# pghysels/STRUMPACK

Hardware: AMD Instinct MI355X
Metric: hss_compress_ulv_factor_solve_gflops (higher is better)
Workload: dtype f64

## Files before the change

include/hssk.h:

```cpp
#ifndef HSSK_H
#define HSSK_H

#ifdef __cplusplus
extern "C" {
#endif

typedef struct hssk_ctx hssk_ctx;

int hssk_ctx_create(hssk_ctx** ctx, int device);
void hssk_ctx_destroy(hssk_ctx* ctx);
void* hssk_ctx_stream(hssk_ctx* ctx);
int hssk_sync(hssk_ctx* ctx);
const char* hssk_last_error(void);
typedef struct hssk_plan hssk_plan;
int hssk_plan_begin(hssk_ctx* ctx, hssk_plan** plan);
int hssk_plan_end(hssk_ctx* ctx);
int hssk_plan_replay(hssk_ctx* ctx, hssk_plan* plan);
void hssk_plan_destroy(hssk_plan* plan);
int hssk_plan_size(const hssk_plan* plan);

void* hssk_malloc(long long bytes);
void hssk_free(void* dptr);
long long hssk_device_total_bytes(void);
int hssk_memcpy_h2d(hssk_ctx* ctx, void* dst, const void* src, long long bytes);
int hssk_memcpy_d2h(hssk_ctx* ctx, void* dst, const void* src, long long bytes);
int hssk_upload_async(hssk_ctx* ctx, void* dst, const void* src, long long bytes);
int hssk_memcpy_d2d(hssk_ctx* ctx, void* dst, const void* src, long long bytes);
int hssk_memcpy2d_h2d(hssk_ctx* ctx, void* dst, long long dpitch, const void* src, long long spitch,
                      long long width, long long height);
int hssk_memcpy2d_d2h(hssk_ctx* ctx, void* dst, long long dpitch, const void* src, long long spitch,
                      long long width, long long height);
int hssk_memset_zero(hssk_ctx* ctx, void* dst, long long bytes);
int hssk_h2d_block_async(hssk_ctx* ctx, double* dst, long long ldd, const double* src, long long lds, long long rows,
                         long long cols);
int hssk_h2d_bytes_async(hssk_ctx* ctx, void* dst, long long dpitch, const void* src, long long spitch, long long width,
                         long long cols);
int hssk_copy_fence(hssk_ctx* ctx);
int hssk_compute_fence(hssk_ctx* ctx);
int hssk_compute_mark(hssk_ctx* ctx, int slot);
int hssk_copy_wait(hssk_ctx* ctx, int slot);
int hssk_is_device_pointer(const void* ptr);
typedef struct hssk_aca_desc {
  const double* A;
  int lda, m, n;
  double rtol, atol;
  int max_rank, row0;
  double* U;
  int ldu;
  double* V;
  int ldv;
  int* rank;
} hssk_aca_desc;
int hssk_aca_vbatched(hssk_ctx* ctx, const hssk_aca_desc* descs, int count);
int hssk_side_begin(hssk_ctx* ctx);
int hssk_side_end(hssk_ctx* ctx);
int hssk_side_join(hssk_ctx* ctx);
int hssk_stream_wait(hssk_ctx* waiter, hssk_ctx* on);
int hssk_watch_start(hssk_ctx* ctx, int id);
int hssk_watch_stop(hssk_ctx* ctx, int id);
double hssk_watch_read_ms(hssk_ctx* ctx, int id, int* pairs);
float hssk_last_dgemm_ms(hssk_ctx* ctx);
double hssk_last_dgemm_flops(hssk_ctx* ctx);
int hssk_dgemm_timing_defer(hssk_ctx* ctx);
int hssk_dgemm_timing_collect(hssk_ctx* ctx, double* ms, double* flops, int* launches);
long long hssk_last_dgemm_trace(hssk_ctx* ctx, long long* out, long long max_wgs);
double hssk_last_dgemm_clock_ghz(hssk_ctx* ctx);

int hssk_fill_toeplitz(hssk_ctx* ctx, double* A, int n, long long lda, char kind);
int hssk_fill_toeplitz_block(hssk_ctx* ctx, double* A, int rows, int cols, long long lda, int i0, int j0, char kind);
int hssk_randn(hssk_ctx* ctx, double* P, int rows, long long cols, long long ld, int row0,
               long long stride, unsigned long long seed);

int hssk_dgemm(hssk_ctx* ctx, int transB, int m, long long n, long long k, double alpha,
               const double* A, long long lda, const double* B, long long ldb, double beta,
               double* C, long long ldc);

int hssk_sgemm_sketch(hssk_ctx* ctx, int transB, int m, long long n, long long k, double alpha,
                      const double* A, long long lda,
                      const float* B, long long ldb,
                      double beta, double* C, long long ldc);
int hssk_narrow_f32(hssk_ctx* ctx, float* dst, long long ldd, const double* src, long long lds, long long rows, long long cols);

#define HSSK_GEN_TOEPLITZ 1
#define HSSK_GEN_TOEPLITZ_UPPER 2
typedef struct hssk_gen {
  int kind, reserved;
  double p[4];
} hssk_gen;
int hssk_sketch_gen(hssk_ctx* ctx, const hssk_gen* g, int transG, int m, long long n, long long k, long long j0, double alpha,
                    const double* A, long long lda, double beta, double* C, long long ldc);
int hssk_gen_fill(hssk_ctx* ctx, const hssk_gen* g, double* A, long long rows, long long cols, long long lda, long long i0,
                  long long j0, int trans);

typedef struct hssk_gemm_desc {
  const double* A;
  const double* B;
  double* C;
  int m, n, k;
  int lda, ldb, ldc;
  int transA, transB;
  double alpha, beta;
} hssk_gemm_desc;
int hssk_gemm_vbatched(hssk_ctx* ctx, const hssk_gemm_desc* descs, int count);

typedef struct hssk_leaf_update_desc {
  const double* R;
  const double* D;
  double* Sr;
  double* Sc;
  int d, m, ldr, ldd, lds;
} hssk_leaf_update_desc;
int hssk_leaf_update_vbatched(hssk_ctx* ctx, const hssk_leaf_update_desc* descs, int count);

typedef struct hssk_kernel_spec {
  const double* X;
  long long n;
  int d, type, p;
  double h, lambda;
} hssk_kernel_spec;
typedef struct hssk_keval_desc {
  const int* ri;
  const int* ci;
  double* out;
  int nr, nc, ldo, r0, c0;
} hssk_keval_desc;
int hssk_kernel_eval_vbatched(hssk_ctx* ctx, const hssk_kernel_spec* spec, const hssk_keval_desc* descs, int count);
int hssk_knn(hssk_ctx* ctx, const double* X, int d, int n, int k, int q0, int q1, int* out_idx);
typedef struct hssk_colset_desc {
  const int* src0;
  const int* src1;
  int n0, n1, lo, hi;
  int* out;
  int* count;
  const int* n0_dev;
  const int* n1_dev;
} hssk_colset_desc;
int hssk_colsets(hssk_ctx* ctx, const hssk_colset_desc* descs, int count, int universe);
long long hssk_colsets_max_universe(void);
int hssk_cluster_median(hssk_ctx* ctx, double* X, int d, int n, int algo, int cluster_size, int* perm, int* status);
int hssk_kernel_predict(hssk_ctx* ctx, const hssk_kernel_spec* spec, const double* w, const double* T, int m, double* pred);

typedef struct hssk_colgather_desc {
  const double* src;
  double* dst;
  const int* idx;
  int rows, ncols, lds, ldd;
  int scatter;
} hssk_colgather_desc;
int hssk_gather_cols(hssk_ctx* ctx, const hssk_colgather_desc* descs, int count);
enum { HSSK_DT_F64 = 0, HSSK_DT_F32 = 1, HSSK_DT_C32 = 2, HSSK_DT_C64 = 3 };
int hssk_expand_image(hssk_ctx* ctx, double* dst, long long ldd, const void* src, long long lds, long long rows, long long cols,
                      int dtype);
typedef struct hssk_rowgather_desc {
  const double* src;
  double* dst;
  const int* idx;
  int nrows, cols, lds, ldd;
  int scatter, accumulate;
} hssk_rowgather_desc;
int hssk_gather_rows(hssk_ctx* ctx, const hssk_rowgather_desc* descs, int count);
typedef struct hssk_elem_desc {
  const double* A;
  long long lda;
  const int* I;
  const int* J;
  int i0, j0;
  double* B;
  int m, n, ldb, transpose;
  int rlo, rhi, clo, chi;
} hssk_elem_desc;
int hssk_gather_elems(hssk_ctx* ctx, const hssk_elem_desc* descs, int count);
int hssk_gather_elems_f32(hssk_ctx* ctx, const hssk_elem_desc* descs, int count);
int hssk_gen_elems(hssk_ctx* ctx, const hssk_gen* g, const hssk_elem_desc* descs, int count);
int hssk_sum_slabs(hssk_ctx* ctx, const double* slabs, long long count, long long stride, int nslab, double* out);
typedef struct hssk_transpose_desc {
  const double* src;
  double* dst;
  int rows, cols, lds, ldd;
} hssk_transpose_desc;
int hssk_transpose(hssk_ctx* ctx, const hssk_transpose_desc* descs, int count);

typedef struct hssk_triu_desc {
  const double* src;
  double* dst;
  int rows, cols, lds, ldd;
  int dstride;
} hssk_triu_desc;
int hssk_copy_triu(hssk_ctx* ctx, const hssk_triu_desc* descs, int count);

int hssk_sjlt_dense(hssk_ctx* ctx, double* Rt, int dn, long long K, long long ld, const int* pat, int nnz);
int hssk_sjlt_sketch(hssk_ctx* ctx, int transA, long long n_out, long long K, const double* A, long long lda,
                     const int* pat, int nnz, int dn, double* St, long long lds);

typedef struct hssk_combine_desc {
  const double *G0, *G1;
  int ldg, gsplit;
  const int* gidx;
  const double *M0, *M1;
  int ldm, msplit;
  const int* midx;
  const double* C;
  int csj, csk;
  double alpha;
  double* out;
  int ldo, rows, J, K;
} hssk_combine_desc;
int hssk_gather_combine(hssk_ctx* ctx, const hssk_combine_desc* descs, int count);

typedef struct hssk_ulvsplit_desc {
  const double* D;
  int ldd, m, r;
  const int* perm;
  const double* X;
  int ldx;
  double* W1;
  int ldw;
  double* W0t;
  int ldt;
} hssk_ulvsplit_desc;
int hssk_ulv_split(hssk_ctx* ctx, const hssk_ulvsplit_desc* descs, int count);
typedef struct hssk_ulvnode_desc {
  const double *B01, *B10, *Vt1a, *Vt1b, *Vd;
  double *Dh, *Vh;
  int ra, rb, rva, rvb;
  int eliminate;
  const int* perm;
  const double* X;
  double *W1, *Rlq, *Qt, *tau, *Vt0T, *Vt1, *Dt, *WQ;
  int m, r, rv, ldt;
} hssk_ulvnode_desc;
int hssk_ulv_node_vbatched(hssk_ctx* ctx, const hssk_ulvnode_desc* descs, int count);
int hssk_ulv_node_fits(int m, int r, int rv, int ra, int rb, int rva, int rvb);
long long hssk_ulv_node_launches(void);

typedef struct hssk_id_desc {
  double* W;
  int ldw, d, m;
  double rtol, atol;
  int max_rank;
  int* perm;
  int* rank;
  double* work;
  const double* src;
  int lds;
  int defer_x;
} hssk_id_desc;
int hssk_id_vbatched(hssk_ctx* ctx, const hssk_id_desc* descs, int count);
long long hssk_id_group_launches(void);
int hssk_id_solves_inline(int dmax, int mmax);
typedef struct hssk_xsolve_desc {
  const double* W;
  int ldw, rank, m;
  double* X;
  int ldx, solved;
} hssk_xsolve_desc;
int hssk_id_xsolve_vbatched(hssk_ctx* ctx, const hssk_xsolve_desc* descs, int count);
typedef struct hssk_pchol_desc {
  const double* G;
  int ldg, m;
  double rtol, atol;
  int max_rank;
  int* perm;
  int* rank;
  double* R;
  int ldr;
} hssk_pchol_desc;
int hssk_pchol_id_vbatched(hssk_ctx* ctx, const hssk_pchol_desc* descs, int count);
int hssk_pchol_id_max_m(void);
int hssk_pchol_id_rank_cap(int m);
typedef struct hssk_sum_desc {
  const double* P;
  long long stride, n;
  int count;
  double* out;
} hssk_sum_desc;
int hssk_sum_partials(hssk_ctx* ctx, const hssk_sum_desc* descs, int count);
typedef struct hssk_gram_desc {
  const double* W;
  int ldw, rows, m;
  double* G;
  int ldg;
} hssk_gram_desc;
int hssk_gram_vbatched(hssk_ctx* ctx, const hssk_gram_desc* descs, int count);
typedef struct hssk_gramgen_desc {
  const int* ri;
  int r0;
  const int* ci;
  int c0;
  int rows, m;
  double* G;
  int ldg;
} hssk_gramgen_desc;
int hssk_gram_gen_vbatched(hssk_ctx* ctx, const hssk_kernel_spec* spec, const hssk_gramgen_desc* descs, int count);
int hssk_gram_gen_supported(const hssk_kernel_spec* spec, int mmax);

typedef struct hssk_tnode {
  int c0, c1, lvl, reserved;
  double* S[2];
  int* perm[2];
  double* Rred[2];
  int* I[2];
  double* X[2];
  double *B01, *B10;
  double* W[2];
  int r[2], m[2], flag[2];
  int status, pad;
} hssk_tnode;
typedef struct hssk_elem_src {
  const double* A;
  long long lda;
  hssk_gen gen;
  int use_gen;
} hssk_elem_src;
int hssk_tree_inner(hssk_ctx* ctx, hssk_tnode* nodes, const int* order, int count, int d, int lds, int rcap, double rtol,
                    double atol, int max_rank, const hssk_elem_src* src, int* res);
int hssk_tree_rcap_max(void);

typedef struct hssk_qr_desc {
  double* A;
  int lda, rows, cols;
  double* Q;
  int ldq, nq;
  double* rdiag;
  double* work;
  int stair;
  double stop_rel, stop_abs;
  int r_only;
} hssk_qr_desc;
int hssk_qr_vbatched(hssk_ctx* ctx, const hssk_qr_desc* descs, int count);
typedef struct hssk_tpqr_desc {
  double* R1;
  int ld1;
  const double* R2;
  int ld2, m;
} hssk_tpqr_desc;
int hssk_tpqr_vbatched(hssk_ctx* ctx, const hssk_tpqr_desc* descs, int count);
int hssk_formq_vbatched(hssk_ctx* ctx, const hssk_qr_desc* descs, int count);

typedef struct hssk_trsm_desc {
  const double* T;
  double* B;
  int n, nrhs, ldt, ldb;
  int lower, transT, unit;
  const double* Tinv;
} hssk_trsm_desc;
int hssk_trsm_vbatched(hssk_ctx* ctx, const hssk_trsm_desc* descs, int count);
typedef struct hssk_lu_desc {
  double* A;
  int n, lda;
  int* piv;
  int* info;
} hssk_lu_desc;
int hssk_getrf_vbatched(hssk_ctx* ctx, const hssk_lu_desc* descs, int count);
typedef struct hssk_lusolve_desc {
  const double* LU;
  const int* piv;
  double* B;
  int n, nrhs, lda, ldb;
} hssk_lusolve_desc;
int hssk_getrs_vbatched(hssk_ctx* ctx, const hssk_lusolve_desc* descs, int count);
int hssk_laswp_vbatched(hssk_ctx* ctx, const hssk_lusolve_desc* descs, int count);

typedef struct hssk_blr_term {
  const double* U;
  const double* V;
  int r, n, src_off, src_flag;
} hssk_blr_term;
typedef struct hssk_blr_row {
  int first_term, nterms, off, m;
  const double* LU;
  int lda, mode;
  const int* piv;
  const double* Tinv;
} hssk_blr_row;
int hssk_blr_sweep(hssk_ctx* ctx, const hssk_blr_row* rows, int nrows, const hssk_blr_term* terms, int nterms, double* X, int* flags);
int hssk_blr_sweep_check(const hssk_blr_row* rows, int nrows, const hssk_blr_term* terms, int nterms);
int hssk_blr_sweep_resident(hssk_ctx* ctx, const hssk_blr_row* d_rows, int nrows, const hssk_blr_term* d_terms, double* X, int* flags);

int hssk_sweep_arm(hssk_ctx* ctx, double* handoff, long long count);
typedef struct hssk_sweep_fwd_desc {
  const double* fsrc;
  const double *B01, *B10, *zc;
  const int* permU;
  const double* XU;
  const double* Rlq;
  const double* Tinv;
  const double* WQ;
  const double* Vt0T;
  const int* permV;
  const double* XV;
  double *ft1, *y, *z;
  const double *LU, *TinvL, *TinvU;
  const int* piv;
  double* xroot;
  int ldf, rU0, rU1, rV0, rV1, ldz_in, m, r, mv, rv, ldp, ldz, ldxr;
  int wait0, wait1;
  const double* G;
  int ldg;
} hssk_sweep_fwd_desc;
int hssk_sweep_chain_ok(int m, int r, int mv, int rv);
long long hssk_sweep_chain_launches(void);
int hssk_ulv_fwd_sweep(hssk_ctx* ctx, const hssk_sweep_fwd_desc* descs, int count, int nrhs);
typedef struct hssk_sweep_bwd_desc {
  const double *Qt, *y, *xpart;
  double* out;
  int m, r, ldx, ldo;
  int wait0;
} hssk_sweep_bwd_desc;
int hssk_ulv_bwd_sweep(hssk_ctx* ctx, const hssk_sweep_bwd_desc* descs, int count, int nrhs);
typedef struct hssk_apply_up_desc {
  const double* src;
  const int* perm;
  const double* X;
  double* dst;
  int m, r, lds, ldd;
  int inner;
  int wait0, wait1;
} hssk_apply_up_desc;
typedef struct hssk_apply_down_desc {
  const double* tmp2;
  const int* perm;
  const double* X;
  const double *D, *x;
  const double *B01, *B10, *t1;
  double* out;
  double beta;
  int ld2, mo, ro, m, ldx, trans, ri_a, ri_b, ro_a, ro_b, ldt1, ldo;
  int wait0, wait1, wait2;
  int acc;
} hssk_apply_down_desc;
int hssk_apply_sweep(hssk_ctx* ctx, const hssk_apply_up_desc* ups, int nup, const hssk_apply_down_desc* downs, int ndown,
                     int nrhs);
int hssk_sweep_status(hssk_ctx* ctx);
int hssk_sweep_require_mma(hssk_ctx* ctx, int on);
int hssk_sweep_mma_min_nrhs(void);
long long hssk_sweep_mma_launches(void);
long long hssk_sweep_fused_launches(void);
long long hssk_sweep_fallbacks(void);
typedef struct hssk_trtri_desc {
  const double* R;
  double* Tinv;
  int n, ldr;
  int mode;
} hssk_trtri_desc;
int hssk_trtri_diag_vbatched(hssk_ctx* ctx, const hssk_trtri_desc* descs, int count);

typedef struct hssk_tree_node {
  int lo, m, c0, c1;
  int rU, rV, mU, mV;
  const double *XU, *XV;
  const int *ipermU, *ipermV;
  const double *B01, *B10, *D;
} hssk_tree_node;
typedef struct hssk_extract_block {
  int ri0, ni, cj0, nj;
  double* out;
  int ldo;
} hssk_extract_block;
int hssk_hss_extract(hssk_ctx* ctx, const hssk_tree_node* nodes, int root, int rmax, int maxdepth, const int* rows, int nrows,
                     const int* cols, int ncols, const hssk_extract_block* blocks, const long long* pair_off, int nblocks,
                     long long npairs, int accumulate, double* work);

typedef struct hssk_norm_desc {
  const double* P;
  int rows, cols, ld;
  double* out;
} hssk_norm_desc;
int hssk_sumsq_vbatched(hssk_ctx* ctx, const hssk_norm_desc* descs, int count);
typedef struct hssk_basis_desc {
  const double* X;
  const int* perm;
  double* out;
  int m, r, ldx, ldo;
} hssk_basis_desc;
int hssk_basis_dense(hssk_ctx* ctx, const hssk_basis_desc* descs, int count);
typedef struct hssk_shift_desc {
  double* A;
  int n, lda;
} hssk_shift_desc;
int hssk_shift_diag(hssk_ctx* ctx, const hssk_shift_desc* descs, int count, double sigma);
int hssk_shift_diag_cplx(hssk_ctx* ctx, const hssk_shift_desc* descs, int count, double re, double im);
double hssk_mfma_f64_peak_tflops(hssk_ctx* ctx, int iters);
int hssk_mfma_f64_probe(hssk_ctx* ctx, int iters, int waves_per_simd, int zero_data, double* out);

#ifdef __cplusplus
}
#endif
#endif
```

strumpack_amd/csrc/host/hss_compress.cpp:

```cpp
#include "hss_engine_internal.hpp"
#include <cstdio>

namespace strumpack {
namespace HSS {

void DeviceHSS::drop_plans() {
  for (auto& kv : plans_) if (kv.second.plan) hssk_plan_destroy(kv.second.plan);
  plans_.clear();
  if (plan_arena_) plan_arena_->reset();
}
bool DeviceHSS::plans_enabled() const {
  static const bool off = [] { const char* e = std::getenv("STRUMPACK_AMD_NO_PLANS"); return e && e[0] == '1'; }();
  return !off;
}

void DeviceHSS::reset_compression() {
  book_ = PendingBook();
  defer_book_ = false;
  drop_plans();
  for (auto& nd : nodes_) {
    int lo = nd.lo, m = nd.m, lvl = nd.lvl, h = nd.height, c0 = nd.c0, c1 = nd.c1, p = nd.parent;
    nd = Node();
    nd.lo = lo; nd.m = m; nd.lvl = lvl; nd.height = h; nd.c0 = c0; nd.c1 = c1; nd.parent = p;
  }
  factor_cancel();
  persist_->reset();
  dev_tree_ = nullptr;
  work_->reset();
  fact_->reset();
  invalidate_factors();
  d_ranks_ = persist_->ints(2 * nodes_.size() + 2);
}

void DeviceHSS::restart_nodes(int d_have) {
  ck(hssk_sync(ctx_));
  factor_cancel();
  for (auto& nd : nodes_) {
    int lo = nd.lo, m = nd.m, lvl = nd.lvl, h = nd.height, c0 = nd.c0, c1 = nd.c1, p = nd.parent;
    nd = Node();
    nd.lo = lo; nd.m = m; nd.lvl = lvl; nd.height = h; nd.c0 = c0; nd.c1 = c1; nd.parent = p;
  }
  persist_->reset();
  dev_tree_ = nullptr;
  invalidate_factors();
  d_ranks_ = persist_->ints(2 * nodes_.size() + 2);
  if (d_have > 0) {
    std::vector<hssk_colgather_desc> cp;
    const int ncols = (int)std::min<long long>(n_, 0x7fffffff);
    cp.push_back(hssk_colgather_desc{Srt0_, Srt_, nullptr, d_have, ncols, dcap_, dcap_, 0});
    cp.push_back(hssk_colgather_desc{Sct0_, Sct_, nullptr, d_have, ncols, dcap_, dcap_, 0});
    ck(hssk_gather_cols(ctx_, cp.data(), 2));
  }
}

void DeviceHSS::free_compress_workspace() {
  ck(hssk_sync(ctx_));
  work_->reset();
  Rt_ = Srt_ = Sct_ = Srt0_ = Sct0_ = nullptr;
  sj_pat_ = nullptr;
  for (auto& nd : nodes_) { nd.Srt = nd.Sct = nd.Rrt = nd.Rct = nd.RrtRed = nd.RctRed = nd.Qr = nd.Qc = nullptr; nd.panels = false; }
}

void DeviceHSS::compress(Source& src) {
  OpGuard op_guard(op_mu_);
  double t0 = now();
  stats_ = PhaseStats();
  int dcap = o_.algorithm != 1 ? o_.d0 + o_.p : o_.d0 + o_.dd;
  dcap = std::max(16, (dcap + 15) / 16 * 16);
  for (;;) {
    if (compress_attempt(src, dcap)) break;
    dcap *= 2;
    if (o_.verbose) std::cout << "# HSS compression: growing the sample capacity to " << dcap << std::endl;
  }
  static const bool trace_host = [] { const char* e = std::getenv("STRUMPACK_AMD_TRACE_HOST"); return e && e[0] == '1'; }();
  const double th0 = now();
  if (dist_subtree_) exchange_node_table();
  free_compress_workspace();
  comm_arena_->reset();
  const double th1 = now();
  {
    const double ms = hssk_watch_read_ms(ctx_, 5, nullptr);
    if (ms > 0.) stats_.t_sketch = ms * 1e-3;
    double kms = 0., kfl = 0.;
    int kn = 0;
    ck(hssk_dgemm_timing_collect(ctx_, &kms, &kfl, &kn));
    stats_.sketch_kernel_ms += kms; stats_.sketch_kernel_flops += kfl; stats_.sketch_launches += kn;
  }
  stats_.t_compress = now() - t0;
  stats_.t_tree = stats_.t_compress - stats_.t_sketch - stats_.t_random;
  stats_.t_mark = now();
  if (trace_host) std::fprintf(stderr, "# host: compress end: free workspace %.1f us, timers %.1f us\n", (th1 - th0) * 1e6, (now() - th1) * 1e6);
}

void DeviceHSS::fill_random(int r0, int dn) {
  if (o_.user_random) { sj_pat_ = nullptr; return; }
  double t0 = now();
  const long long N = n_;
  sj_pat_ = nullptr;
  if (o_.sketch == 1) {
    if (r0 == 0 || !rng_) rng_.reset(new HostRng());
    auto& e = rng_->sj;
    const int nnz = std::max(1, std::min(r0 == 0 ? o_.nnz0 : o_.nnz, dn));
    const bool dense_pat = nnz > 8;
    const int nq = dense_pat ? nnz : (nnz <= 4 ? 4 : 8);
    std::vector<int> pat((size_t)nq * N, dn);
    std::uniform_int_distribution<int> sign(0, 1);
    if (o_.sjlt_algo == 0) {
      const int chunk = dn / nnz;
      std::uniform_int_distribution<int> shift(0, chunk - 1);
      for (long long k = 0; k < N; k++)
        for (int q = 0; q < nnz; q++) {
          const int c = shift(e) + chunk * q;
          pat[(size_t)k * nq + q] = sign(e) == 0 ? c : (c | (int)0x80000000);
        }
    } else {
      std::vector<int> cols(dn);
      for (int j = 0; j < dn; j++) cols[j] = j;
      for (long long k = 0; k < N; k++)
        for (int q = 0; q < nnz; q++) {
          std::uniform_int_distribution<int> pick(q, dn - 1);
          std::swap(cols[q], cols[pick(e)]);
          pat[(size_t)k * nq + q] = sign(e) == 0 ? cols[q] : (cols[q] | (int)0x80000000);
        }
    }
    if (dense_pat) {
      std::vector<double> buf((size_t)dn * N, 0.);
      host_parallel_for((size_t)N, [&](size_t k) {
        for (int q = 0; q < nnz; q++) {
          const int p = pat[k * nq + q];
          buf[(size_t)(p & 0x7fffffff) + k * dn] = p < 0 ? -1. : 1.;
        }
      });
      ck(hssk_memcpy2d_h2d(ctx_, Rt_ + r0, sizeof(double) * dcap_, buf.data(), sizeof(double) * dn, sizeof(double) * dn, N));
      ck(hssk_sync(ctx_));
      stats_.t_random += now() - t0;
      return;
    }
    int* dp = work_->ints((size_t)nq * N);
    ck(hssk_memcpy_h2d(ctx_, dp, pat.data(), (long long)sizeof(int) * nq * N));
    ck(hssk_sjlt_dense(ctx_, Rt_ + r0, dn, N, dcap_, dp, nnz));
    sj_pat_ = dp;
    sj_nnz_ = nnz;
  } else if (o_.random_engine == 2) {
    if (o_.random_dist != 0) throw std::invalid_argument("philox engine implements the normal distribution only");
    ck(hssk_randn(ctx_, Rt_ + r0, dn, N, dcap_, r0, N, 0x5354524dull));
  } else {
    if (r0 == 0 || !rng_) rng_.reset(new HostRng());
    if (o_.random_engine == 0 && o_.random_dist == 0 && N > 0 && dn > 0) {
      std::vector<double> blk((size_t)dn * N);
      rng_->linnorm.fill(blk.data(), blk.size(), [](std::size_t n, const std::function<void(std::size_t)>& fn) { host_parallel_for(n, fn); });
      double* dT = tmp_->dbl((size_t)dn * N);
      ck(hssk_memcpy_h2d(ctx_, dT, blk.data(), (long long)(sizeof(double) * blk.size())));
      hssk_transpose_desc t{dT, Rt_ + r0, (int)N, dn, (int)N, dcap_};
      ck(hssk_transpose(ctx_, &t, 1));
    } else {
      std::minstd_rand* lin = &rng_->lin;
      std::mt19937* mer = &rng_->mer;
      auto& nd = rng_->nd;
      auto& ud = rng_->ud;
      std::vector<double> buf((size_t)dn * N);
      for (int s = 0; s < dn; s++)
        for (long long c = 0; c < N; c++) {
          double v;
          if (o_.random_engine == 0) v = o_.random_dist == 0 ? nd(*lin) : ud(*lin);
          else v = o_.random_dist == 0 ? nd(*mer) : ud(*mer);
          buf[s + (size_t)c * dn] = v;
        }
      ck(hssk_memcpy2d_h2d(ctx_, Rt_ + r0, sizeof(double) * dcap_, buf.data(), sizeof(double) * dn, sizeof(double) * dn, N));
    }
  }
  ck(hssk_sync(ctx_));
  stats_.t_random += now() - t0;
}

bool DeviceHSS::compress_attempt(Source& src, int dcap) {
  reset_compression();
  attempt_++;
  dcap_ = dcap;
  const size_t N = n_;
  cols_per_rank_ = o_.world > 1 ? ((long long)N + o_.world - 1) / o_.world : (long long)N;
  const size_t Npad = o_.world > 1 ? (size_t)cols_per_rank_ * o_.world : N;
  Rt_ = work_->dbl((size_t)dcap * N);
  Srt_ = work_->dbl((size_t)dcap * Npad);
  Sct_ = work_->dbl((size_t)dcap * Npad);
  if (o_.algorithm == 2) { Srt0_ = work_->dbl((size_t)dcap * Npad); Sct0_ = work_->dbl((size_t)dcap * Npad); }
  stats_.rounds = 0;
  stats_.f_sketch = stats_.f_local = stats_.f_reduce = stats_.f_id = stats_.f_ortho = 0;
  const bool original = (o_.algorithm != 1);
  if (!original) {
    int d = o_.d0, dd = o_.dd;
    while (!is_compressed()) {
      int c = (d == o_.d0) ? 0 : d;
      int dnew = (d == o_.d0) ? d + dd : dd;
      if (c + dnew > dcap) return false;
      fill_random(c, dnew);
      if (stats_.rounds == 0 && src.extract_before_sample()) {
        std::vector<int> leaves;
        for (auto& ids : own_by_height_) for (int id : ids) if (nodes_[id].leaf() && nodes_[id].lvl != 0) leaves.push_back(id);
        extract_blocks(src, leaves);
      }
      ck(hssk_watch_start(ctx_, 5));
      src.sample(*this, c, dnew);
      ck(hssk_watch_stop(ctx_, 5));
      stats_.f_sketch += src.sketch_flops(*this, dnew);
      if (o_.verbose) std::cout << "# compressing with d+dd = " << d << "+" << dd << " (stable)" << std::endl;
      stats_.rounds++;
      for (size_t h = 0; h < own_by_height_.size(); h++) {
        if (h == 1 && tree_pass(src, d, dd)) {
          for (size_t hh = 1; hh < own_by_height_.size(); hh++) factor_ahead_level(hh);
          break;
        }
        process_level(src, own_by_height_[h], d, dd, false);
        factor_ahead_level(h);
      }
      if (dist_subtree_) {
        exchange_cut_compress(d + dd);
        for (auto& ids : top_by_height_) process_level(src, ids, d, dd, false);
      }
      stats_.d_final = d + dd;
      if (!is_compressed()) {
        d += dd;
        dd = std::min(dd, o_.max_rank - d);
        if (dd <= 0) break;
      }
    }
  } else {
    int d_old = 0, d = o_.d0 + o_.p;
    while (!is_compressed()) {
      if (d > dcap) return false;
      fill_random(d_old, d - d_old);
      ck(hssk_watch_start(ctx_, 5));
      src.sample(*this, d_old, d - d_old);
      ck(hssk_watch_stop(ctx_, 5));
      stats_.f_sketch += src.sketch_flops(*this, d - d_old);
      if (o_.verbose) std::cout << "# compressing with d = " << d - o_.p << " + " << o_.p << (o_.algorithm == 2 ? " (original, hard restart)" : " (original)") << std::endl;
      if (o_.algorithm == 2) {
        if (dist_subtree_ || o_.world > 1) throw std::invalid_argument("hard restart is a single-GPU option");
        std::vector<hssk_colgather_desc> cp;
        cp.push_back(hssk_colgather_desc{Srt_ + d_old, Srt0_ + d_old, nullptr, d - d_old, (int)N, dcap_, dcap_, 0});
        cp.push_back(hssk_colgather_desc{Sct_ + d_old, Sct0_ + d_old, nullptr, d - d_old, (int)N, dcap_, dcap_, 0});
        ck(hssk_gather_cols(ctx_, cp.data(), 2));
      }
      stats_.rounds++;
      for (auto& ids : own_by_height_) process_level(src, ids, d, d - d_old, true);
      if (dist_subtree_) {
        exchange_cut_compress(d);
        for (auto& ids : top_by_height_) process_level(src, ids, d, d - d_old, true);
      }
      stats_.d_final = d;
      if (!is_compressed()) {
        d_old = d;
        d = 2 * (d_old - o_.p) + o_.p;
        if (d_old >= 4 * n_ + o_.p + 64) break;
        if (o_.algorithm == 2 && d <= dcap) restart_nodes(d_old);
      }
    }
  }
  return true;
}

void DeviceHSS::process_level(Source& src, const std::vector<int>& ids_all, int d, int dd, bool original) {
  const int dtot = original ? d : d + dd;
  const int dnew0 = original ? d - dd : d;
  std::vector<int> ids;
  for (int id : ids_all) {
    Node& nd = nodes_[id];
    if (!nd.leaf() && !(nodes_[nd.c0].compressed() && nodes_[nd.c1].compressed())) continue;
    if (nd.lvl == 0 && nd.compressed()) continue;
    ids.push_back(id);
  }
  if (ids.empty()) return;
  std::vector<int> fresh;
  std::vector<char> was_untouched(nodes_.size(), 0), was_compressed(nodes_.size(), 0);
  for (int id : ids) {
    Node& nd = nodes_[id];
    was_untouched[id] = nd.untouched();
    was_compressed[id] = nd.compressed();
    if (nd.untouched()) fresh.push_back(id);
  }
  extract_blocks(src, fresh);
  std::vector<int> work_ids, r0s, dns;
  for (int id : ids) {
    Node& nd = nodes_[id];
    if (nd.lvl == 0) { nd.Ustate = nd.Vstate = 2; continue; }
    if (!nd.panels) {
      if (nd.leaf()) {
        nd.mU = nd.mV = nd.m;
        nd.Srt = Srt_ + (size_t)nd.lo * dcap_;
        nd.Sct = Sct_ + (size_t)nd.lo * dcap_;
        nd.Rrt = nd.Rct = Rt_ + (size_t)nd.lo * dcap_;
      } else {
        nd.mU = nodes_[nd.c0].rU + nodes_[nd.c1].rU;
        nd.mV = nodes_[nd.c0].rV + nodes_[nd.c1].rV;
        nd.Srt = work_->dbl((size_t)dcap_ * std::max(nd.mU, 1));
        nd.Sct = work_->dbl((size_t)dcap_ * std::max(nd.mV, 1));
        nd.Rrt = work_->dbl((size_t)dcap_ * std::max(nd.mV, 1));
        nd.Rct = work_->dbl((size_t)dcap_ * std::max(nd.mU, 1));
      }
      nd.panels = true;
    }
    work_ids.push_back(id);
    r0s.push_back(was_untouched[id] ? 0 : dnew0);
    dns.push_back(was_untouched[id] ? dtot : dtot - dnew0);
  }
  if (work_ids.empty()) return;
  local_samples(work_ids, r0s, dns);

  std::vector<int> id_nodes, id_which, ot_nodes, ot_which;
  for (int id : work_ids) {
    Node& nd = nodes_[id];
    if (was_compressed[id]) continue;
    for (int w = 0; w < 2; w++) {
      int st = w == 0 ? nd.Ustate : nd.Vstate;
      if (st == 2) continue;
      int rows = w == 0 ? nd.mU : nd.mV;
      if (original || dtot >= o_.max_rank || dtot >= rows) { id_nodes.push_back(id); id_which.push_back(w); }
      else { ot_nodes.push_back(id); ot_which.push_back(w); }
    }
  }
  if (!ot_nodes.empty()) {
    std::vector<char> resolved;
    ortho_test(ot_nodes, ot_which, d, dd, resolved);
    for (size_t i = 0; i < ot_nodes.size(); i++) {
      if (resolved[i]) { id_nodes.push_back(ot_nodes[i]); id_which.push_back(ot_which[i]); }
      else {
        Node& nd = nodes_[ot_nodes[i]];
        (ot_which[i] == 0 ? nd.Ustate : nd.Vstate) = 1;
      }
    }
  }
  defer_book_ = !original;
  run_id(id_nodes, id_which, dtot);
  defer_book_ = false;
  if (original) {
    for (int id : work_ids) {
      Node& nd = nodes_[id];
      if (was_compressed[id]) continue;
      bool ok = (dtot - o_.p >= o_.max_rank) || (nd.rU < dtot - o_.p && nd.rV < dtot - o_.p);
      if (!ok) { nd.Ustate = nd.Vstate = 1; nd.rU = nd.rV = 0; nd.Ir.clear(); nd.Ic.clear(); }
    }
  }
  std::vector<int> rd_ids, rd_r0, rd_dn;
  for (int id : work_ids) {
    Node& nd = nodes_[id];
    if (!nd.compressed()) continue;
    if (!was_compressed[id]) {
      nd.RrtRed = work_->dbl((size_t)dcap_ * std::max(nd.rV, 1));
      nd.RctRed = work_->dbl((size_t)dcap_ * std::max(nd.rU, 1));
      rd_ids.push_back(id); rd_r0.push_back(0); rd_dn.push_back(dtot);
    } else {
      rd_ids.push_back(id); rd_r0.push_back(dnew0); rd_dn.push_back(dtot - dnew0);
    }
  }
  reduce_samples(rd_ids, rd_r0, rd_dn);
  finish_id_bookkeeping();
}

void DeviceHSS::extract_blocks(Source& src, const std::vector<int>& ids) {
  std::vector<ElemReq> reqs;
  for (int id : ids) {
    Node& nd = nodes_[id];
    if (nd.leaf()) {
      if (nd.D) continue;
      nd.D = persist_->dbl((size_t)nd.m * nd.m);
      reqs.push_back(ElemReq{nullptr, nullptr, nullptr, nullptr, nd.lo, nd.lo, nd.m, nd.m, nd.D, nd.m});
    } else {
      Node &a = nodes_[nd.c0], &b = nodes_[nd.c1];
      nd.B01 = persist_->dbl((size_t)std::max(a.rU, 1) * std::max(b.rV, 1));
      nd.B10 = persist_->dbl((size_t)std::max(b.rU, 1) * std::max(a.rV, 1));
      reqs.push_back(ElemReq{a.dIr, b.dIc, &a.Ir, &b.Ic, 0, 0, a.rU, b.rV, nd.B01, std::max(a.rU, 1)});
      reqs.push_back(ElemReq{b.dIr, a.dIc, &b.Ir, &a.Ic, 0, 0, b.rU, a.rV, nd.B10, std::max(b.rU, 1)});
    }
  }
  if (!reqs.empty()) src.extract(*this, reqs);
}

void DeviceHSS::local_samples(const std::vector<int>& ids, const std::vector<int>& r0s, const std::vector<int>& dns) {
  std::vector<hssk_combine_desc> cb;
  std::vector<hssk_gemm_desc> mm;
  std::vector<hssk_leaf_update_desc> lu;
  for (size_t k = 0; k < ids.size(); k++) {
    Node& nd = nodes_[ids[k]];
    const int r0 = r0s[k], dn = dns[k];
    if (dn <= 0) continue;
    if (nd.leaf()) {
      const int m = nd.m;
      if (dn <= 192 && dn % 2 == 0 && r0 % 2 == 0 && nd.Rrt == nd.Rct)
        lu.push_back(hssk_leaf_update_desc{nd.Rrt + r0, nd.D, nd.Srt + r0, nd.Sct + r0, dn, m, dcap_, m, dcap_});
      else {
        mm.push_back(hssk_gemm_desc{nd.Rrt + r0, nd.D, nd.Srt + r0, dn, m, m, dcap_, m, dcap_, 0, 1, -1.0, 1.0});
        mm.push_back(hssk_gemm_desc{nd.Rct + r0, nd.D, nd.Sct + r0, dn, m, m, dcap_, m, dcap_, 0, 0, -1.0, 1.0});
      }
      stats_.f_local += 4.0 * m * (double)m * dn;
    } else {
      Node &a = nodes_[nd.c0], &b = nodes_[nd.c1];
      const int none = 0x7fffffff;
      const int l01 = std::max(a.rU, 1), l10 = std::max(b.rU, 1);
      cb.push_back(hssk_combine_desc{a.Srt + r0, nullptr, dcap_, none, a.permU, b.RrtRed + r0, nullptr, dcap_, none, nullptr,
                                     nd.B01, 1, l01, -1.0, nd.Srt + r0, dcap_, dn, a.rU, b.rV});
      cb.push_back(hssk_combine_desc{b.Srt + r0, nullptr, dcap_, none, b.permU, a.RrtRed + r0, nullptr, dcap_, none, nullptr,
                                     nd.B10, 1, l10, -1.0, nd.Srt + r0 + (size_t)a.rU * dcap_, dcap_, dn, b.rU, a.rV});
      cb.push_back(hssk_combine_desc{a.Sct + r0, nullptr, dcap_, none, a.permV, b.RctRed + r0, nullptr, dcap_, none, nullptr,
                                     nd.B10, l10, 1, -1.0, nd.Sct + r0, dcap_, dn, a.rV, b.rU});
      cb.push_back(hssk_combine_desc{b.Sct + r0, nullptr, dcap_, none, b.permV, a.RctRed + r0, nullptr, dcap_, none, nullptr,
                                     nd.B01, l01, 1, -1.0, nd.Sct + r0 + (size_t)a.rV * dcap_, dcap_, dn, b.rV, a.rU});
      stats_.f_local += 4.0 * ((double)a.rU * b.rV + (double)b.rU * a.rV) * dn;
    }
  }
  if (!cb.empty()) ck(hssk_gather_combine(ctx_, cb.data(), (int)cb.size()));
  if (!lu.empty()) {
    int rc = hssk_leaf_update_vbatched(ctx_, lu.data(), (int)lu.size());
    if (rc == 2) {
      for (auto& u : lu) {
        mm.push_back(hssk_gemm_desc{u.R, u.D, u.Sr, u.d, u.m, u.m, u.ldr, u.ldd, u.lds, 0, 1, -1.0, 1.0});
        mm.push_back(hssk_gemm_desc{u.R, u.D, u.Sc, u.d, u.m, u.m, u.ldr, u.ldd, u.lds, 0, 0, -1.0, 1.0});
      }
    } else ck(rc);
  }
  if (!mm.empty()) ck(hssk_gemm_vbatched(ctx_, mm.data(), (int)mm.size()));
}

void DeviceHSS::reduce_samples(const std::vector<int>& ids, const std::vector<int>& r0s, const std::vector<int>& dns) {
  if (ids.empty()) return;
  std::vector<hssk_combine_desc> cb;
  const int none = 0x7fffffff;
  for (size_t k = 0; k < ids.size(); k++) {
    Node& nd = nodes_[ids[k]];
    const int r0 = r0s[k], dn = dns[k];
    if (dn <= 0) continue;
    const double *rr0, *rr1 = nullptr, *rc0, *rc1 = nullptr;
    int sr = none, sc = none;
    if (nd.leaf()) { rr0 = nd.Rrt + r0; rc0 = nd.Rct + r0; }
    else {
      Node &a = nodes_[nd.c0], &b = nodes_[nd.c1];
      rr0 = a.RrtRed + r0; rr1 = b.RrtRed + r0; sr = a.rV;
      rc0 = a.RctRed + r0; rc1 = b.RctRed + r0; sc = a.rU;
    }
    {
      const int m = nd.mV, r = nd.rV, K = (m > r && r > 0) ? m - r : 0;
      if (r > 0)
        cb.push_back(hssk_combine_desc{rr0, rr1, dcap_, sr, nd.permV, rr0, rr1, dcap_, sr, nd.permV + r, nd.XV, 1, r, 1.0,
                                       nd.RrtRed + r0, dcap_, dn, r, K});
      stats_.f_reduce += 2.0 * r * (double)K * dn;
    }
    {
      const int m = nd.mU, r = nd.rU, K = (m > r && r > 0) ? m - r : 0;
      if (r > 0)
        cb.push_back(hssk_combine_desc{rc0, rc1, dcap_, sc, nd.permU, rc0, rc1, dcap_, sc, nd.permU + r, nd.XU, 1, r, 1.0,
                                       nd.RctRed + r0, dcap_, dn, r, K});
      stats_.f_reduce += 2.0 * r * (double)K * dn;
    }
  }
  if (!cb.empty()) ck(hssk_gather_combine(ctx_, cb.data(), (int)cb.size()));
}

void DeviceHSS::run_id(const std::vector<int>& ids, const std::vector<int>& which, int dtot) {
  if (ids.empty()) return;
  Arena& tmp = *tmp_;
  tmp.rewind();
  const size_t cnt = ids.size();
  std::vector<double*> Ws(cnt, nullptr);
  std::vector<const double*> srcs(cnt, nullptr);
  std::vector<int> ds(cnt, dtot);
  for (size_t k = 0; k < cnt; k++) {
    Node& nd = nodes_[ids[k]];
    const int m = which[k] == 0 ? nd.mU : nd.mV;
    const double* S = which[k] == 0 ? nd.Srt : nd.Sct;
    if (m == 0) continue;
    Ws[k] = tmp.dbl((size_t)dtot * m);
    srcs[k] = S;
  }
  id_panels(ids, which, Ws, ds, &srcs, dcap_);
}

static bool tsqr_staircase() {
  const char* e = std::getenv("STRUMPACK_AMD_TSQR_DENSE");
  return !(e && std::atoi(e));
}

void DeviceHSS::tsqr_reduce(const std::vector<int>& ids, const std::vector<int>& which, std::vector<double*>& Ws,
                            std::vector<int>& ds) {
  Arena& tmp = *tmp_;
  const size_t cnt = ids.size();
  struct Piece { double* p; int ld, rows; };
  std::vector<std::vector<Piece>> pieces(cnt);
  std::vector<int> ms(cnt, 0);
  bool any = false;
  std::vector<hssk_qr_desc> qr;
  for (size_t k = 0; k < cnt; k++) {
    const Node& nd = nodes_[ids[k]];
    const int m = which[k] == 0 ? nd.mU : nd.mV, d = ds[k];
    ms[k] = m;
    if (m <= 0 || !Ws[k] || d <= std::max(256, 2 * m)) continue;
    const int chunk = m <= 192 ? 256 : (m <= 208 ? 208 : (m <= 256 ? 512 : 2 * m));
    for (int r0 = 0; r0 < d; r0 += chunk) {
      const int cr = std::min(chunk, d - r0);
      double* wk = tmp.dbl((size_t)cr + m);
      qr.push_back(hssk_qr_desc{Ws[k] + r0, d, cr, m, nullptr, 0, 0, nullptr, wk, 0, 0., 0., 1});
      pieces[k].push_back(Piece{Ws[k] + r0, d, std::min(cr, m)});
      {
        const double a_ = std::max(cr, m), b_ = std::min(cr, m);
        stats_.f_ortho += 2.0 * a_ * b_ * b_ - 2.0 / 3.0 * b_ * b_ * b_;
      }
    }
    any = true;
  }
  if (!any) return;
  ck(hssk_qr_vbatched(ctx_, qr.data(), (int)qr.size()));
  static const bool pairs_off = [] { const char* e = std::getenv("STRUMPACK_AMD_TSQR_PAIRS"); return e && e[0] == '0'; }();
  for (;;) {
    std::vector<hssk_triu_desc> cp;
    std::vector<hssk_tpqr_desc> tp;
    qr.clear();
    bool more = false;
    for (size_t k = 0; k < cnt; k++) {
      std::vector<Piece>& pc = pieces[k];
      if (pc.size() <= 1) continue;
      const int m = ms[k];
      static const int fan_env = std::getenv("STRUMPACK_AMD_TSQR_FANIN") ? std::atoi(std::getenv("STRUMPACK_AMD_TSQR_FANIN")) : 0;
      const size_t fan_wide = fan_env >= 2 ? (size_t)fan_env : 2;
      const size_t fan = m <= 128 ? std::max<size_t>(2, 256 / std::max(m, 1)) : fan_wide;
      std::vector<Piece> next;
      for (size_t i = 0; i < pc.size(); i += fan) {
        const size_t cntp = std::min(fan, pc.size() - i);
        if (cntp == 1) { next.push_back(pc[i]); continue; }
        int rows = 0;
        bool full = true;
        for (size_t t = 0; t < cntp; t++) { rows += pc[i + t].rows; full = full && pc[i + t].rows == m; }
        if (cntp == 2 && full && m <= 224 && !pairs_off && tsqr_staircase()) {
          tp.push_back(hssk_tpqr_desc{pc[i].p, pc[i].ld, pc[i + 1].p, pc[i + 1].ld, m});
          next.push_back(pc[i]);
          stats_.f_ortho += 2.0 / 3.0 * (double)m * m * m;
          continue;
        }
        double* dst = tmp.dbl((size_t)rows * m);
        const bool stair = full && rows > 256 && tsqr_staircase();
        int r0 = 0;
        for (size_t t = 0; t < cntp; t++) {
          if (stair) cp.push_back(hssk_triu_desc{pc[i + t].p, dst + t, pc[i + t].rows, m, pc[i + t].ld, rows, (int)cntp});
          else cp.push_back(hssk_triu_desc{pc[i + t].p, dst + r0, pc[i + t].rows, m, pc[i + t].ld, rows, 1});
          r0 += pc[i + t].rows;
        }
        double* wk = tmp.dbl((size_t)rows + m);
        qr.push_back(hssk_qr_desc{dst, rows, rows, m, nullptr, 0, 0, nullptr, wk, stair ? (int)cntp : 0, 0., 0., 1});
        next.push_back(Piece{dst, rows, std::min(rows, m)});
        {
          const double a_ = std::max(rows, m), b_ = std::min(rows, m);
          stats_.f_ortho += (2.0 * a_ * b_ * b_ - 2.0 / 3.0 * b_ * b_ * b_) * (stair ? 1.0 / 3.0 : 1.0);
        }
      }
      pc.swap(next);
      more = more || pc.size() > 1;
    }
    if (cp.empty() && tp.empty()) break;
    if (!tp.empty()) ck(hssk_tpqr_vbatched(ctx_, tp.data(), (int)tp.size()));
    if (!cp.empty()) {
      ck(hssk_copy_triu(ctx_, cp.data(), (int)cp.size()));
      ck(hssk_qr_vbatched(ctx_, qr.data(), (int)qr.size()));
    }
    if (!more) break;
  }
  std::vector<hssk_triu_desc> fin;
  for (size_t k = 0; k < cnt; k++) {
    if (pieces[k].empty()) continue;
    const Piece& pc = pieces[k][0];
    double* R = tmp.dbl((size_t)pc.rows * ms[k]);
    fin.push_back(hssk_triu_desc{pc.p, R, pc.rows, ms[k], pc.ld, pc.rows});
    Ws[k] = R;
    ds[k] = pc.rows;
  }
  if (!fin.empty()) ck(hssk_copy_triu(ctx_, fin.data(), (int)fin.size()));
}

void DeviceHSS::id_panels(const std::vector<int>& ids, const std::vector<int>& which, const std::vector<double*>& Ws_in,
                          const std::vector<int>& ds_in, const std::vector<const double*>* srcs, int ldsrc) {
  Arena& tmp = *tmp_;
  const size_t cnt = ids.size();
  std::vector<double*> Ws(Ws_in);
  std::vector<int> ds(ds_in);
  if (srcs) {
    std::vector<hssk_colgather_desc> cp;
    bool tall = false;
    for (size_t k = 0; k < cnt; k++) tall = tall || ds[k] > 256;
    if (tall) {
      for (size_t k = 0; k < cnt; k++) {
        const int m = which[k] == 0 ? nodes_[ids[k]].mU : nodes_[ids[k]].mV;
        if (Ws[k] && m) cp.push_back(hssk_colgather_desc{(*srcs)[k], Ws[k], nullptr, ds[k], m, ldsrc, ds[k], 0});
      }
      if (!cp.empty()) ck(hssk_gather_cols(ctx_, cp.data(), (int)cp.size()));
      srcs = nullptr;
    }
  }
  static const bool gram_on = [] { const char* e = std::getenv("STRUMPACK_AMD_ID_GRAM"); return !(e && e[0] == '0'); }();
  std::vector<char> gram(cnt, 0);
  std::vector<double*> gramR(cnt, nullptr);
  std::vector<int> gramLd(cnt, 0);
  std::vector<hssk_pchol_desc> pcd;
  std::vector<size_t> pck;
  const std::vector<hssk_keval_desc>* gen = id_gen_;
  std::vector<char> evaluated(cnt, gen ? 0 : 1);
  auto evaluate = [&](const std::vector<size_t>& ks_) {
    std::vector<hssk_keval_desc> ev;
    for (size_t k : ks_)
      if (!evaluated[k] && (*gen)[k].out) { ev.push_back((*gen)[k]); evaluated[k] = 1; }
    if (!ev.empty()) ck(hssk_kernel_eval_vbatched(ctx_, &id_gen_spec_, ev.data(), (int)ev.size()));
  };
  if (gram_on && id_gram_ && !srcs) {
    std::vector<hssk_gram_desc> gd;
    std::vector<hssk_gramgen_desc> gg;
    std::vector<hssk_sum_desc> sd;
    size_t tiles_total = 0;
    for (size_t k = 0; k < cnt; k++) {
      const Node& nd = nodes_[ids[k]];
      const int m = which[k] == 0 ? nd.mU : nd.mV, d = ds[k];
      if (m <= 0 || m > hssk_pchol_id_max_m() || !Ws[k] || d <= std::max(256, 2 * m) || o_.rel_tol / nd.lvl < 1e-6) continue;
      gram[k] = 1;
      tiles_total++;
    }
    for (size_t k = 0; k < cnt; k++) {
      if (!gram[k]) continue;
      const Node& nd = nodes_[ids[k]];
      const int m = which[k] == 0 ? nd.mU : nd.mV, d = ds[k];
      static const int wgs = [] { const char* e = std::getenv("STRUMPACK_AMD_GRAM_WGS"); return e ? std::max(1, std::atoi(e)) : 768; }();
      const int want = (int)std::max<size_t>(1, ((size_t)wgs + tiles_total - 1) / tiles_total);
      const int chunks = std::max(1, std::min(want, (d + 255) / 256)), rows = ((d + chunks - 1) / chunks + 15) & ~15;
      int nch = (d + rows - 1) / rows;
      if (nch > 1 && d - (nch - 1) * rows < 16) nch--;
      double* G = tmp.dbl((size_t)m * m);
      double* P = nch > 1 ? tmp.dbl((size_t)nch * m * m) : G;
      const bool fused = gen && (*gen)[k].out == Ws[k] && hssk_gram_gen_supported(&id_gen_spec_, m);
      for (int c = 0; c < nch; c++) {
        const int r0 = c * rows, kr = c == nch - 1 ? d - r0 : rows;
        if (fused) {
          const hssk_keval_desc& kd = (*gen)[k];
          gg.push_back(hssk_gramgen_desc{kd.ri ? kd.ri + r0 : nullptr, kd.r0 + r0, kd.ci, kd.c0, kr, m, P + (size_t)c * m * m, m});
        } else gd.push_back(hssk_gram_desc{Ws[k] + r0, d, kr, m, P + (size_t)c * m * m, m});
      }
      if (!fused && gen) evaluate({k});
      if (nch > 1) sd.push_back(hssk_sum_desc{P, (long long)m * m, (long long)m * m, nch, G});
      const int cap = std::max(1, std::min(m, hssk_pchol_id_rank_cap(m)));
      gramR[k] = tmp.dbl((size_t)cap * m);
      gramLd[k] = cap;
      pcd.push_back(hssk_pchol_desc{G, m, m, o_.rel_tol / nd.lvl, o_.abs_tol / nd.lvl, o_.max_rank, nullptr, nullptr, gramR[k], cap});
      pck.push_back(k);
      stats_.f_ortho += (double)d * m * (m + 1.0);
    }
    if (!gd.empty()) ck(hssk_gram_vbatched(ctx_, gd.data(), (int)gd.size()));
    if (!gg.empty()) ck(hssk_gram_gen_vbatched(ctx_, &id_gen_spec_, gg.data(), (int)gg.size()));
    if (!sd.empty()) ck(hssk_sum_partials(ctx_, sd.data(), (int)sd.size()));
  }
  {
    std::vector<double*> Wt(Ws);
    for (size_t k = 0; k < cnt; k++) if (gram[k]) Wt[k] = nullptr;
    if (gen) {
      std::vector<size_t> rest;
      for (size_t k = 0; k < cnt; k++) if (!gram[k]) rest.push_back(k);
      evaluate(rest);
    }
    tsqr_reduce(ids, which, Wt, ds);
    for (size_t k = 0; k < cnt; k++) if (!gram[k]) Ws[k] = Wt[k];
  }
  std::vector<hssk_id_desc> idd;
  int id_dmax = 0, id_mmax = 0;
  std::vector<int*> perms(cnt, nullptr);
  size_t perm_total = 0;
  for (size_t k = 0; k < cnt; k++) perm_total += (which[k] == 0 ? nodes_[ids[k]].mU : nodes_[ids[k]].mV);
  int* rank_block = persist_->ints(cnt + std::max<size_t>(perm_total, 1));
  int* perm_block = rank_block + cnt;
  size_t poff = 0;
  for (size_t k = 0; k < cnt; k++) {
    Node& nd = nodes_[ids[k]];
    const int m = which[k] == 0 ? nd.mU : nd.mV;
    perms[k] = perm_block + poff;
    poff += m;
    if (m == 0) continue;
    if (gram[k]) continue;
    double* wk = tmp.dbl(3 * (size_t)m);
    idd.push_back(hssk_id_desc{Ws[k], ds[k], ds[k], m, o_.rel_tol / nd.lvl, o_.abs_tol / nd.lvl, o_.max_rank, perms[k], rank_block + k, wk,
                               srcs ? (*srcs)[k] : nullptr, ldsrc, 1});
    id_dmax = std::max(id_dmax, ds[k]);
    id_mmax = std::max(id_mmax, m);
  }
  if (!idd.empty()) ck(hssk_id_vbatched(ctx_, idd.data(), (int)idd.size()));
  for (size_t q = 0; q < pcd.size(); q++) { pcd[q].perm = perms[pck[q]]; pcd[q].rank = rank_block + pck[q]; }
  if (!pcd.empty()) ck(hssk_pchol_id_vbatched(ctx_, pcd.data(), (int)pcd.size()));
  const int x_solved = hssk_id_solves_inline(id_dmax, id_mmax);
  std::vector<int> hall(cnt + std::max<size_t>(perm_total, 1));
  ck(hssk_memcpy_d2h(ctx_, hall.data(), rank_block, (long long)sizeof(int) * (cnt + perm_total)));
  {
    std::vector<int> rid, rwh, rds;
    std::vector<double*> rW;
    std::vector<size_t> rk_;
    for (size_t k = 0; k < cnt; k++)
      if (gram[k] && hall[k] < 0) { rid.push_back(ids[k]); rwh.push_back(which[k]); rW.push_back(Ws[k]); rds.push_back(ds[k]); rk_.push_back(k); }
    if (!rid.empty()) {
      if (gen) evaluate(rk_);
      tsqr_reduce(rid, rwh, rW, rds);
      std::vector<hssk_id_desc> rdd;
      int dmx = 0, mmx = 0;
      for (size_t q = 0; q < rid.size(); q++) {
        const size_t k = rk_[q];
        const Node& nd = nodes_[ids[k]];
        const int m = which[k] == 0 ? nd.mU : nd.mV;
        double* wk = tmp.dbl(3 * (size_t)m);
        rdd.push_back(hssk_id_desc{rW[q], rds[q], rds[q], m, o_.rel_tol / nd.lvl, o_.abs_tol / nd.lvl, o_.max_rank, perms[k], rank_block + k, wk, nullptr, 0, 0});
        dmx = std::max(dmx, rds[q]); mmx = std::max(mmx, m);
        gram[k] = 2;
        Ws[k] = rW[q]; ds[k] = rds[q];
      }
      ck(hssk_id_vbatched(ctx_, rdd.data(), (int)rdd.size()));
      ck(hssk_memcpy_d2h(ctx_, hall.data(), rank_block, (long long)sizeof(int) * (cnt + perm_total)));
    }
  }
  if (hssk_sweep_status(ctx_)) throw std::runtime_error(std::string("compress: interpolative decomposition: ") + hssk_last_error());
  const int* hranks = hall.data();
  const int* hperm = hall.data() + cnt;
  std::vector<hssk_xsolve_desc> xc;
  std::vector<size_t> idx_off(cnt), perm_off(cnt);
  size_t idx_total = 0;
  poff = 0;
  for (size_t k = 0; k < cnt; k++) {
    Node& nd = nodes_[ids[k]];
    const int w = which[k];
    const int m = w == 0 ? nd.mU : nd.mV;
    const int dtot = gram[k] == 1 ? gramLd[k] : ds[k];
    const int r = m ? hranks[k] : 0;
    perm_off[k] = poff;
    poff += m;
    idx_off[k] = idx_total;
    idx_total += r;
    double* X = persist_->dbl((size_t)std::max(r, 1) * std::max(m - r, 1));
    if (r > 0 && m > r) xc.push_back(hssk_xsolve_desc{gram[k] == 1 ? gramR[k] : Ws[k], dtot, r, m, X, r, gram[k] == 1 ? 0 : (gram[k] == 2 ? 1 : x_solved)});
    if (w == 0) { nd.rU = r; nd.XU = X; nd.permU = perms[k]; nd.Ustate = 2; }
    else { nd.rV = r; nd.XV = X; nd.permV = perms[k]; nd.Vstate = 2; }
    stats_.f_id += 2.0 * (4.0 * m * (double)dtot * r - 2.0 * (m + dtot) * (double)r * r + 4.0 * r * (double)r * r / 3.0 + (double)r * r * (m - r));
  }
  if (!xc.empty()) ck(hssk_id_xsolve_vbatched(ctx_, xc.data(), (int)xc.size()));
  book_.ids = ids; book_.which = which; book_.hall = std::move(hall);
  book_.idx_off = std::move(idx_off); book_.perm_off = std::move(perm_off);
  book_.cnt = cnt; book_.idx_total = idx_total; book_.active = true;
  if (!defer_book_) finish_id_bookkeeping();
}

void DeviceHSS::finish_id_bookkeeping() {
  if (!book_.active) return;
  book_.active = false;
  const std::vector<int>&ids = book_.ids, &which = book_.which;
  const size_t cnt = book_.cnt, idx_total = book_.idx_total;
  const int* hperm = book_.hall.data() + cnt;
  std::vector<int> idx_host(std::max<size_t>(idx_total, 1));
  for (size_t k = 0; k < cnt; k++) {
    Node& nd = nodes_[ids[k]];
    const int w = which[k];
    const int m = w == 0 ? nd.mU : nd.mV;
    const int r = w == 0 ? nd.rU : nd.rV;
    std::vector<int> perm(hperm + book_.perm_off[k], hperm + book_.perm_off[k] + m);
    std::vector<int> I(r);
    if (nd.leaf()) for (int i = 0; i < r; i++) I[i] = nd.lo + perm[i];
    else {
      const std::vector<int>& ia = w == 0 ? nodes_[nd.c0].Ir : nodes_[nd.c0].Ic;
      const std::vector<int>& ib = w == 0 ? nodes_[nd.c1].Ir : nodes_[nd.c1].Ic;
      const int r0 = (int)ia.size();
      for (int i = 0; i < r; i++) I[i] = perm[i] < r0 ? ia[perm[i]] : ib[perm[i] - r0];
    }
    std::copy(I.begin(), I.end(), idx_host.begin() + book_.idx_off[k]);
    if (w == 0) { nd.hpermU = std::move(perm); nd.Ir = std::move(I); }
    else { nd.hpermV = std::move(perm); nd.Ic = std::move(I); }
  }
  int* idx_dev = persist_->ints(std::max<size_t>(idx_total, 1));
  if (idx_total) ck(hssk_upload_async(ctx_, idx_dev, idx_host.data(), (long long)sizeof(int) * idx_total));
  for (size_t k = 0; k < cnt; k++) {
    Node& nd = nodes_[ids[k]];
    (which[k] == 0 ? nd.dIr : nd.dIc) = idx_dev + book_.idx_off[k];
  }
}

void DeviceHSS::ortho_test(const std::vector<int>& ids, const std::vector<int>& which, int d, int dd,
                           std::vector<char>& resolved) {
  const size_t cnt = ids.size();
  resolved.assign(cnt, 0);
  Arena& tmp = *tmp_;
  tmp.rewind();
  std::vector<hssk_transpose_desc> tr;
  std::vector<hssk_colgather_desc> cp;
  std::vector<hssk_qr_desc> qr;
  double* rdiag = tmp.dbl(2 * cnt);
  std::vector<char> untouched(cnt);
  for (size_t k = 0; k < cnt; k++) {
    Node& nd = nodes_[ids[k]];
    const int w = which[k];
    const int m = w == 0 ? nd.mU : nd.mV;
    const double* S = w == 0 ? nd.Srt : nd.Sct;
    double* Q = w == 0 ? nd.Qr : nd.Qc;
    untouched[k] = (w == 0 ? nd.Ustate : nd.Vstate) == 0;
    int c2, n2;
    if (untouched[k]) { c2 = 0; n2 = std::min(d, m); }
    else { c2 = d - dd; n2 = std::min(dd, m - (d - dd)); }
    double* T = tmp.dbl((size_t)m * std::max(n2, 1));
    if (untouched[k]) tr.push_back(hssk_transpose_desc{S, T, n2, m, dcap_, m});
    else cp.push_back(hssk_colgather_desc{Q + (size_t)c2 * m, T, nullptr, m, n2, m, m, 0});
    double* wk = tmp.dbl((size_t)m + n2);
    {
      const double atol = o_.abs_tol / nd.lvl, rtol = o_.rel_tol / nd.lvl;
      const double r0 = w == 0 ? nd.Ur_max : nd.Vr_max;
      hssk_qr_desc q{T, m, m, n2, nullptr, m, 0, rdiag + 2 * k, wk, 0, 0., 0.};
      if (untouched[k]) { q.stop_rel = rtol * (1. - 1e-12); q.stop_abs = atol; }
      else q.stop_abs = std::max(atol, rtol * std::abs(r0) * (1. - 1e-12));
      qr.push_back(q);
    }
    stats_.f_ortho += 4.0 * m * (double)n2 * n2;
  }
  if (!cp.empty()) ck(hssk_gather_cols(ctx_, cp.data(), (int)cp.size()));
  if (!tr.empty()) ck(hssk_transpose(ctx_, tr.data(), (int)tr.size()));
  ck(hssk_qr_vbatched(ctx_, qr.data(), (int)qr.size()));
  std::vector<double> hr(2 * cnt);
  ck(hssk_memcpy_d2h(ctx_, hr.data(), rdiag, (long long)sizeof(double) * 2 * cnt));
  std::vector<size_t> pend;
  for (size_t k = 0; k < cnt; k++) {
    Node& nd = nodes_[ids[k]];
    const int w = which[k];
    double r_max = hr[2 * k], r_min = hr[2 * k + 1];
    double& r_max_0 = w == 0 ? nd.Ur_max : nd.Vr_max;
    if (untouched[k]) r_max_0 = r_max;
    const double atol = o_.abs_tol / nd.lvl, rtol = o_.rel_tol / nd.lvl;
    if (std::abs(r_min) < atol || std::abs(r_min / r_max_0) < rtol) resolved[k] = 1;
    else pend.push_back(k);
  }
  if (pend.empty()) return;
  {
    std::vector<hssk_qr_desc> fq;
    tr.clear();
    for (size_t k : pend) {
      Node& nd = nodes_[ids[k]];
      const int w = which[k];
      const int m = w == 0 ? nd.mU : nd.mV;
      const double* S = w == 0 ? nd.Srt : nd.Sct;
      double*& Q = w == 0 ? nd.Qr : nd.Qc;
      if (!Q) Q = work_->dbl((size_t)m * dcap_);
      const int c2 = untouched[k] ? 0 : d - dd;
      hssk_qr_desc q = qr[k];
      q.Q = Q + (size_t)c2 * m; q.ldq = m; q.nq = q.cols; q.rdiag = nullptr;
      fq.push_back(q);
      tr.push_back(hssk_transpose_desc{S + d, Q + (size_t)d * m, dd, m, dcap_, m});
    }
    ck(hssk_formq_vbatched(ctx_, fq.data(), (int)fq.size()));
    ck(hssk_transpose(ctx_, tr.data(), (int)tr.size()));
  }
  const int pc = std::min(dd, o_.p);
  double* nrm = tmp.dbl(2 * pend.size());
  std::vector<hssk_norm_desc> n0, n1;
  std::vector<hssk_gemm_desc> g1, g2;
  for (size_t i = 0; i < pend.size(); i++) {
    size_t k = pend[i];
    Node& nd = nodes_[ids[k]];
    const int w = which[k];
    const int m = w == 0 ? nd.mU : nd.mV;
    double* Q = w == 0 ? nd.Qr : nd.Qc;
    const int q12 = std::min(d, m);
    double* Q3 = Q + (size_t)d * m;
    double* P = tmp.dbl((size_t)q12 * dd);
    n0.push_back(hssk_norm_desc{Q3, m, pc, m, nrm + 2 * i});
    g1.push_back(hssk_gemm_desc{Q, Q3, P, q12, dd, m, m, m, q12, 1, 0, 1.0, 0.0});
    g2.push_back(hssk_gemm_desc{Q, P, Q3, m, dd, q12, m, q12, m, 0, 0, -1.0, 1.0});
    n1.push_back(hssk_norm_desc{Q3, m, pc, m, nrm + 2 * i + 1});
    stats_.f_ortho += 8.0 * m * (double)q12 * dd;
  }
  ck(hssk_sumsq_vbatched(ctx_, n0.data(), (int)n0.size()));
  for (int it = 0; it < 2; it++) {
    ck(hssk_gemm_vbatched(ctx_, g1.data(), (int)g1.size()));
    ck(hssk_gemm_vbatched(ctx_, g2.data(), (int)g2.size()));
  }
  ck(hssk_sumsq_vbatched(ctx_, n1.data(), (int)n1.size()));
  std::vector<double> hn(2 * pend.size());
  ck(hssk_memcpy_d2h(ctx_, hn.data(), nrm, (long long)sizeof(double) * hn.size()));
  for (size_t i = 0; i < pend.size(); i++) {
    size_t k = pend[i];
    Node& nd = nodes_[ids[k]];
    const double atol = o_.abs_tol / nd.lvl, rtol = o_.rel_tol / nd.lvl;
    double S3 = std::sqrt(hn[2 * i]), Q3 = std::sqrt(hn[2 * i + 1]);
    if (Q3 / std::sqrt(double(dd)) < atol || Q3 / S3 < rtol) resolved[k] = 1;
  }
}

}
}
```

strumpack_amd/csrc/host/hss_sources.cpp:

```cpp
#include "hss_engine_internal.hpp"

namespace strumpack {
namespace HSS {

double DeviceHSS::Source::sketch_flops(const DeviceHSS& H, int dn) const {
  return 2.0 * products(H) * (double)H.n_ * (double)H.n_ * (H.sj_pat_ ? H.sj_nnz_ : dn);
}

struct DeviceHSS::DenseDeviceSource : DeviceHSS::Source {
  const double* dA;
  long long lda;
  DenseDeviceSource(const double* a, long long l) : dA(a), lda(l) {}
  bool extract_before_sample() const override { return true; }
  bool device_elems(const DeviceHSS&, hssk_elem_src* e) const override { e->A = dA; e->lda = lda; e->use_gen = 0; return true; }
  int done_products_ = 2;
  bool done_sparse_ = false;
  int products(const DeviceHSS&) const override { return done_products_; }
  double sketch_flops(const DeviceHSS& H, int dn) const override {
    return 2.0 * done_products_ * (double)H.n_ * (double)H.n_ * (done_sparse_ ? H.sj_nnz_ : dn);
  }
  void sample(DeviceHSS& H, int r0, int dn) override {
    const long long N = H.n_;
    long long j0 = 0, j1 = N;
    if (H.dist_subtree_) {
      const Node& c = H.nodes_[H.cut_nodes_[H.o_.rank]];
      j0 = c.lo; j1 = c.lo + c.m;
    } else if (H.o_.world > 1) {
      j0 = std::min(N, H.cols_per_rank_ * H.o_.rank); j1 = std::min(N, j0 + H.cols_per_rank_);
    }
    const long long nloc = j1 - j0;
    static const bool sj_dense = std::getenv("STRUMPACK_AMD_SJLT_DENSE") && std::atoi(std::getenv("STRUMPACK_AMD_SJLT_DENSE"));
    done_sparse_ = H.sj_pat_ && dn <= 1024 && !sj_dense;
    done_products_ = (!done_sparse_ && H.o_.symmetric) ? 1 : 2;
    if (nloc > 0 && done_sparse_) {
      for (int t = 0; t < 2; t++) {
        const double* Aop = t == 0 ? dA + j0 : dA + j0 * lda;
        double* St = (t == 0 ? H.Srt_ : H.Sct_) + r0 + j0 * H.dcap_;
        ck(hssk_sjlt_sketch(H.ctx_, t, nloc, N, Aop, lda, H.sj_pat_, H.sj_nnz_, dn, St, H.dcap_));
        ck(hssk_sync(H.ctx_));
        float ms = hssk_last_dgemm_ms(H.ctx_);
        if (ms > 0) {
          H.stats_.sketch_kernel_ms += ms; H.stats_.sketch_launches++;
          H.stats_.sketch_kernel_flops += hssk_last_dgemm_flops(H.ctx_);
          H.stats_.sketch_kernel_bytes += 8.0 * (double)nloc * (double)N;
        }
      }
    } else if (nloc > 0) {
      ck(hssk_dgemm(H.ctx_, 1, dn, nloc, N, 1.0, H.Rt_ + r0, H.dcap_, dA + j0, lda, 0.0, H.Srt_ + r0 + j0 * H.dcap_, H.dcap_));
      ck(hssk_dgemm_timing_defer(H.ctx_));
      if (H.o_.symmetric) {
        hssk_colgather_desc cp{H.Srt_ + r0 + j0 * H.dcap_, H.Sct_ + r0 + j0 * H.dcap_, nullptr, dn, (int)nloc, H.dcap_, H.dcap_, 0};
        ck(hssk_gather_cols(H.ctx_, &cp, 1));
      } else {
        ck(hssk_dgemm(H.ctx_, 0, dn, nloc, N, 1.0, H.Rt_ + r0, H.dcap_, dA + j0 * lda, lda, 0.0, H.Sct_ + r0 + j0 * H.dcap_, H.dcap_));
        ck(hssk_dgemm_timing_defer(H.ctx_));
      }
    }
    if (H.o_.world > 1 && !H.dist_subtree_) {
      const long long bytes = (long long)sizeof(double) * H.dcap_ * H.cols_per_rank_;
      H.comm(H.Srt_, bytes);
      H.comm(H.Sct_, bytes);
    }
  }
  void extract(DeviceHSS& H, const std::vector<ElemReq>& reqs) override {
    std::vector<hssk_elem_desc> d;
    d.reserve(reqs.size());
    for (auto& r : reqs)
      if (r.m > 0 && r.n > 0) d.push_back(hssk_elem_desc{dA, lda, r.dI, r.dJ, r.i0, r.j0, r.dB, r.m, r.n, r.ldb, 0});
    if (!d.empty()) ck(hssk_gather_elems(H.ctx_, d.data(), (int)d.size()));
  }
};

struct DeviceHSS::DenseDeviceSourceF32 : DeviceHSS::Source {
  const float* dA;
  long long lda;
  int route;
  double* dBuf = nullptr;
  long long nb = 0;
  int gen = -1;
  int done_products_ = 2;
  DenseDeviceSourceF32(const float* a, long long l, int r) : dA(a), lda(l), route(r) {}
  bool extract_before_sample() const override { return true; }
  bool device_elems(const DeviceHSS&, hssk_elem_src* e) const override {
    e->A = reinterpret_cast<const double*>(dA); e->lda = lda; e->use_gen = 2;
    return true;
  }
  int products(const DeviceHSS&) const override { return done_products_; }
  double sketch_flops(const DeviceHSS& H, int dn) const override { return 2.0 * done_products_ * (double)H.n_ * (double)H.n_ * dn; }
  void sample(DeviceHSS& H, int r0, int dn) override {
    if (H.o_.world > 1) throw std::invalid_argument("single-precision device operand: single-GPU only (multi-GPU float operands are not supported)");
    if (H.sj_pat_) throw std::invalid_argument("single-precision device operand: the SJLT sketch is not supported; use the Gaussian sketch");
    const long long N = H.n_;
    if (N <= 0 || dn <= 0) return;
    auto timed = [&](double bytes) {
      ck(hssk_dgemm_timing_defer(H.ctx_));
      H.stats_.sketch_kernel_bytes += bytes;
    };
    if (route == 1) {
      done_products_ = H.o_.symmetric ? 1 : 2;
      ck(hssk_sgemm_sketch(H.ctx_, 1, dn, N, N, 1.0, H.Rt_ + r0, H.dcap_, dA, lda, 0.0, H.Srt_ + r0, H.dcap_));
      timed(4.0 * (double)N * (double)N);
      if (H.o_.symmetric) {
        hssk_colgather_desc cp{H.Srt_ + r0, H.Sct_ + r0, nullptr, dn, (int)N, H.dcap_, H.dcap_, 0};
        ck(hssk_gather_cols(H.ctx_, &cp, 1));
      } else {
        ck(hssk_sgemm_sketch(H.ctx_, 0, dn, N, N, 1.0, H.Rt_ + r0, H.dcap_, dA, lda, 0.0, H.Sct_ + r0, H.dcap_));
        timed(4.0 * (double)N * (double)N);
      }
      return;
    }
    done_products_ = 2;
    if (gen != H.attempt_) {
      gen = H.attempt_;
      nb = std::max<long long>(64, (1LL << 30) / (8 * N) / 64 * 64);
      nb = std::min(nb, (N + 63) / 64 * 64);
      dBuf = H.work_->dbl((size_t)N * nb);
    }
    for (long long c0 = 0, b = 0; c0 < N; c0 += nb, b++) {
      const long long c1 = std::min(N, c0 + nb);
      ck(hssk_expand_image(H.ctx_, dBuf, N, dA + c0 * lda, lda, N, c1 - c0, HSSK_DT_F32));
      ck(hssk_dgemm(H.ctx_, 0, dn, c1 - c0, N, 1.0, H.Rt_ + r0, H.dcap_, dBuf, N, 0.0, H.Sct_ + r0 + c0 * H.dcap_, H.dcap_));
      timed(0.);
      ck(hssk_dgemm(H.ctx_, 1, dn, N, c1 - c0, 1.0, H.Rt_ + r0 + c0 * H.dcap_, H.dcap_, dBuf, N, b ? 1.0 : 0.0, H.Srt_ + r0, H.dcap_));
      timed(0.);
    }
  }
  void extract(DeviceHSS& H, const std::vector<ElemReq>& reqs) override {
    std::vector<hssk_elem_desc> d;
    d.reserve(reqs.size());
    for (auto& r : reqs)
      if (r.m > 0 && r.n > 0) d.push_back(hssk_elem_desc{reinterpret_cast<const double*>(dA), lda, r.dI, r.dJ, r.i0, r.j0, r.dB, r.m, r.n, r.ldb, 0});
    if (!d.empty()) ck(hssk_gather_elems_f32(H.ctx_, d.data(), (int)d.size()));
  }
};

struct DeviceHSS::ShardedDenseSource : DeviceHSS::Source {
  const double* dRows;
  long long ldr;
  const double* dCols;
  long long ldc;
  ShardedDenseSource(const double* r, long long lr, const double* c, long long lc) : dRows(r), ldr(lr), dCols(c), ldc(lc) {}
  bool device_elems(const DeviceHSS& H, hssk_elem_src* e) const override {
    const Node& c = H.nodes_[H.o_.world == 1 ? 0 : H.cut_nodes_[H.o_.rank]];
    e->A = dCols - (long long)c.lo * ldc; e->lda = ldc; e->use_gen = 0;
    return true;
  }
  void sample(DeviceHSS& H, int r0, int dn) override {
    const bool single = H.o_.world == 1;
    if (!single && !H.dist_subtree_) throw std::invalid_argument("sharded operand: the tree cannot be cut into one subtree per rank (world must be a power of two and the tree complete down to that depth)");
    if (H.sj_pat_) throw std::invalid_argument("sharded operand: the SJLT sketch needs the replicated-operand interface");
    const long long N = H.n_;
    const Node& c = H.nodes_[single ? 0 : H.cut_nodes_[H.o_.rank]];
    const long long j0 = c.lo, nloc = c.m;
    auto timed = [&] { ck(hssk_dgemm_timing_defer(H.ctx_)); };
    ck(hssk_dgemm(H.ctx_, 0, dn, nloc, N, 1.0, H.Rt_ + r0, H.dcap_, dCols, ldc, 0.0, H.Sct_ + r0 + j0 * H.dcap_, H.dcap_));
    timed();
    if (dRows) {
      ck(hssk_dgemm(H.ctx_, 1, dn, nloc, N, 1.0, H.Rt_ + r0, H.dcap_, dRows, ldr, 0.0, H.Srt_ + r0 + j0 * H.dcap_, H.dcap_));
      timed();
    } else {
      H.tmp_->rewind();
      double* P = H.tmp_->dbl((size_t)dn * N);
      double* mineP = H.tmp_->dbl((size_t)dn * nloc);
      ck(hssk_dgemm(H.ctx_, 1, dn, N, nloc, 1.0, H.Rt_ + r0 + j0 * H.dcap_, H.dcap_, dCols, ldc, 0.0, P, dn));
      timed();
      const double tc = now();
      std::vector<long long> offs(H.o_.world), counts(H.o_.world);
      for (int g = 0; g < H.o_.world; g++) {
        const Node& cg = H.nodes_[single ? 0 : H.cut_nodes_[g]];
        offs[g] = (long long)cg.lo * dn; counts[g] = (long long)cg.m * dn;
      }
      H.reduce_scatter_sum(P, offs, counts, mineP);
      hssk_colgather_desc cp{mineP, H.Srt_ + r0 + j0 * H.dcap_, nullptr, dn, (int)nloc, dn, H.dcap_, 0};
      ck(hssk_gather_cols(H.ctx_, &cp, 1));
      ck(hssk_sync(H.ctx_));
      H.stats_.t_comm += now() - tc;
    }
  }
  void extract(DeviceHSS& H, const std::vector<ElemReq>& reqs) override {
    const Node& c = H.nodes_[H.o_.world == 1 ? 0 : H.cut_nodes_[H.o_.rank]];
    const int j0 = c.lo, j1 = c.lo + c.m;
    auto inside = [&](const std::vector<int>* h, int i0, int cnt) {
      if (!h) return i0 >= j0 && i0 + cnt <= j1;
      for (int i = 0; i < cnt; i++) if ((*h)[i] < j0 || (*h)[i] >= j1) return false;
      return true;
    };
    std::vector<hssk_elem_desc> own, part, back;
    size_t tot = 0;
    for (auto& r : reqs) if (r.m > 0 && r.n > 0 && !(inside(r.hI, r.i0, r.m) && inside(r.hJ, r.j0, r.n))) tot += (size_t)r.m * r.n;
    double* stage = tot ? H.comm_arena_->dbl(tot) : nullptr;
    size_t off = 0;
    for (auto& r : reqs) {
      if (r.m <= 0 || r.n <= 0) continue;
      if (inside(r.hI, r.i0, r.m) && inside(r.hJ, r.j0, r.n)) {
        own.push_back(hssk_elem_desc{dCols - (long long)j0 * ldc, ldc, r.dI, r.dJ, r.i0, r.j0, r.dB, r.m, r.n, r.ldb, 0, 0, 0, 0, 0});
      } else {
        double* T = stage + off;
        off += (size_t)r.m * r.n;
        if (dRows) part.push_back(hssk_elem_desc{dRows - j0, ldr, r.dI, r.dJ, r.i0, r.j0, T, r.m, r.n, r.m, 0, j0, j1, 0, 0});
        else part.push_back(hssk_elem_desc{dCols - (long long)j0 * ldc, ldc, r.dI, r.dJ, r.i0, r.j0, T, r.m, r.n, r.m, 0, 0, 0, j0, j1});
        back.push_back(hssk_elem_desc{T, r.m, nullptr, nullptr, 0, 0, r.dB, r.m, r.n, r.ldb, 0, 0, 0, 0, 0});
      }
    }
    if (!own.empty()) ck(hssk_gather_elems(H.ctx_, own.data(), (int)own.size()));
    if (!part.empty()) {
      const double tc = now();
      ck(hssk_gather_elems(H.ctx_, part.data(), (int)part.size()));
      H.allreduce_sum(stage, (long long)tot);
      ck(hssk_gather_elems(H.ctx_, back.data(), (int)back.size()));
      H.stats_.t_comm += now() - tc;
    }
  }
};

struct DeviceHSS::HostBlockSource : DeviceHSS::Source {
  const void* hA;
  long long lda;
  int dtype = HSSK_DT_F64;
  const host_fill_t* fill;
  const host_elem_t* elem;
  double* dBuf[2] = {nullptr, nullptr};
  double* dNat[2] = {nullptr, nullptr};
  long long nb = 0;
  int gen = -1;
  std::vector<double*> dcache;
  HostBlockSource(const void* a, long long l, const host_fill_t* f, const host_elem_t* e, int dt = HSSK_DT_F64)
      : hA(a), lda(l), dtype(dt), fill(f), elem(e) {}
  long long reals() const { return dtype == HSSK_DT_C32 || dtype == HSSK_DT_C64 ? 2 : 1; }
  size_t esize() const { return dtype == HSSK_DT_F32 ? 4 : dtype == HSSK_DT_C64 ? 16 : 8; }
  double image_at(size_t I, size_t J) const {
    switch (dtype) {
      case HSSK_DT_F32: return (double)((const float*)hA)[I + J * (size_t)lda];
      case HSSK_DT_C32: {
        const float* z = (const float*)hA + 2 * (I / 2 + (J / 2) * (size_t)lda);
        return (I & 1) == (J & 1) ? (double)z[0] : ((I & 1) ? (double)z[1] : -(double)z[1]);
      }
      case HSSK_DT_C64: {
        const double* z = (const double*)hA + 2 * (I / 2 + (J / 2) * (size_t)lda);
        return (I & 1) == (J & 1) ? z[0] : ((I & 1) ? z[1] : -z[1]);
      }
      default: return ((const double*)hA)[I + J * (size_t)lda];
    }
  }
  void sample(DeviceHSS& H, int r0, int dn) override {
    if (H.o_.world > 1) throw std::invalid_argument("host-resident operands are single-GPU (use the device / sharded interfaces)");
    const long long N = H.n_;
    const bool typed = hA && dtype != HSSK_DT_F64;
    const long long W = typed ? reals() : 1, ns = N / W;
    if (typed && N % W) throw std::logic_error("image dimension of a complex operand must be even");
    const bool first = gen != H.attempt_;
    if (first) {
      gen = H.attempt_;
      long long bytes = 1536LL << 20;
      if (const char* e = std::getenv("STRUMPACK_AMD_HOST_BLOCK_MB")) bytes = std::max(1LL, std::atoll(e)) << 20;
      if (const char* e = std::getenv("STRUMPACK_AMD_HOST_BLOCK_KB")) bytes = std::max(1LL, std::atoll(e)) << 10;
      nb = std::max<long long>(64, bytes / (8 * std::max<long long>(N, 1)) / 64 * 64);
      nb = std::min(nb, (N + 63) / 64 * 64);
      dBuf[0] = H.work_->dbl((size_t)N * nb);
      if (!typed) dBuf[1] = H.work_->dbl((size_t)N * nb);
      else for (int k = 0; k < 2; k++) dNat[k] = H.work_->dbl(((size_t)ns * (size_t)(nb / W) * esize() + 7) / 8);
    }
    const long long nblk = (N + nb - 1) / nb;
    const bool capture = first;
    if (capture) {
      dcache.assign(H.nodes_.size(), nullptr);
      for (size_t id = 0; id < H.nodes_.size(); id++)
        if (H.nodes_[id].leaf() && H.nodes_[id].m > 0) dcache[id] = H.work_->dbl((size_t)H.nodes_[id].m * H.nodes_[id].m);
    }
    std::vector<double> tmp;
    auto upload = [&](long long b) {
      const long long c0 = b * nb, c1 = std::min(N, c0 + nb);
      if (typed)
        ck(hssk_h2d_bytes_async(H.ctx_, dNat[b & 1], (long long)(ns * esize()), (const char*)hA + (size_t)(c0 / W) * lda * esize(),
                                (long long)(lda * esize()), (long long)(ns * esize()), (c1 - c0) / W));
      else if (hA) ck(hssk_h2d_block_async(H.ctx_, dBuf[b & 1], N, (const double*)hA + (size_t)c0 * lda, lda, N, c1 - c0));
      else {
        tmp.resize((size_t)N * (c1 - c0));
        (*fill)(c0, c1, tmp.data());
        ck(hssk_h2d_block_async(H.ctx_, dBuf[b & 1], N, tmp.data(), N, N, c1 - c0));
      }
    };
    upload(0);
    for (long long b = 0; b < nblk; b++) {
      const long long c0 = b * nb, c1 = std::min(N, c0 + nb);
      ck(hssk_copy_fence(H.ctx_));
      const double* Ab = typed ? dBuf[0] : dBuf[b & 1];
      if (typed) {
        ck(hssk_expand_image(H.ctx_, dBuf[0], N, dNat[b & 1], ns, ns, (c1 - c0) / W, dtype));
        ck(hssk_compute_mark(H.ctx_, (int)(b & 1)));
      }
      ck(hssk_dgemm(H.ctx_, 0, dn, c1 - c0, N, 1.0, H.Rt_ + r0, H.dcap_, Ab, N, 0.0, H.Sct_ + r0 + c0 * H.dcap_, H.dcap_));
      ck(hssk_dgemm(H.ctx_, 1, dn, N, c1 - c0, 1.0, H.Rt_ + r0 + c0 * H.dcap_, H.dcap_, Ab, N, b ? 1.0 : 0.0, H.Srt_ + r0, H.dcap_));
      if (capture) {
        std::vector<hssk_colgather_desc> dg;
        for (size_t id = 0; id < H.nodes_.size(); id++) {
          const Node& nd = H.nodes_[id];
          if (!dcache[id]) continue;
          const long long a = std::max<long long>(nd.lo, c0), e = std::min<long long>(nd.lo + nd.m, c1);
          if (a >= e) continue;
          dg.push_back(hssk_colgather_desc{Ab + nd.lo + (size_t)(a - c0) * N, dcache[id] + (size_t)(a - nd.lo) * nd.m, nullptr, nd.m, (int)(e - a),
                                           (int)N, nd.m, 0});
        }
        if (!dg.empty()) ck(hssk_gather_cols(H.ctx_, dg.data(), (int)dg.size()));
      }
      if (!typed) ck(hssk_compute_mark(H.ctx_, (int)(b & 1)));
      if (b + 1 < nblk) {
        ck(hssk_copy_wait(H.ctx_, (int)((b + 1) & 1)));
        upload(b + 1);
      }
    }
    ck(hssk_sync(H.ctx_));
  }
  void extract(DeviceHSS& H, const std::vector<ElemReq>& reqs) override {
    std::vector<size_t> off(reqs.size() + 1, 0);
    for (size_t k = 0; k < reqs.size(); k++) off[k + 1] = off[k] + (size_t)std::max(reqs[k].m, 0) * std::max(reqs[k].n, 0);
    std::vector<const double*> hit(reqs.size(), nullptr);
    if (!dcache.empty()) {
      std::vector<std::pair<int, size_t>> by_lo;
      for (size_t id = 0; id < H.nodes_.size(); id++) if (dcache[id]) by_lo.push_back({H.nodes_[id].lo, id});
      std::sort(by_lo.begin(), by_lo.end());
      std::vector<hssk_colgather_desc> cp;
      for (size_t k = 0; k < reqs.size(); k++) {
        const ElemReq& r = reqs[k];
        if (r.hI || r.hJ || r.i0 != r.j0 || r.m != r.n || r.m <= 0 || gen != H.attempt_) continue;
        auto it = std::lower_bound(by_lo.begin(), by_lo.end(), std::make_pair(r.i0, size_t(0)));
        if (it == by_lo.end() || it->first != r.i0 || H.nodes_[it->second].m != r.m) continue;
        hit[k] = dcache[it->second];
        cp.push_back(hssk_colgather_desc{hit[k], r.dB, nullptr, r.m, r.n, r.m, r.ldb, 0});
      }
      if (!cp.empty()) ck(hssk_gather_cols(H.ctx_, cp.data(), (int)cp.size()));
    }
    for (size_t k = 0; k < reqs.size(); k++)
      if (hit[k]) off[k + 1] = off[k];
      else off[k + 1] = off[k] + (size_t)std::max(reqs[k].m, 0) * std::max(reqs[k].n, 0);
    std::unique_ptr<double[]> img_store(new double[std::max<size_t>(off.back(), 1)]);
    struct { double* p; double* data() { return p; } } img{img_store.get()};
    host_parallel_for(reqs.size(), [&](size_t k) {
      const ElemReq& r = reqs[k];
      if (r.m <= 0 || r.n <= 0 || hit[k]) return;
      double* B = img.data() + off[k];
      if (hA && dtype != HSSK_DT_F64) {
        for (int j = 0; j < r.n; j++) {
          const size_t J = (size_t)(r.hJ ? (*r.hJ)[j] : r.j0 + j);
          for (int i = 0; i < r.m; i++) B[i + (size_t)j * r.m] = image_at((size_t)(r.hI ? (*r.hI)[i] : r.i0 + i), J);
        }
      } else if (hA) {
        for (int j = 0; j < r.n; j++) {
          const double* col = (const double*)hA + (size_t)(r.hJ ? (*r.hJ)[j] : r.j0 + j) * lda;
          if (r.hI) for (int i = 0; i < r.m; i++) B[i + (size_t)j * r.m] = col[(*r.hI)[i]];
          else std::memcpy(B + (size_t)j * r.m, col + r.i0, sizeof(double) * r.m);
        }
      } else {
        std::vector<int> I(r.m), J(r.n);
        for (int i = 0; i < r.m; i++) I[i] = r.hI ? (*r.hI)[i] : r.i0 + i;
        for (int j = 0; j < r.n; j++) J[j] = r.hJ ? (*r.hJ)[j] : r.j0 + j;
        (*elem)(r.m, I.data(), r.n, J.data(), B, r.m);
      }
    });
    for (size_t k = 0; k < reqs.size(); k++) {
      const ElemReq& r = reqs[k];
      if (r.m <= 0 || r.n <= 0 || hit[k]) continue;
      if (r.ldb == r.m) ck(hssk_upload_async(H.ctx_, r.dB, img.data() + off[k], (long long)(sizeof(double) * (off[k + 1] - off[k]))));
      else ck(hssk_memcpy2d_h2d(H.ctx_, r.dB, sizeof(double) * r.ldb, img.data() + off[k], sizeof(double) * r.m, sizeof(double) * r.m, r.n));
    }
  }
};

struct DeviceHSS::CallbackSource : DeviceHSS::Source {
  const host_mult_t* mult;
  const host_sample_t* usample = nullptr;
  const host_elem_t& elem;
  CallbackSource(const host_mult_t& m, const host_elem_t& e) : mult(&m), elem(e) {}
  CallbackSource(const host_sample_t& s, const host_elem_t& e) : mult(nullptr), usample(&s), elem(e) {}
  void sample(DeviceHSS& H, int r0, int dn) override {
    if (H.o_.world > 1) throw std::invalid_argument("the host-callback interface is single-GPU");
    if (usample) {
      const int N = H.n_;
      if (N == 0 || dn == 0) return;
      std::vector<double> R((size_t)N * dn), Sr((size_t)N * dn), Sc((size_t)N * dn);
      (*usample)(N, dn, R.data(), Sr.data(), Sc.data());
      double* dT = H.tmp_->dbl((size_t)N * dn);
      const double* src[3] = {R.data(), Sr.data(), Sc.data()};
      double* dst[3] = {H.Rt_ + r0, H.Srt_ + r0, H.Sct_ + r0};
      for (int q = 0; q < 3; q++) {
        ck(hssk_memcpy_h2d(H.ctx_, dT, src[q], (long long)(sizeof(double) * (size_t)N * dn)));
        hssk_transpose_desc b{dT, dst[q], N, dn, N, H.dcap_};
        ck(hssk_transpose(H.ctx_, &b, 1));
        ck(hssk_sync(H.ctx_));
      }
      return;
    }
    const int N = H.n_;
    if (N == 0 || dn == 0) return;
    double* dT = H.tmp_->dbl((size_t)N * dn);
    std::vector<double> R((size_t)N * dn), S((size_t)N * dn);
    hssk_transpose_desc t{H.Rt_ + r0, dT, dn, N, H.dcap_, N};
    ck(hssk_transpose(H.ctx_, &t, 1));
    ck(hssk_memcpy_d2h(H.ctx_, R.data(), dT, (long long)(sizeof(double) * R.size())));
    for (int pass = 0; pass < 2; pass++) {
      (*mult)(pass == 0 ? 'N' : 'C', N, dn, R.data(), N, S.data(), N);
      ck(hssk_memcpy_h2d(H.ctx_, dT, S.data(), (long long)(sizeof(double) * S.size())));
      hssk_transpose_desc b{dT, (pass == 0 ? H.Srt_ : H.Sct_) + r0, N, dn, N, H.dcap_};
      ck(hssk_transpose(H.ctx_, &b, 1));
      ck(hssk_sync(H.ctx_));
    }
  }
  void extract(DeviceHSS& H, const std::vector<ElemReq>& reqs) override {
    for (auto& r : reqs) {
      if (r.m <= 0 || r.n <= 0) continue;
      std::vector<int> I(r.m), J(r.n);
      for (int i = 0; i < r.m; i++) I[i] = r.hI ? (*r.hI)[i] : r.i0 + i;
      for (int j = 0; j < r.n; j++) J[j] = r.hJ ? (*r.hJ)[j] : r.j0 + j;
      std::vector<double> B((size_t)r.m * r.n);
      elem(r.m, I.data(), r.n, J.data(), B.data(), r.m);
      ck(hssk_memcpy2d_h2d(H.ctx_, r.dB, sizeof(double) * r.ldb, B.data(), sizeof(double) * r.m, sizeof(double) * r.m, r.n));
    }
  }
};

struct DeviceHSS::GeneratorSource : DeviceHSS::Source {
  hssk_gen g;
  explicit GeneratorSource(const hssk_gen& g_) : g(g_) {}
  bool extract_before_sample() const override { return true; }
  bool device_elems(const DeviceHSS&, hssk_elem_src* e) const override { e->A = nullptr; e->lda = 0; e->gen = g; e->use_gen = 1; return true; }
  int products(const DeviceHSS& H) const override { return H.o_.symmetric ? 1 : 2; }
  void sample(DeviceHSS& H, int r0, int dn) override {
    if (H.sj_pat_) throw std::invalid_argument("generated operand: the SJLT sketch streams a stored matrix; use the Gaussian sketch");
    const long long N = H.n_;
    long long j0 = 0, j1 = N;
    if (H.dist_subtree_) {
      const Node& c = H.nodes_[H.cut_nodes_[H.o_.rank]];
      j0 = c.lo; j1 = c.lo + c.m;
    } else if (H.o_.world > 1) {
      j0 = std::min(N, H.cols_per_rank_ * H.o_.rank); j1 = std::min(N, j0 + H.cols_per_rank_);
    }
    const long long nloc = j1 - j0;
    auto timed = [&] { ck(hssk_dgemm_timing_defer(H.ctx_)); };
    if (nloc > 0) {
      ck(hssk_sketch_gen(H.ctx_, &g, 1, dn, nloc, N, j0, 1.0, H.Rt_ + r0, H.dcap_, 0.0, H.Srt_ + r0 + j0 * H.dcap_, H.dcap_));
      timed();
      if (H.o_.symmetric) {
        hssk_colgather_desc cp{H.Srt_ + r0 + j0 * H.dcap_, H.Sct_ + r0 + j0 * H.dcap_, nullptr, dn, (int)nloc, H.dcap_, H.dcap_, 0};
        ck(hssk_gather_cols(H.ctx_, &cp, 1));
      } else {
        ck(hssk_sketch_gen(H.ctx_, &g, 0, dn, nloc, N, j0, 1.0, H.Rt_ + r0, H.dcap_, 0.0, H.Sct_ + r0 + j0 * H.dcap_, H.dcap_));
        timed();
      }
    }
    if (H.o_.world > 1 && !H.dist_subtree_) {
      const long long bytes = (long long)sizeof(double) * H.dcap_ * H.cols_per_rank_;
      H.comm(H.Srt_, bytes);
      H.comm(H.Sct_, bytes);
    }
  }
  void extract(DeviceHSS& H, const std::vector<ElemReq>& reqs) override {
    std::vector<hssk_elem_desc> d;
    d.reserve(reqs.size());
    for (auto& r : reqs)
      if (r.m > 0 && r.n > 0) d.push_back(hssk_elem_desc{nullptr, 0, r.dI, r.dJ, r.i0, r.j0, r.dB, r.m, r.n, r.ldb, 0});
    if (!d.empty()) ck(hssk_gen_elems(H.ctx_, &g, d.data(), (int)d.size()));
  }
};

void DeviceHSS::compress_generator(const hssk_gen& g) {
  GeneratorSource s(g);
  check_symmetry(s);
  compress(s);
}
void DeviceHSS::check_symmetry(Source& src) {
  if (o_.symmetric != 2 || n_ < 2) return;
  const int q = std::min(512, n_);
  std::vector<int> I(q), J(q);
  std::minstd_rand g(12345);
  for (int i = 0; i < q; i++) { I[i] = (int)(g() % (unsigned)n_); J[i] = (int)(g() % (unsigned)n_); }
  tmp_->rewind();
  int* dI = tmp_->ints(q);
  int* dJ = tmp_->ints(q);
  double* B1 = tmp_->dbl((size_t)q * q);
  double* B2 = tmp_->dbl((size_t)q * q);
  ck(hssk_memcpy_h2d(ctx_, dI, I.data(), (long long)sizeof(int) * q));
  ck(hssk_memcpy_h2d(ctx_, dJ, J.data(), (long long)sizeof(int) * q));
  std::vector<ElemReq> rq{ElemReq{dI, dJ, &I, &J, 0, 0, q, q, B1, q}, ElemReq{dJ, dI, &J, &I, 0, 0, q, q, B2, q}};
  src.extract(*this, rq);
  std::vector<double> h1((size_t)q * q), h2((size_t)q * q);
  ck(hssk_memcpy_d2h(ctx_, h1.data(), B1, (long long)sizeof(double) * q * q));
  ck(hssk_memcpy_d2h(ctx_, h2.data(), B2, (long long)sizeof(double) * q * q));
  double dmax = 0, amax = 0;
  for (int j = 0; j < q; j++)
    for (int i = 0; i < q; i++) {
      dmax = std::max(dmax, std::abs(h1[i + (size_t)j * q] - h2[j + (size_t)i * q]));
      amax = std::max(amax, std::abs(h1[i + (size_t)j * q]));
    }
  if (dmax > 1e-14 * std::max(amax, 1e-300)) throw std::invalid_argument("compress: the operand was declared symmetric and is not (sampled entries differ from their mirror images)");
}

void DeviceHSS::compress_dense_device(const double* dA, long long lda) {
  DenseDeviceSource s(dA, lda);
  check_symmetry(s);
  compress(s);
}
void DeviceHSS::compress_dense_device_f32(const float* dA, long long lda, int precision) {
  if (precision < 0 || precision > 2) throw std::invalid_argument("compress_dense_device_f32: sketch precision must be 0 (auto), 1 (FP32 matrix cores) or 2 (exact)");
  if (o_.world > 1) throw std::invalid_argument("compress_dense_device_f32: single-GPU only (multi-GPU float operands are not supported)");
  if (o_.sketch == 1) throw std::invalid_argument("compress_dense_device_f32: the SJLT sketch is not supported on a float operand; use the Gaussian sketch");
  if (!dA || lda < n_) throw std::invalid_argument("compress_dense_device_f32: bad operand");
  const int route = precision ? precision : (o_.rel_tol >= ((double)n_ + 4.) * std::ldexp(1., -24) ? 1 : 2);
  f32_route_ = route;
  DenseDeviceSourceF32 s(dA, lda, route);
  check_symmetry(s);
  compress(s);
}
void DeviceHSS::compress_dense_host(const double* A, long long lda) {
  HostBlockSource s(A, lda, nullptr, nullptr);
  compress(s);
}
void DeviceHSS::compress_dense_host_typed(const void* A, long long lda, int dtype) {
  if (dtype != HSSK_DT_F32 && dtype != HSSK_DT_C32 && dtype != HSSK_DT_C64) throw std::invalid_argument("compress_dense_host_typed: unknown scalar type");
  HostBlockSource s(A, lda, nullptr, nullptr, dtype);
  compress(s);
}
void DeviceHSS::compress_host_blocks(const host_fill_t& fill, const host_elem_t& elem) {
  HostBlockSource s(nullptr, 0, &fill, &elem);
  compress(s);
}
void DeviceHSS::compress_dense_device_sharded(const double* dRows, long long ldr, const double* dCols, long long ldc) {
  if (!dCols) throw std::invalid_argument("sharded operand: the column block is required");
  ShardedDenseSource s(dRows, ldr, dCols, ldc);
  compress(s);
}
bool DeviceHSS::shard_range(int rank, int& lo, int& hi) const {
  if (o_.world == 1) { lo = 0; hi = n_; return true; }
  if (!dist_subtree_ || rank < 0 || rank >= (int)cut_nodes_.size()) return false;
  lo = nodes_[cut_nodes_[rank]].lo;
  hi = lo + nodes_[cut_nodes_[rank]].m;
  return true;
}
void DeviceHSS::compress_callbacks_user_random(const host_sample_t& sample, const host_elem_t& elem) {
  if (!o_.user_random) throw std::logic_error("compress_callbacks_user_random: the engine was not built with user_random");
  CallbackSource s(sample, elem);
  compress(s);
}
void DeviceHSS::compress_callbacks(const host_mult_t& mult, const host_elem_t& elem) {
  CallbackSource s(mult, elem);
  compress(s);
}

}
}
```

strumpack_amd/csrc/kernels/hssk_dgemm.hip:

```cpp
#include "hssk_device.h"
#include "hssk_internal.h"
#include "hssk_gen.h"

#include <algorithm>
#include <cstdlib>
#include <type_traits>

namespace {

constexpr int BN = 64, BK = 16;

template <int BM, bool TRANSB, bool FULL, int TAG = 0>
__global__ __launch_bounds__(256, 2) void dgemm_kernel(int m, long long n, long long k, const double* __restrict__ A,
                                                       long long lda, const double* __restrict__ B, long long ldb,
                                                       double* __restrict__ P, long long ldp, long long pstride,
                                                       long long kchunk, int jtile0, long long* __restrict__ clk) {
  const long long t0_ = clk ? hssk_clock() : 0, w0_ = clk ? hssk_wallclock() : 0;
  constexpr int LDA_S = BM + 16, LDB_S = BN + 16;
  constexpr int WM = BM / 2;
  constexpr int MT = WM / 16;
  constexpr int NT = 2;
  constexpr int A_PER_THREAD = BM * BK / 256;
  constexpr int B_PER_THREAD = BN * BK / 256;
  constexpr int A2 = A_PER_THREAD / 2, B2 = B_PER_THREAD / 2;
  HSSK_SHARED double As[2 * BK * LDA_S];
  HSSK_SHARED double Bs[2 * BK * LDB_S];

  const int tid = threadIdx.x, lane = tid & 63, wave = tid >> 6;
  const int l15 = lane & 15, l4 = lane >> 4;
  int bx = blockIdx.x;
  {
    const int nx = gridDim.x, x = bx & 7, q = nx >> 3, r = nx & 7;
    bx = x * q + (x < r ? x : r) + (bx >> 3);
  }
  const long long j0 = (long long)(bx + jtile0) * BN;
  const int i0 = blockIdx.y * BM;
  const long long kbeg = (long long)blockIdx.z * kchunk;
  const long long kend = kbeg + kchunk < k ? kbeg + kchunk : k;
  const int wm = (wave & 1) * WM, wn = (wave >> 1) * 32;

  hssk_d4 acc[MT][NT];
#pragma unroll
  for (int a = 0; a < MT; a++)
#pragma unroll
    for (int b = 0; b < NT; b++) acc[a][b] = hssk_d4{0., 0., 0., 0.};

  const double* Ak = A + i0 + kbeg * lda;
  const double* Bk = TRANSB ? B + j0 + kbeg * ldb : B + j0 * ldb + kbeg;
  const long long stepA = (long long)BK * lda, stepB = TRANSB ? (long long)BK * ldb : (long long)BK;
  const long long nst = (kend - kbeg + BK - 1) / BK;

  auto compute = [&](int buf) {
    const double* as = As + buf * BK * LDA_S + wm + l15;
    const double* bs = Bs + buf * BK * LDB_S + wn + l15;
    double af[2][MT], bf[2][NT];
#pragma unroll
    for (int a = 0; a < MT; a++) af[0][a] = as[l4 * LDA_S + a * 16];
#pragma unroll
    for (int b = 0; b < NT; b++) bf[0][b] = bs[l4 * LDB_S + b * 16];
#pragma unroll
    for (int ks = 0; ks < BK; ks += 4) {
      const int cur = (ks >> 2) & 1, nxt = cur ^ 1;
      if (ks + 4 < BK) {
#pragma unroll
        for (int a = 0; a < MT; a++) af[nxt][a] = as[(ks + 4 + l4) * LDA_S + a * 16];
#pragma unroll
        for (int b = 0; b < NT; b++) bf[nxt][b] = bs[(ks + 4 + l4) * LDB_S + b * 16];
      }
#pragma unroll
      for (int a = 0; a < MT; a++)
#pragma unroll
        for (int b = 0; b < NT; b++)
          acc[a][b] = hssk_mfma_f64_16x16x4(bf[cur][b], af[cur][a], acc[a][b]);
    }
  };

  if (FULL) {
    int offA[A2], ldsA[A2], offB[B2], ldsB[B2];
#pragma unroll
    for (int r = 0; r < A2; r++) {
      int e = tid + 256 * r;
      int i = 2 * (e % (BM / 2)), kk = e / (BM / 2);
      offA[r] = i + kk * (int)lda;
      ldsA[r] = kk * LDA_S + i;
    }
#pragma unroll
    for (int r = 0; r < B2; r++) {
      int e = tid + 256 * r;
      if (TRANSB) {
        int j = 2 * (e % (BN / 2)), kk = e / (BN / 2);
        offB[r] = j + kk * (int)ldb;
        ldsB[r] = kk * LDB_S + j;
      } else {
        int kk = 2 * (e % (BK / 2)), j = e / (BK / 2);
        offB[r] = kk + j * (int)ldb;
        ldsB[r] = kk * LDB_S + j;
      }
    }
    hssk_d2 ra0[A2], rb0[B2], ra1[A2], rb1[B2];
    auto load = [&](hssk_d2 (&ra)[A2], hssk_d2 (&rb)[B2]) {
#pragma unroll
      for (int r = 0; r < A2; r++) ra[r] = *reinterpret_cast<const hssk_d2*>(Ak + offA[r]);
#pragma unroll
      for (int r = 0; r < B2; r++) rb[r] = *reinterpret_cast<const hssk_d2*>(Bk + offB[r]);
      Ak += stepA; Bk += stepB;
    };
    auto store = [&](int buf, const hssk_d2 (&ra)[A2], const hssk_d2 (&rb)[B2]) {
      double* as = As + buf * BK * LDA_S;
      double* bs = Bs + buf * BK * LDB_S;
#pragma unroll
      for (int r = 0; r < A2; r++) *reinterpret_cast<hssk_d2*>(as + ldsA[r]) = ra[r];
#pragma unroll
      for (int r = 0; r < B2; r++) {
        if (TRANSB) *reinterpret_cast<hssk_d2*>(bs + ldsB[r]) = rb[r];
        else { bs[ldsB[r]] = rb[r][0]; bs[ldsB[r] + LDB_S] = rb[r][1]; }
      }
    };
    load(ra0, rb0);
    store(0, ra0, rb0);
    if (nst > 1) load(ra1, rb1);
    __syncthreads();
    long long st = 0;
    for (; st + 2 < nst; st += 2) {
      load(ra0, rb0);
      compute(0);
      store(1, ra1, rb1);
      __syncthreads();
      if (st + 3 < nst) load(ra1, rb1);
      compute(1);
      store(0, ra0, rb0);
      __syncthreads();
    }
    compute(0);
    if (st + 1 < nst) {
      store(1, ra1, rb1);
      __syncthreads();
      compute(1);
    }
  } else {
    double ra[A_PER_THREAD], rb[B_PER_THREAD];
    auto load = [&](long long k0) {
#pragma unroll
      for (int r = 0; r < A_PER_THREAD; r++) {
        int e = tid + 256 * r;
        int i = e % BM, kk = e / BM;
        ra[r] = (i0 + i < m && k0 + kk < kend) ? A[i0 + i + (k0 + kk) * lda] : 0.;
      }
#pragma unroll
      for (int r = 0; r < B_PER_THREAD; r++) {
        int e = tid + 256 * r;
        if (TRANSB) {
          int j = e % BN, kk = e / BN;
          rb[r] = (j0 + j < n && k0 + kk < kend) ? B[j0 + j + (k0 + kk) * ldb] : 0.;
        } else {
          int kk = e % BK, j = e / BK;
          rb[r] = (j0 + j < n && k0 + kk < kend) ? B[k0 + kk + (j0 + j) * ldb] : 0.;
        }
      }
    };
    auto store = [&](int buf) {
      double* as = As + buf * BK * LDA_S;
      double* bs = Bs + buf * BK * LDB_S;
#pragma unroll
      for (int r = 0; r < A_PER_THREAD; r++) {
        int e = tid + 256 * r;
        as[(e / BM) * LDA_S + (e % BM)] = ra[r];
      }
#pragma unroll
      for (int r = 0; r < B_PER_THREAD; r++) {
        int e = tid + 256 * r;
        if (TRANSB) bs[(e / BN) * LDB_S + (e % BN)] = rb[r];
        else bs[(e % BK) * LDB_S + (e / BK)] = rb[r];
      }
    };
    if (nst > 0) { load(kbeg); store(0); }
    __syncthreads();
    int buf = 0;
    long long k0 = kbeg;
    for (long long st = 0; st + 1 < nst; st++) {
      k0 += BK;
      load(k0);
      compute(buf);
      store(buf ^ 1);
      __syncthreads();
      buf ^= 1;
    }
    if (nst > 0) compute(buf);
  }
  double* Pz = P + (long long)blockIdx.z * pstride;
#pragma unroll
  for (int a = 0; a < MT; a++)
#pragma unroll
    for (int b = 0; b < NT; b++)
#pragma unroll
      for (int r = 0; r < 4; r++) {
        int gi = i0 + wm + a * 16 + l15;
        long long gj = j0 + wn + b * 16 + l4 + 4 * r;
        if (gi < m && gj < n) Pz[gi + gj * ldp] = acc[a][b][r];
      }
  if (clk && threadIdx.x == 0) {
    const long long w1 = hssk_wallclock();
    if (blockIdx.x == 0 && blockIdx.y == 0 && blockIdx.z == 0) {
      clk[0] = hssk_clock() - t0_;
      clk[1] = w1 - w0_;
    }
    const long long fid = blockIdx.x + (long long)gridDim.x * (blockIdx.y + (long long)gridDim.y * blockIdx.z);
    long long* rec = clk + 4 + 4 * fid;
    rec[0] = w0_; rec[1] = w1; rec[2] = hssk_hwid(); rec[3] = bx;
  }
}

template <int MBLK, bool TRANSB, int TAG = 0, bool GEN = false>
__global__ __launch_bounds__(512, 2) void sketch_kernel(long long n, long long k, const double* __restrict__ A, long long lda,
                                                        const double* __restrict__ B, long long ldb,
                                                        double* __restrict__ P, long long ldp, long long pstride,
                                                        long long kchunk, int jtile0, long long* __restrict__ clk,
                                                        hssk_gen gen, long long jg0) {
  const long long t0_ = clk ? hssk_clock() : 0, w0_ = clk ? hssk_wallclock() : 0;
  constexpr int BM = 64 * MBLK, BN2 = 128;
  constexpr int WM = BM / 2, MT = WM / 16, NT = 2;
  constexpr int A_DBL = BM * BK, B_DBL = BN2 * BK, SLOT = A_DBL + B_DBL;
  constexpr int NCH = GEN ? MBLK : MBLK + 2;
  constexpr bool KJ_IMAGE = TRANSB && !GEN;
  HSSK_DYN_SHARED(double, lds);

  const int tid = threadIdx.x, lane = tid & 63, wave = hssk_uniform(tid >> 6);
  const int l15 = lane & 15, l4 = lane >> 4;
  int bx = blockIdx.x;
  {
    const int nx = gridDim.x, x = bx & 7, q = nx >> 3, r = nx & 7;
    bx = x * q + (x < r ? x : r) + (bx >> 3);
  }
  const long long j0 = (long long)(bx + jtile0) * BN2;
  const int i0 = blockIdx.y * BM;
  const long long kbeg = (long long)blockIdx.z * kchunk;
  const long long kend = kbeg + kchunk < k ? kbeg + kchunk : k;
  const int nst = (int)((kend - kbeg) / BK);
  const int wm = (wave & 1) * WM, wn = (wave >> 1) * 32;

  const int kk = lane >> 5, pos = 2 * (lane & 31);
  const double* srcA = A + i0 + (pos ^ (16 * kk)) + (kbeg + 2 * wave + kk) * lda;
  const long long stepA = (long long)BK * lda;
  const double* srcB[2] = {nullptr, nullptr};
  long long stepB = 0;
  if (GEN) {
  } else if (TRANSB) {
    const long long jp = j0 + (pos ^ (16 * kk));
    srcB[0] = B + (jp < n - 2 ? jp : n - 2) + (kbeg + 2 * wave + kk) * ldb;
    srcB[1] = B + (jp + 64 < n - 2 ? jp + 64 : n - 2) + (kbeg + 2 * wave + kk) * ldb;
    stepB = (long long)BK * ldb;
  } else {
#pragma unroll
    for (int r = 0; r < 2; r++) {
      const int j = 8 * (wave + 8 * r) + (lane >> 3), q = lane & 7;
      const long long jc = j0 + j < n - 1 ? j0 + j : n - 1;
      srcB[r] = B + jc * ldb + kbeg + 2 * (q ^ ((j >> 1) & 7));
    }
    stepB = BK;
  }
  auto copy_one = [&](int stage, int slot, int c) {
    const int sc = stage < nst ? stage : nst - 1;
    double* base = lds + slot * SLOT;
    if (c < MBLK) hssk_glds16(srcA + sc * stepA + 64 * c, base + c * 1024 + wave * 128);
    else if (GEN) {}
    else if (TRANSB) hssk_glds16(srcB[c - MBLK] + sc * stepB, base + A_DBL + (c - MBLK) * 1024 + wave * 128);
    else hssk_glds16(srcB[c - MBLK] + sc * stepB, base + A_DBL + (wave + 8 * (c - MBLK)) * 128);
  };
  const int gen_dfirst = (int)kbeg - ((int)(jg0 + j0) + 127);
  auto gen_tau = [&](int i) {
    const int d = gen_dfirst + i;
    return TRANSB ? hssk_gen_eval(gen, 0, d) : hssk_gen_eval(gen, d, 0);
  };
  auto copy_stage = [&](int stage, int slot) {
#pragma unroll
    for (int c = 0; c < NCH; c++) copy_one(stage, slot, c);
  };

  int offA[MT], offB[NT][4];
#pragma unroll
  for (int a = 0; a < MT; a++) {
    const int il = wm + a * 16 + l15;
    offA[a] = hssk_opaque((il >> 6) * 1024 + ((l4 & 1) + 8 * (l4 >> 1)) * 64 + ((il & 63) ^ (16 * (l4 & 1))));
  }
#pragma unroll
  for (int b = 0; b < NT; b++) {
    const int jl = wn + b * 16 + l15;
    if (GEN) {
      const int o = hssk_opaque(A_DBL + (l4 & 1) + 8 * (l4 >> 1) + 127 - jl);
#pragma unroll
      for (int s = 0; s < 4; s++) offB[b][s] = o + 2 * s;
    } else if (KJ_IMAGE) {
      const int o = hssk_opaque(A_DBL + (jl >> 6) * 1024 + ((l4 & 1) + 8 * (l4 >> 1)) * 64 + ((jl & 63) ^ (16 * (l4 & 1))));
#pragma unroll
      for (int s = 0; s < 4; s++) offB[b][s] = o + s * 128;
    } else {
      const int h = (jl >> 1) & 7;
#pragma unroll
      for (int s = 0; s < 4; s++) offB[b][s] = hssk_opaque(A_DBL + jl * 16 + 2 * ((s + 4 * (l4 >> 1)) ^ h) + (l4 & 1));
    }
  }

  hssk_d4 acc[MT][NT];
#pragma unroll
  for (int a = 0; a < MT; a++)
#pragma unroll
    for (int b = 0; b < NT; b++) acc[a][b] = hssk_d4{0., 0., 0., 0.};
  double af[2][MT], bf[2][NT];
  auto frags = [&](int slot, int s, int set) {
    const double* base = lds + slot * SLOT;
#pragma unroll
    for (int a = 0; a < MT; a++) af[set][a] = base[offA[a] + s * 128];
#pragma unroll
    for (int b = 0; b < NT; b++) bf[set][b] = base[offB[b][s]];
  };
  auto mfmas = [&](int set) {
#pragma unroll
    for (int a = 0; a < MT; a++)
#pragma unroll
      for (int b = 0; b < NT; b++)
        acc[a][b] = hssk_mfma_f64_16x16x4(bf[set][b], af[set][a], acc[a][b]);
  };
  auto stage = [&](int st, auto slot_tag) {
    constexpr int S = decltype(slot_tag)::value;
    double gen_moved = 0.;
    if (GEN && wave < 2 && tid < 127) gen_moved = lds[((S + 1) % 3) * SLOT + A_DBL + tid + 16];
    frags(S, 1, 1);
    hssk_sched_barrier();
    mfmas(0);
    hssk_sched_barrier();
    if (GEN && wave < 2 && tid < 127) lds[((S + 2) % 3) * SLOT + A_DBL + tid] = gen_moved;
    if (GEN && wave == 2 + (st & 1)) lds[((S + 2) % 3) * SLOT + A_DBL + 127 + l15] = gen_tau(16 * (st + 2) + 127 + l15);
    hssk_sched_barrier();
    frags(S, 2, 0);
    hssk_sched_barrier();
    mfmas(1);
    hssk_sched_barrier();
    frags(S, 3, 1);
    hssk_sched_barrier();
    mfmas(0);
    hssk_sched_barrier();
    hssk_wait_glds<NCH>();
    hssk_wg_barrier();
    hssk_sched_barrier();
#pragma unroll
    for (int a = 0; a < MT; a++) {
#pragma unroll
      for (int b = 0; b < NT; b++) acc[a][b] = hssk_mfma_f64_16x16x4(bf[1][b], af[1][a], acc[a][b]);
      hssk_sched_barrier();
      if (a == 0) frags((S + 1) % 3, 0, 0);
      else if (a - 1 < NCH) copy_one(st + 3, S, a - 1);
      hssk_sched_barrier();
    }
#pragma unroll
    for (int c = MT - 1; c < NCH; c++) copy_one(st + 3, S, c);
    hssk_sched_barrier();
  };

  if (nst > 0) {
    copy_stage(0, 0);
    copy_stage(1, 1);
    copy_stage(2, 2);
    if (GEN && tid < 143) {
      lds[A_DBL + tid] = gen_tau(tid);
      lds[SLOT + A_DBL + tid] = gen_tau(16 + tid);
    }
    hssk_wait_glds<2 * NCH>();
    hssk_wg_barrier();
    frags(0, 0, 0);
    int st = 0;
    for (; st + 3 <= nst; st += 3) {
      stage(st, std::integral_constant<int, 0>());
      stage(st + 1, std::integral_constant<int, 1>());
      stage(st + 2, std::integral_constant<int, 2>());
    }
    if (st < nst) stage(st, std::integral_constant<int, 0>());
    if (st + 1 < nst) stage(st + 1, std::integral_constant<int, 1>());
    hssk_wait_glds<0>();
  }
  double* Pz = P + (long long)blockIdx.z * pstride;
#pragma unroll
  for (int a = 0; a < MT; a++)
#pragma unroll
    for (int b = 0; b < NT; b++)
#pragma unroll
      for (int r = 0; r < 4; r++) {
        const int gi = i0 + wm + a * 16 + l15;
        const long long gj = j0 + wn + b * 16 + l4 + 4 * r;
        Pz[gi + gj * ldp] = acc[a][b][r];
      }
  if (clk && threadIdx.x == 0) {
    const long long w1 = hssk_wallclock();
    if (blockIdx.x == 0 && blockIdx.y == 0 && blockIdx.z == 0) {
      clk[0] = hssk_clock() - t0_;
      clk[1] = w1 - w0_;
    }
    const long long fid = blockIdx.x + (long long)gridDim.x * (blockIdx.y + (long long)gridDim.y * blockIdx.z);
    long long* rec = clk + 4 + 4 * fid;
    rec[0] = w0_; rec[1] = w1; rec[2] = hssk_hwid(); rec[3] = bx;
  }
}

__global__ void dgemm_reduce_kernel(int m, long long n, const double* __restrict__ P, long long ldp,
                                    long long pstride, int nz, double alpha, double beta,
                                    double* __restrict__ C, long long ldc) {
  long long total = (long long)m * n;
  for (long long e = (long long)blockIdx.x * blockDim.x + threadIdx.x; e < total;
       e += (long long)gridDim.x * blockDim.x) {
    int i = (int)(e % m);
    long long j = e / m;
    double s = 0.;
    for (int z = 0; z < nz; z++) s += P[i + j * ldp + z * pstride];
    double* c = C + i + j * ldc;
    double v = alpha * s;
    if (beta != 0.) v += beta * (*c);
    *c = v;
  }
}

__global__ void dgemm_reduce_wide_kernel(int m, long long n, const double* __restrict__ P, long long ldp,
                                         long long pstride, int nz, double alpha, double beta,
                                         double* __restrict__ C, long long ldc) {
  HSSK_SHARED double s_part[256];
  const int el = threadIdx.x & 15, zl = threadIdx.x >> 4;
  const long long total = (long long)m * n;
  for (long long e0 = (long long)blockIdx.x * 16; e0 < total; e0 += (long long)gridDim.x * 16) {
    const long long e = e0 + el;
    const int i = (int)(e % m);
    const long long j = e / m;
    double s = 0.;
    if (e < total) {
      const double* p = P + i + j * ldp;
      for (int z = zl; z < nz; z += 16) s += p[z * pstride];
    }
    s_part[threadIdx.x] = s;
    __syncthreads();
    if (zl == 0 && e < total) {
      double t = 0.;
      for (int q = 0; q < 16; q++) t += s_part[el + 16 * q];
      double* c = C + i + j * ldc;
      double v = alpha * t;
      if (beta != 0.) v += beta * (*c);
      *c = v;
    }
    __syncthreads();
  }
}

template <int BM, bool FULL, int TAG>
void launch_dgemm(hssk_ctx* ctx, int transB, dim3 grid, int m, long long n, long long k, const double* A,
                  long long lda, const double* B, long long ldb, double* P, long long ldp, long long pstride,
                  long long kchunk, int jtile0, long long* clk) {
  if (grid.x == 0) return;
  if (transB)
    HSSK_LAUNCH((dgemm_kernel<BM, true, FULL, TAG>), grid, dim3(256), 0, ctx->stream, m, n, k, A, lda, B, ldb, P, ldp, pstride, kchunk, jtile0, clk);
  else
    HSSK_LAUNCH((dgemm_kernel<BM, false, FULL, TAG>), grid, dim3(256), 0, ctx->stream, m, n, k, A, lda, B, ldb, P, ldp, pstride, kchunk, jtile0, clk);
}

}

namespace {
template <bool FULL, int TAG>
void launch_bm(int BM, hssk_ctx* ctx, int transB, dim3 grid, int m, long long n, long long k, const double* A,
               long long lda, const double* B, long long ldb, double* P, long long ldp, long long pstride,
               long long kchunk, int jtile0, long long* clk) {
  if (BM == 192) launch_dgemm<192, FULL, TAG>(ctx, transB, grid, m, n, k, A, lda, B, ldb, P, ldp, pstride, kchunk, jtile0, clk);
  else if (BM == 128) launch_dgemm<128, FULL, TAG>(ctx, transB, grid, m, n, k, A, lda, B, ldb, P, ldp, pstride, kchunk, jtile0, clk);
  else launch_dgemm<64, FULL, TAG>(ctx, transB, grid, m, n, k, A, lda, B, ldb, P, ldp, pstride, kchunk, jtile0, clk);
}

constexpr int BN2 = 128;
inline size_t sketch_lds_bytes(int mblk) { return sizeof(double) * 3 * (size_t)(64 * mblk + BN2) * BK; }
template <int MBLK, int TAG>
void launch_sketch_m(hssk_ctx* ctx, int transB, dim3 grid, long long n, long long k, const double* A, long long lda,
                     const double* B, long long ldb, double* P, long long ldp, long long pstride, long long kchunk,
                     int jtile0, long long* clk, const hssk_gen* gen, long long jg0) {
  const size_t shm = sketch_lds_bytes(MBLK);
  const hssk_gen g0{0, 0, {0., 0., 0., 0.}};
  if (gen) {
    if (transB) HSSK_LAUNCH((sketch_kernel<MBLK, true, TAG, true>), grid, dim3(512), shm, ctx->stream, n, k, A, lda, B, ldb, P, ldp, pstride, kchunk, jtile0, clk, *gen, jg0);
    else HSSK_LAUNCH((sketch_kernel<MBLK, false, TAG, true>), grid, dim3(512), shm, ctx->stream, n, k, A, lda, B, ldb, P, ldp, pstride, kchunk, jtile0, clk, *gen, jg0);
  } else {
    if (transB) HSSK_LAUNCH((sketch_kernel<MBLK, true, TAG, false>), grid, dim3(512), shm, ctx->stream, n, k, A, lda, B, ldb, P, ldp, pstride, kchunk, jtile0, clk, g0, jg0);
    else HSSK_LAUNCH((sketch_kernel<MBLK, false, TAG, false>), grid, dim3(512), shm, ctx->stream, n, k, A, lda, B, ldb, P, ldp, pstride, kchunk, jtile0, clk, g0, jg0);
  }
}
template <int MBLK>
bool sketch_prepare_m() {
  static const bool ok = [] {
    try {
      const size_t b = sketch_lds_bytes(MBLK);
      if (b > hssk_rt::max_lds_per_workgroup()) return false;
      hssk_rt::allow_dynamic_lds(sketch_kernel<MBLK, true, 0, false>, b);
      hssk_rt::allow_dynamic_lds(sketch_kernel<MBLK, false, 0, false>, b);
      hssk_rt::allow_dynamic_lds(sketch_kernel<MBLK, true, 1, false>, b);
      hssk_rt::allow_dynamic_lds(sketch_kernel<MBLK, false, 1, false>, b);
      hssk_rt::allow_dynamic_lds(sketch_kernel<MBLK, true, 0, true>, b);
      hssk_rt::allow_dynamic_lds(sketch_kernel<MBLK, false, 0, true>, b);
      hssk_rt::allow_dynamic_lds(sketch_kernel<MBLK, true, 1, true>, b);
      hssk_rt::allow_dynamic_lds(sketch_kernel<MBLK, false, 1, true>, b);
      return true;
    } catch (const std::exception&) {
      return false;
    }
  }();
  return ok;
}
inline bool sketch_prepare(int BM) {
  return BM == 192 ? sketch_prepare_m<3>() : (BM == 128 ? sketch_prepare_m<2>() : sketch_prepare_m<1>());
}
template <int TAG>
void launch_sketch(int BM, hssk_ctx* ctx, int transB, dim3 grid, long long n, long long k, const double* A, long long lda,
                   const double* B, long long ldb, double* P, long long ldp, long long pstride, long long kchunk,
                   int jtile0, long long* clk, const hssk_gen* gen, long long jg0) {
  if (grid.x == 0) return;
  if (BM == 192) launch_sketch_m<3, TAG>(ctx, transB, grid, n, k, A, lda, B, ldb, P, ldp, pstride, kchunk, jtile0, clk, gen, jg0);
  else if (BM == 128) launch_sketch_m<2, TAG>(ctx, transB, grid, n, k, A, lda, B, ldb, P, ldp, pstride, kchunk, jtile0, clk, gen, jg0);
  else launch_sketch_m<1, TAG>(ctx, transB, grid, n, k, A, lda, B, ldb, P, ldp, pstride, kchunk, jtile0, clk, gen, jg0);
}
}

static void dgemm_impl(hssk_ctx* ctx, int transB, int m, long long n, long long k, double alpha, const double* A, long long lda,
                       const double* B, long long ldb, const hssk_gen* gen, long long jg0, double beta, double* C, long long ldc) {
  if (m <= 0 || n <= 0) return;
  const int BM = m > 128 ? 192 : (m > 64 ? 128 : 64);
  const unsigned gm = (unsigned)((m + BM - 1) / BM);
  const long long ksteps = (k + BK - 1) / BK;
  const bool aligned = (m % BM == 0) && (k % BK == 0) && (lda % 2 == 0) && (gen || ldb % 2 == 0) &&
                       (((size_t)A | (gen ? (size_t)0 : (size_t)B)) % 16 == 0);
  static const int cus = hssk_rt::cu_count();
  const bool force_v1 = [] { const char* e = std::getenv("HSSK_DGEMM_V1"); return e && std::atoi(e) != 0; }();
  const bool v2 = aligned && (gen || !force_v1) && k > 0 && n >= BN2 && sketch_prepare(BM);
  if (gen && !v2) {
    const long long nb_max = std::max<long long>(64, std::min<long long>(1024, (long long)(size_t(1) << 28) / std::max<long long>(k, 1)));
    const long long ldg = k + (k & 1);
    for (long long c0 = 0; c0 < n; c0 += nb_max) {
      const long long nb = std::min(nb_max, n - c0);
      double* G = ctx->gen_block(sizeof(double) * (size_t)ldg * nb);
      if (hssk_gen_fill(ctx, gen, G, k, nb, ldg, 0, jg0 + c0, transB)) throw std::runtime_error(hssk_last_error());
      dgemm_impl(ctx, 0, m, nb, k, alpha, A, lda, G, ldg, nullptr, 0, beta, C + c0 * ldc, ldc);
    }
    return;
  }
  const int BNt = v2 ? BN2 : BN;
  static const bool no_fold = [] { const char* e = std::getenv("HSSK_DGEMM_NO_FOLD"); return e && std::atoi(e) != 0; }();
  const bool fold_edge = v2 && !no_fold && n % BNt != 0 && n % 2 == 0;
  const unsigned gn_full = aligned ? (unsigned)(n / BNt) + (fold_edge ? 1u : 0u) : 0u;
  const long long edge_col0 = std::min<long long>(n, (long long)gn_full * BNt);
  const unsigned gn_edge = (unsigned)((n - edge_col0 + BN - 1) / BN);
  const long long slots = v2 ? cus : 2LL * cus;
  struct Group { long long col0 = 0, ntiles = 0; int split = 1; long long kchunk = BK; int nz = 0; double* P = nullptr; long long cols = 0, vcols = 0; };
  auto chunk_of = [&](int split) {
    long long c = ((ksteps + split - 1) / split) * BK;
    return c > 0 ? c : (long long)BK;
  };
  auto max_split = [&]() { return (int)std::max<long long>(1, std::min<long long>(256, ksteps / 24)); };
  auto one_round_split = [&](long long tiles) {
    if (tiles <= 0 || k <= 0) return 1;
    return (int)std::max<long long>(1, std::min<long long>(max_split(), slots / tiles));
  };
  Group gmain, gtail, gedge;
  if (gn_full) {
    const long long T = (long long)gm * gn_full;
    const double epi = 3.0, red = 0.0067 * (BNt / BN);
    double best = 1e300;
    int best_s = 1;
    long long best_main = T;
    const int sp_min = (int)std::min<long long>(std::min(max_split(), 64), (ksteps + 1023) / 1024);
    for (int sp = std::max(1, sp_min); sp <= std::min(max_split(), 64); sp++) {
      const long long r = (T * sp) / slots;
      long long tm = r > 0 ? std::min<long long>(T, (r * slots) / sp) : 0;
      if (gm > 1) tm = T;
      const long long tt = T - tm;
      double cost = 0.;
      if (tm) cost += (double)((tm * sp + slots - 1) / slots) * ((double)(ksteps + sp - 1) / sp + epi) + red * sp * (double)tm;
      if (tt) {
        const int st = one_round_split(tt);
        cost += (double)((tt * st + slots - 1) / slots) * ((double)(ksteps + st - 1) / st + epi) + red * st * (double)tt + 2.0;
      }
      if (cost < best - 1e-9) { best = cost; best_s = sp; best_main = tm; }
    }
    if (k <= 0) { best_s = 1; best_main = T; }
    if (const char* e = std::getenv("HSSK_DGEMM_SPLIT")) {
      const int sp = std::max(1, std::min(max_split(), std::atoi(e)));
      const long long r = (T * sp) / slots;
      best_s = sp;
      best_main = (gm > 1 || r == 0) ? T : std::min<long long>(T, (r * slots) / sp);
    }
    gmain.col0 = 0; gmain.ntiles = gm > 1 ? gn_full : best_main; gmain.split = best_s; gmain.cols = gmain.ntiles * BNt;
    gtail.col0 = gmain.cols; gtail.ntiles = gn_full - gmain.ntiles; gtail.split = one_round_split(gtail.ntiles); gtail.cols = gtail.ntiles * BNt;
  }
  gedge.col0 = edge_col0; gedge.ntiles = gn_edge; gedge.split = one_round_split((long long)gm * gn_edge); gedge.cols = n - edge_col0;
  const long long ldp = m;
  size_t ptot = 0;
  for (Group* g : {&gmain, &gtail, &gedge}) {
    if (!g->ntiles) continue;
    g->vcols = std::min(g->cols, n - g->col0);
    g->kchunk = chunk_of(g->split);
    g->nz = (int)std::max<long long>(1, (k + g->kchunk - 1) / g->kchunk);
    ptot += (size_t)ldp * g->cols * g->nz;
  }
  const size_t ntrace = gmain.ntiles ? (size_t)gmain.ntiles * gm * gmain.nz : 0;
  double* P = ctx->scratch(sizeof(double) * (ptot + 4 + 4 * ntrace));
  long long* clk = (long long*)(P + ptot);
  {
    double* q = P;
    for (Group* g : {&gmain, &gtail, &gedge}) {
      if (!g->ntiles) continue;
      g->P = q;
      q += (size_t)ldp * g->cols * g->nz;
    }
  }
  auto shifted = [&](const Group& g) { return g.P - g.col0 * ldp; };
  const Group* timed = gmain.ntiles ? &gmain : (gtail.ntiles ? &gtail : &gedge);
  auto bracket = [&](const Group* g, auto&& launch) {
    if (!g->ntiles) return;
    if (g == timed) hssk_rt::event_record(ctx->ev0, ctx->stream);
    launch();
    if (g == timed) hssk_rt::event_record(ctx->ev1, ctx->stream);
  };
  auto grid_of = [&](const Group& g) { return dim3((unsigned)g.ntiles, gm, (unsigned)g.nz); };
  if (gen && gedge.ntiles) {
    const long long ldg = k + (k & 1);
    double* G = ctx->gen_block(sizeof(double) * (size_t)ldg * gedge.cols);
    if (hssk_gen_fill(ctx, gen, G, k, gedge.cols, ldg, 0, jg0 + gedge.col0, transB)) throw std::runtime_error(hssk_last_error());
    const double* Gs = G - gedge.col0 * ldg;
    bracket(&gedge, [&] { launch_bm<false, 0>(BM, ctx, 0, grid_of(gedge), m, n, k, A, lda, Gs, ldg, shifted(gedge), ldp, ldp * gedge.cols, gedge.kchunk, (int)(gedge.col0 / BN), nullptr); });
  } else
  bracket(&gedge, [&] { launch_bm<false, 0>(BM, ctx, transB, grid_of(gedge), m, n, k, A, lda, B, ldb, shifted(gedge), ldp, ldp * gedge.cols, gedge.kchunk, (int)(gedge.col0 / BN), nullptr); });
  if (v2) {
    bracket(&gtail, [&] { launch_sketch<1>(BM, ctx, transB, grid_of(gtail), n, k, A, lda, B, ldb, shifted(gtail), ldp, ldp * gtail.cols, gtail.kchunk, (int)(gtail.col0 / BN2), nullptr, gen, jg0); });
    bracket(&gmain, [&] { launch_sketch<0>(BM, ctx, transB, grid_of(gmain), n, k, A, lda, B, ldb, shifted(gmain), ldp, ldp * gmain.cols, gmain.kchunk, (int)(gmain.col0 / BN2), clk, gen, jg0); });
  } else {
    bracket(&gtail, [&] { launch_bm<true, 1>(BM, ctx, transB, grid_of(gtail), m, n, k, A, lda, B, ldb, shifted(gtail), ldp, ldp * gtail.cols, gtail.kchunk, (int)(gtail.col0 / BN), nullptr); });
    bracket(&gmain, [&] { launch_bm<true, 0>(BM, ctx, transB, grid_of(gmain), m, n, k, A, lda, B, ldb, shifted(gmain), ldp, ldp * gmain.cols, gmain.kchunk, (int)(gmain.col0 / BN), clk); });
  }
  ctx->d_clk = gmain.ntiles ? clk : nullptr;
  ctx->dgemm_trace_wgs = (long long)ntrace;
  ctx->dgemm_timed = true;
  ctx->dgemm_timed_flops = 2.0 * (double)m * (double)timed->vcols * (double)k;
  for (const Group* g : {&gmain, &gtail, &gedge}) {
    if (!g->ntiles) continue;
    long long total = (long long)m * g->vcols;
    unsigned rb = (unsigned)std::min<long long>((total + 255) / 256, 4096);
    if (g->nz >= 32 && total <= 65536)
      HSSK_LAUNCH(dgemm_reduce_wide_kernel, dim3((unsigned)((total + 15) / 16)), dim3(256), 0, ctx->stream, m, g->vcols, (const double*)g->P, ldp, ldp * g->cols, g->nz, alpha, beta, C + g->col0 * ldc, ldc);
    else
      HSSK_LAUNCH(dgemm_reduce_kernel, dim3(rb), dim3(256), 0, ctx->stream, m, g->vcols, (const double*)g->P, ldp, ldp * g->cols, g->nz, alpha, beta, C + g->col0 * ldc, ldc);
  }
  hssk_rt::check_launch();
}

extern "C" int hssk_dgemm(hssk_ctx* ctx, int transB, int m, long long n, long long k, double alpha,
                          const double* A, long long lda, const double* B, long long ldb, double beta,
                          double* C, long long ldc) {
  HSSK_API_BEGIN
  dgemm_impl(ctx, transB, m, n, k, alpha, A, lda, B, ldb, nullptr, 0, beta, C, ldc);
  HSSK_API_END
}

extern "C" int hssk_sketch_gen(hssk_ctx* ctx, const hssk_gen* g, int transG, int m, long long n, long long k, long long j0,
                               double alpha, const double* A, long long lda, double beta, double* C, long long ldc) {
  HSSK_API_BEGIN
  if (!g || (g->kind != HSSK_GEN_TOEPLITZ && g->kind != HSSK_GEN_TOEPLITZ_UPPER)) throw std::invalid_argument("hssk_sketch_gen: unknown generator kind");
  if (k > 0x7fffffffLL || j0 + n > 0x7fffffffLL) throw std::invalid_argument("hssk_sketch_gen: indices beyond 2^31");
  dgemm_impl(ctx, transG, m, n, k, alpha, A, lda, nullptr, 0, g, j0, beta, C, ldc);
  HSSK_API_END
}
```

strumpack_amd/hssk.py:

```python
import ctypes as C

import numpy as np

c_dp = C.POINTER(C.c_double)
c_ip = C.POINTER(C.c_int)


class GemmDesc(C.Structure):
    _fields_ = [("A", C.c_void_p), ("B", C.c_void_p), ("C", C.c_void_p),
                ("m", C.c_int), ("n", C.c_int), ("k", C.c_int),
                ("lda", C.c_int), ("ldb", C.c_int), ("ldc", C.c_int),
                ("transA", C.c_int), ("transB", C.c_int),
                ("alpha", C.c_double), ("beta", C.c_double)]


class LeafUpdateDesc(C.Structure):
    _fields_ = [("R", C.c_void_p), ("D", C.c_void_p), ("Sr", C.c_void_p), ("Sc", C.c_void_p),
                ("d", C.c_int), ("m", C.c_int), ("ldr", C.c_int), ("ldd", C.c_int), ("lds", C.c_int)]


class KernelSpec(C.Structure):
    _fields_ = [("X", C.c_void_p), ("n", C.c_longlong), ("d", C.c_int), ("type", C.c_int), ("p", C.c_int),
                ("h", C.c_double), ("lam", C.c_double)]


class KevalDesc(C.Structure):
    _fields_ = [("ri", C.c_void_p), ("ci", C.c_void_p), ("out", C.c_void_p),
                ("nr", C.c_int), ("nc", C.c_int), ("ldo", C.c_int), ("r0", C.c_int), ("c0", C.c_int)]


class ColsetDesc(C.Structure):
    _fields_ = [("src0", C.c_void_p), ("src1", C.c_void_p), ("n0", C.c_int), ("n1", C.c_int), ("lo", C.c_int), ("hi", C.c_int),
                ("out", C.c_void_p), ("count", C.c_void_p), ("n0_dev", C.c_void_p), ("n1_dev", C.c_void_p)]


class ColGatherDesc(C.Structure):
    _fields_ = [("src", C.c_void_p), ("dst", C.c_void_p), ("idx", C.c_void_p),
                ("rows", C.c_int), ("ncols", C.c_int), ("lds", C.c_int), ("ldd", C.c_int),
                ("scatter", C.c_int)]


class RowGatherDesc(C.Structure):
    _fields_ = [("src", C.c_void_p), ("dst", C.c_void_p), ("idx", C.c_void_p),
                ("nrows", C.c_int), ("cols", C.c_int), ("lds", C.c_int), ("ldd", C.c_int),
                ("scatter", C.c_int), ("accumulate", C.c_int)]


class ElemDesc(C.Structure):
    _fields_ = [("A", C.c_void_p), ("lda", C.c_longlong), ("I", C.c_void_p), ("J", C.c_void_p),
                ("i0", C.c_int), ("j0", C.c_int), ("B", C.c_void_p),
                ("m", C.c_int), ("n", C.c_int), ("ldb", C.c_int), ("transpose", C.c_int),
                ("rlo", C.c_int), ("rhi", C.c_int), ("clo", C.c_int), ("chi", C.c_int)]


class TransposeDesc(C.Structure):
    _fields_ = [("src", C.c_void_p), ("dst", C.c_void_p),
                ("rows", C.c_int), ("cols", C.c_int), ("lds", C.c_int), ("ldd", C.c_int)]


class IdDesc(C.Structure):
    _fields_ = [("W", C.c_void_p), ("ldw", C.c_int), ("d", C.c_int), ("m", C.c_int),
                ("rtol", C.c_double), ("atol", C.c_double), ("max_rank", C.c_int),
                ("perm", C.c_void_p), ("rank", C.c_void_p), ("work", C.c_void_p),
                ("src", C.c_void_p), ("lds", C.c_int), ("defer_x", C.c_int)]


class CombineDesc(C.Structure):
    _fields_ = [("G0", C.c_void_p), ("G1", C.c_void_p), ("ldg", C.c_int), ("gsplit", C.c_int), ("gidx", C.c_void_p),
                ("M0", C.c_void_p), ("M1", C.c_void_p), ("ldm", C.c_int), ("msplit", C.c_int), ("midx", C.c_void_p),
                ("C", C.c_void_p), ("csj", C.c_int), ("csk", C.c_int), ("alpha", C.c_double),
                ("out", C.c_void_p), ("ldo", C.c_int), ("rows", C.c_int), ("J", C.c_int), ("K", C.c_int)]


class UlvSplitDesc(C.Structure):
    _fields_ = [("D", C.c_void_p), ("ldd", C.c_int), ("m", C.c_int), ("r", C.c_int), ("perm", C.c_void_p),
                ("X", C.c_void_p), ("ldx", C.c_int), ("W1", C.c_void_p), ("ldw", C.c_int), ("W0t", C.c_void_p), ("ldt", C.c_int)]


class TpqrDesc(C.Structure):
    _fields_ = [("R1", C.c_void_p), ("ld1", C.c_int), ("R2", C.c_void_p), ("ld2", C.c_int), ("m", C.c_int)]


class XsolveDesc(C.Structure):
    _fields_ = [("W", C.c_void_p), ("ldw", C.c_int), ("rank", C.c_int), ("m", C.c_int),
                ("X", C.c_void_p), ("ldx", C.c_int), ("solved", C.c_int)]


class PcholDesc(C.Structure):
    _fields_ = [("G", C.c_void_p), ("ldg", C.c_int), ("m", C.c_int), ("rtol", C.c_double), ("atol", C.c_double),
                ("max_rank", C.c_int), ("perm", C.c_void_p), ("rank", C.c_void_p), ("R", C.c_void_p), ("ldr", C.c_int)]


class SumDesc(C.Structure):
    _fields_ = [("P", C.c_void_p), ("stride", C.c_longlong), ("n", C.c_longlong), ("count", C.c_int), ("out", C.c_void_p)]


class GramDesc(C.Structure):
    _fields_ = [("W", C.c_void_p), ("ldw", C.c_int), ("rows", C.c_int), ("m", C.c_int), ("G", C.c_void_p), ("ldg", C.c_int)]


class GramGenDesc(C.Structure):
    _fields_ = [("ri", C.c_void_p), ("r0", C.c_int), ("ci", C.c_void_p), ("c0", C.c_int), ("rows", C.c_int), ("m", C.c_int),
                ("G", C.c_void_p), ("ldg", C.c_int)]


class QrDesc(C.Structure):
    _fields_ = [("A", C.c_void_p), ("lda", C.c_int), ("rows", C.c_int), ("cols", C.c_int),
                ("Q", C.c_void_p), ("ldq", C.c_int), ("nq", C.c_int),
                ("rdiag", C.c_void_p), ("work", C.c_void_p), ("stair", C.c_int),
                ("stop_rel", C.c_double), ("stop_abs", C.c_double), ("r_only", C.c_int)]


class TrsmDesc(C.Structure):
    _fields_ = [("T", C.c_void_p), ("B", C.c_void_p), ("n", C.c_int), ("nrhs", C.c_int),
                ("ldt", C.c_int), ("ldb", C.c_int), ("lower", C.c_int), ("transT", C.c_int),
                ("unit", C.c_int), ("Tinv", C.c_void_p)]


class TrtriDesc(C.Structure):
    _fields_ = [("R", C.c_void_p), ("Tinv", C.c_void_p), ("n", C.c_int), ("ldr", C.c_int), ("mode", C.c_int)]


class LuDesc(C.Structure):
    _fields_ = [("A", C.c_void_p), ("n", C.c_int), ("lda", C.c_int), ("piv", C.c_void_p),
                ("info", C.c_void_p)]


class LuSolveDesc(C.Structure):
    _fields_ = [("LU", C.c_void_p), ("piv", C.c_void_p), ("B", C.c_void_p),
                ("n", C.c_int), ("nrhs", C.c_int), ("lda", C.c_int), ("ldb", C.c_int)]


class NormDesc(C.Structure):
    _fields_ = [("P", C.c_void_p), ("rows", C.c_int), ("cols", C.c_int), ("ld", C.c_int),
                ("out", C.c_void_p)]


class ShiftDesc(C.Structure):
    _fields_ = [("A", C.c_void_p), ("n", C.c_int), ("lda", C.c_int)]


class Gen(C.Structure):
    _fields_ = [("kind", C.c_int), ("reserved", C.c_int), ("p", C.c_double * 4)]


HSSK_SYMBOLS = [
    "hssk_ctx_create", "hssk_ctx_destroy", "hssk_ctx_stream", "hssk_sync", "hssk_last_error",
    "hssk_malloc", "hssk_free", "hssk_memcpy_h2d", "hssk_memcpy_d2h", "hssk_last_dgemm_ms", "hssk_last_dgemm_flops", "hssk_last_dgemm_trace",
    "hssk_fill_toeplitz", "hssk_randn", "hssk_dgemm", "hssk_gemm_vbatched", "hssk_gather_cols",
    "hssk_gather_rows", "hssk_gather_elems", "hssk_transpose", "hssk_id_vbatched",
    "hssk_qr_vbatched", "hssk_trsm_vbatched", "hssk_getrf_vbatched", "hssk_getrs_vbatched",
    "hssk_sumsq_vbatched", "hssk_shift_diag", "hssk_mfma_f64_peak_tflops", "hssk_memcpy_d2d",
    "hssk_memcpy2d_h2d", "hssk_memcpy2d_d2h", "hssk_memset_zero", "hssk_is_device_pointer",
    "hssk_basis_dense", "hssk_mfma_f64_probe", "hssk_last_dgemm_clock_ghz", "hssk_leaf_update_vbatched", "hssk_formq_vbatched",
    "hssk_kernel_eval_vbatched", "hssk_knn", "hssk_kernel_predict", "hssk_copy_triu",
    "hssk_laswp_vbatched", "hssk_shift_diag_cplx", "hssk_upload_async", "hssk_h2d_block_async", "hssk_h2d_bytes_async", "hssk_expand_image", "hssk_copy_fence", "hssk_compute_fence", "hssk_compute_mark", "hssk_copy_wait", "hssk_id_xsolve_vbatched", "hssk_id_solves_inline", "hssk_gather_combine", "hssk_ulv_split", "hssk_tpqr_vbatched", "hssk_fill_toeplitz_block", "hssk_sum_slabs", "hssk_ulv_fwd_sweep", "hssk_ulv_bwd_sweep", "hssk_apply_sweep", "hssk_sweep_status", "hssk_sweep_arm", "hssk_trtri_diag_vbatched", "hssk_sjlt_dense", "hssk_sjlt_sketch",
    "hssk_plan_begin", "hssk_plan_end", "hssk_plan_replay", "hssk_plan_destroy", "hssk_plan_size",
    "hssk_sketch_gen", "hssk_gen_elems", "hssk_gen_fill", "hssk_colsets", "hssk_colsets_max_universe",
    "hssk_cluster_median", "hssk_pchol_id_vbatched", "hssk_pchol_id_max_m", "hssk_pchol_id_rank_cap", "hssk_sum_partials", "hssk_gram_vbatched", "hssk_gram_gen_vbatched", "hssk_gram_gen_supported",
    "hssk_sgemm_sketch", "hssk_narrow_f32", "hssk_gather_elems_f32",
]


class DevArray:

    def __init__(self, hk, shape, dtype=np.float64):
        self.hk, self.shape, self.dtype = hk, tuple(shape), np.dtype(dtype)
        self.nbytes = int(np.prod(self.shape)) * self.dtype.itemsize
        self.ptr = hk.lib.hssk_malloc(max(self.nbytes, 8))
        if not self.ptr:
            raise MemoryError(hk.error())

    def free(self):
        if self.ptr:
            self.hk.lib.hssk_free(self.ptr)
            self.ptr = None

    def __del__(self):
        try:
            self.free()
        except Exception:
            pass

    def get(self):
        out = np.empty(self.shape, dtype=self.dtype, order="F")
        if self.nbytes:
            self.hk.check(self.hk.lib.hssk_memcpy_d2h(self.hk.ctx, out.ctypes.data, self.ptr, self.nbytes))
        return out

    def set(self, arr):
        a = np.asfortranarray(arr, dtype=self.dtype)
        assert a.shape == self.shape
        if self.nbytes:
            self.hk.check(self.hk.lib.hssk_memcpy_h2d(self.hk.ctx, self.ptr, a.ctypes.data, self.nbytes))
        return self

    def at(self, *idx):
        off, stride = 0, 1
        for i, n in zip(idx, self.shape):
            off += i * stride
            stride *= n
        return self.ptr + off * self.dtype.itemsize


class Hssk:
    def __init__(self, path, device=0):
        self.lib = L = C.CDLL(path)
        L.hssk_malloc.restype = C.c_void_p
        L.hssk_malloc.argtypes = [C.c_longlong]
        L.hssk_free.argtypes = [C.c_void_p]
        L.hssk_last_error.restype = C.c_char_p
        L.hssk_ctx_create.argtypes = [C.POINTER(C.c_void_p), C.c_int]
        L.hssk_ctx_destroy.argtypes = [C.c_void_p]
        L.hssk_ctx_stream.restype = C.c_void_p
        L.hssk_ctx_stream.argtypes = [C.c_void_p]
        L.hssk_sync.argtypes = [C.c_void_p]
        L.hssk_memcpy_h2d.argtypes = [C.c_void_p, C.c_void_p, C.c_void_p, C.c_longlong]
        L.hssk_memcpy_d2h.argtypes = [C.c_void_p, C.c_void_p, C.c_void_p, C.c_longlong]
        L.hssk_memcpy_d2d.argtypes = [C.c_void_p, C.c_void_p, C.c_void_p, C.c_longlong]
        L.hssk_memset_zero.argtypes = [C.c_void_p, C.c_void_p, C.c_longlong]
        for f in ("hssk_memcpy2d_h2d", "hssk_memcpy2d_d2h"):
            getattr(L, f).argtypes = [C.c_void_p, C.c_void_p, C.c_longlong, C.c_void_p, C.c_longlong,
                                      C.c_longlong, C.c_longlong]
        L.hssk_is_device_pointer.argtypes = [C.c_void_p]
        L.hssk_last_dgemm_clock_ghz.restype = C.c_double
        L.hssk_last_dgemm_clock_ghz.argtypes = [C.c_void_p]
        L.hssk_last_dgemm_ms.restype = C.c_float
        L.hssk_last_dgemm_ms.argtypes = [C.c_void_p]
        L.hssk_last_dgemm_trace.restype = C.c_longlong
        L.hssk_last_dgemm_trace.argtypes = [C.c_void_p, C.c_void_p, C.c_longlong]
        L.hssk_last_dgemm_flops.restype = C.c_double
        L.hssk_last_dgemm_flops.argtypes = [C.c_void_p]
        L.hssk_fill_toeplitz.argtypes = [C.c_void_p, C.c_void_p, C.c_int, C.c_longlong, C.c_char]
        L.hssk_fill_toeplitz_block.argtypes = [C.c_void_p, C.c_void_p, C.c_int, C.c_int, C.c_longlong, C.c_int, C.c_int, C.c_char]
        L.hssk_sum_slabs.argtypes = [C.c_void_p, C.c_void_p, C.c_longlong, C.c_longlong, C.c_int, C.c_void_p]
        L.hssk_upload_async.argtypes = [C.c_void_p, C.c_void_p, C.c_void_p, C.c_longlong]
        L.hssk_h2d_block_async.argtypes = [C.c_void_p, C.c_void_p, C.c_longlong, C.c_void_p, C.c_longlong, C.c_longlong, C.c_longlong]
        L.hssk_copy_fence.argtypes = [C.c_void_p]
        L.hssk_compute_fence.argtypes = [C.c_void_p]
        L.hssk_h2d_bytes_async.argtypes = [C.c_void_p, C.c_void_p, C.c_longlong, C.c_void_p, C.c_longlong, C.c_longlong, C.c_longlong]
        L.hssk_expand_image.argtypes = [C.c_void_p, C.c_void_p, C.c_longlong, C.c_void_p, C.c_longlong, C.c_longlong, C.c_longlong, C.c_int]
        L.hssk_compute_mark.argtypes = [C.c_void_p, C.c_int]
        L.hssk_copy_wait.argtypes = [C.c_void_p, C.c_int]
        L.hssk_sweep_status.argtypes = [C.c_void_p]
        L.hssk_randn.argtypes = [C.c_void_p, C.c_void_p, C.c_int, C.c_longlong, C.c_longlong,
                                 C.c_int, C.c_longlong, C.c_ulonglong]
        L.hssk_dgemm.argtypes = [C.c_void_p, C.c_int, C.c_int, C.c_longlong, C.c_longlong,
                                 C.c_double, C.c_void_p, C.c_longlong, C.c_void_p, C.c_longlong,
                                 C.c_double, C.c_void_p, C.c_longlong]
        L.hssk_sgemm_sketch.argtypes = [C.c_void_p, C.c_int, C.c_int, C.c_longlong, C.c_longlong,
                                        C.c_double, C.c_void_p, C.c_longlong, C.c_void_p, C.c_longlong,
                                        C.c_double, C.c_void_p, C.c_longlong]
        L.hssk_narrow_f32.argtypes = [C.c_void_p, C.c_void_p, C.c_longlong, C.c_void_p, C.c_longlong, C.c_longlong, C.c_longlong]
        for name in ("hssk_gemm_vbatched", "hssk_gather_cols", "hssk_gather_rows",
                     "hssk_gather_elems", "hssk_gather_elems_f32", "hssk_transpose", "hssk_id_vbatched", "hssk_qr_vbatched",
                     "hssk_trsm_vbatched", "hssk_getrf_vbatched", "hssk_getrs_vbatched",
                     "hssk_sumsq_vbatched", "hssk_leaf_update_vbatched", "hssk_formq_vbatched",
                     "hssk_id_xsolve_vbatched", "hssk_gather_combine", "hssk_ulv_split", "hssk_tpqr_vbatched"):
            getattr(L, name).argtypes = [C.c_void_p, C.c_void_p, C.c_int]
        L.hssk_sketch_gen.argtypes = [C.c_void_p, C.c_void_p, C.c_int, C.c_int, C.c_longlong, C.c_longlong, C.c_longlong,
                                      C.c_double, C.c_void_p, C.c_longlong, C.c_double, C.c_void_p, C.c_longlong]
        L.hssk_gen_elems.argtypes = [C.c_void_p, C.c_void_p, C.c_void_p, C.c_int]
        L.hssk_gen_fill.argtypes = [C.c_void_p, C.c_void_p, C.c_void_p, C.c_longlong, C.c_longlong, C.c_longlong, C.c_longlong,
                                    C.c_longlong, C.c_int]
        L.hssk_id_solves_inline.argtypes = [C.c_int, C.c_int]
        L.hssk_shift_diag.argtypes = [C.c_void_p, C.c_void_p, C.c_int, C.c_double]
        L.hssk_kernel_eval_vbatched.argtypes = [C.c_void_p, C.c_void_p, C.c_void_p, C.c_int]
        L.hssk_knn.argtypes = [C.c_void_p, C.c_void_p, C.c_int, C.c_int, C.c_int, C.c_int, C.c_int, C.c_void_p]
        L.hssk_kernel_predict.argtypes = [C.c_void_p, C.c_void_p, C.c_void_p, C.c_void_p, C.c_int, C.c_void_p]
        L.hssk_colsets.argtypes = [C.c_void_p, C.c_void_p, C.c_int, C.c_int]
        L.hssk_cluster_median.argtypes = [C.c_void_p, C.c_void_p, C.c_int, C.c_int, C.c_int, C.c_int, C.c_void_p, C.c_void_p]
        for fn in ("hssk_pchol_id_vbatched", "hssk_sum_partials", "hssk_gram_vbatched"):
            getattr(L, fn).argtypes = [C.c_void_p, C.c_void_p, C.c_int]
        L.hssk_pchol_id_rank_cap.argtypes = [C.c_int]
        L.hssk_gram_gen_vbatched.argtypes = [C.c_void_p, C.c_void_p, C.c_void_p, C.c_int]
        L.hssk_gram_gen_supported.argtypes = [C.c_void_p, C.c_int]
        L.hssk_colsets_max_universe.argtypes = []
        L.hssk_colsets_max_universe.restype = C.c_longlong
        L.hssk_sjlt_dense.argtypes = [C.c_void_p, C.c_void_p, C.c_int, C.c_longlong, C.c_longlong, C.c_void_p, C.c_int]
        L.hssk_sjlt_sketch.argtypes = [C.c_void_p, C.c_int, C.c_longlong, C.c_longlong, C.c_void_p, C.c_longlong,
                                       C.c_void_p, C.c_int, C.c_int, C.c_void_p, C.c_longlong]
        L.hssk_mfma_f64_peak_tflops.restype = C.c_double
        L.hssk_mfma_f64_peak_tflops.argtypes = [C.c_void_p, C.c_int]
        L.hssk_mfma_f64_probe.argtypes = [C.c_void_p, C.c_int, C.c_int, C.c_int, C.POINTER(C.c_double)]
        ctx = C.c_void_p()
        if L.hssk_ctx_create(C.byref(ctx), device):
            raise RuntimeError(self.error())
        self.ctx = ctx

    def error(self):
        return self.lib.hssk_last_error().decode()

    def check(self, rc):
        if rc:
            raise RuntimeError(self.error())

    def close(self):
        if self.ctx:
            self.lib.hssk_ctx_destroy(self.ctx)
            self.ctx = None

    def sync(self):
        self.check(self.lib.hssk_sync(self.ctx))

    def empty(self, shape, dtype=np.float64):
        return DevArray(self, shape, dtype)

    def array(self, arr, dtype=None):
        a = np.asarray(arr)
        d = DevArray(self, a.shape, dtype or a.dtype)
        return d.set(a)

    def batch(self, fn_name, descs):
        if not descs:
            return
        arr = (type(descs[0]) * len(descs))(*descs)
        self.check(getattr(self.lib, fn_name)(self.ctx, arr, len(descs)))
```

Before: 69890.

## Fuse row and column sketch GEMMs into one persistent ticket-scheduled launch

Adds hssk_dgemm_pair, which breaks the two sketch products (A^T R and A R) into tiles and runs them from a single persistent kernel, where workgroups take tiles through an atomic ticket counter. All partial-sum reductions are then folded in one kernel. The aim is to cut launch count and the tail idle time between the two separate GEMM passes, and to balance load across CUs. The path is on by default for single-rank runs and also drops a host sync after random-matrix generation in some configs, so correctness now depends on stream ordering.

```diff
diff --git a/include/hssk.h b/include/hssk.h
--- a/include/hssk.h
+++ b/include/hssk.h
@@ -89,6 +89,18 @@
 } hssk_gen;
 int hssk_sketch_gen(hssk_ctx* ctx, const hssk_gen* g, int transG, int m, long long n, long long k, long long j0, double alpha,
                     const double* A, long long lda, double beta, double* C, long long ldc);
+typedef struct hssk_dgemm_job {
+  int transB, reserved;
+  long long n, k;
+  const double* B;
+  long long ldb;
+  const hssk_gen* gen;
+  long long j0;
+  double* C;
+  long long ldc;
+} hssk_dgemm_job;
+int hssk_dgemm_pair(hssk_ctx* ctx, int m, double alpha, const double* A, long long lda, double beta,
+                    const hssk_dgemm_job* jobs, int count);
 int hssk_gen_fill(hssk_ctx* ctx, const hssk_gen* g, double* A, long long rows, long long cols, long long lda, long long i0,
                   long long j0, int trans);
 
diff --git a/strumpack_amd/csrc/host/hss_compress.cpp b/strumpack_amd/csrc/host/hss_compress.cpp
--- a/strumpack_amd/csrc/host/hss_compress.cpp
+++ b/strumpack_amd/csrc/host/hss_compress.cpp
@@ -169,7 +169,7 @@
       ck(hssk_memcpy2d_h2d(ctx_, Rt_ + r0, sizeof(double) * dcap_, buf.data(), sizeof(double) * dn, sizeof(double) * dn, N));
     }
   }
-  ck(hssk_sync(ctx_));
+  if (o_.sketch == 1 || o_.random_engine != 2) ck(hssk_sync(ctx_));
   stats_.t_random += now() - t0;
 }
 
diff --git a/strumpack_amd/csrc/host/hss_sources.cpp b/strumpack_amd/csrc/host/hss_sources.cpp
--- a/strumpack_amd/csrc/host/hss_sources.cpp
+++ b/strumpack_amd/csrc/host/hss_sources.cpp
@@ -2,6 +2,11 @@
 
 namespace strumpack {
 namespace HSS {
+
+static bool sketch_pair_enabled() {
+  const char* e = std::getenv("HSSK_SKETCH_PAIR");
+  return !e || std::atoi(e) != 0;
+}
 
 double DeviceHSS::Source::sketch_flops(const DeviceHSS& H, int dn) const {
   return 2.0 * products(H) * (double)H.n_ * (double)H.n_ * (H.sj_pat_ ? H.sj_nnz_ : dn);
@@ -46,12 +51,16 @@
         }
       }
     } else if (nloc > 0) {
-      ck(hssk_dgemm(H.ctx_, 1, dn, nloc, N, 1.0, H.Rt_ + r0, H.dcap_, dA + j0, lda, 0.0, H.Srt_ + r0 + j0 * H.dcap_, H.dcap_));
+      const bool pair = H.o_.world == 1 && sketch_pair_enabled();
+      hssk_dgemm_job jobs[2] = {{1, 0, nloc, N, dA + j0, lda, nullptr, 0, H.Srt_ + r0 + j0 * H.dcap_, H.dcap_},
+                                {0, 0, nloc, N, dA + j0 * lda, lda, nullptr, 0, H.Sct_ + r0 + j0 * H.dcap_, H.dcap_}};
+      if (pair) ck(hssk_dgemm_pair(H.ctx_, dn, 1.0, H.Rt_ + r0, H.dcap_, 0.0, jobs, H.o_.symmetric ? 1 : 2));
+      else ck(hssk_dgemm(H.ctx_, 1, dn, nloc, N, 1.0, H.Rt_ + r0, H.dcap_, dA + j0, lda, 0.0, H.Srt_ + r0 + j0 * H.dcap_, H.dcap_));
       ck(hssk_dgemm_timing_defer(H.ctx_));
       if (H.o_.symmetric) {
         hssk_colgather_desc cp{H.Srt_ + r0 + j0 * H.dcap_, H.Sct_ + r0 + j0 * H.dcap_, nullptr, dn, (int)nloc, H.dcap_, H.dcap_, 0};
         ck(hssk_gather_cols(H.ctx_, &cp, 1));
-      } else {
+      } else if (!pair) {
         ck(hssk_dgemm(H.ctx_, 0, dn, nloc, N, 1.0, H.Rt_ + r0, H.dcap_, dA + j0 * lda, lda, 0.0, H.Sct_ + r0 + j0 * H.dcap_, H.dcap_));
         ck(hssk_dgemm_timing_defer(H.ctx_));
       }
@@ -437,12 +446,16 @@
     const long long nloc = j1 - j0;
     auto timed = [&] { ck(hssk_dgemm_timing_defer(H.ctx_)); };
     if (nloc > 0) {
-      ck(hssk_sketch_gen(H.ctx_, &g, 1, dn, nloc, N, j0, 1.0, H.Rt_ + r0, H.dcap_, 0.0, H.Srt_ + r0 + j0 * H.dcap_, H.dcap_));
+      const bool pair = H.o_.world == 1 && sketch_pair_enabled();
+      hssk_dgemm_job jobs[2] = {{1, 0, nloc, N, nullptr, 0, &g, j0, H.Srt_ + r0 + j0 * H.dcap_, H.dcap_},
+                                {0, 0, nloc, N, nullptr, 0, &g, j0, H.Sct_ + r0 + j0 * H.dcap_, H.dcap_}};
+      if (pair) ck(hssk_dgemm_pair(H.ctx_, dn, 1.0, H.Rt_ + r0, H.dcap_, 0.0, jobs, H.o_.symmetric ? 1 : 2));
+      else ck(hssk_sketch_gen(H.ctx_, &g, 1, dn, nloc, N, j0, 1.0, H.Rt_ + r0, H.dcap_, 0.0, H.Srt_ + r0 + j0 * H.dcap_, H.dcap_));
       timed();
       if (H.o_.symmetric) {
         hssk_colgather_desc cp{H.Srt_ + r0 + j0 * H.dcap_, H.Sct_ + r0 + j0 * H.dcap_, nullptr, dn, (int)nloc, H.dcap_, H.dcap_, 0};
         ck(hssk_gather_cols(H.ctx_, &cp, 1));
-      } else {
+      } else if (!pair) {
         ck(hssk_sketch_gen(H.ctx_, &g, 0, dn, nloc, N, j0, 1.0, H.Rt_ + r0, H.dcap_, 0.0, H.Sct_ + r0 + j0 * H.dcap_, H.dcap_));
         timed();
       }
diff --git a/strumpack_amd/csrc/kernels/hssk_dgemm.hip b/strumpack_amd/csrc/kernels/hssk_dgemm.hip
--- a/strumpack_amd/csrc/kernels/hssk_dgemm.hip
+++ b/strumpack_amd/csrc/kernels/hssk_dgemm.hip
@@ -210,30 +210,20 @@
   }
 }
 
-template <int MBLK, bool TRANSB, int TAG = 0, bool GEN = false>
-__global__ __launch_bounds__(512, 2) void sketch_kernel(long long n, long long k, const double* __restrict__ A, long long lda,
-                                                        const double* __restrict__ B, long long ldb,
-                                                        double* __restrict__ P, long long ldp, long long pstride,
-                                                        long long kchunk, int jtile0, long long* __restrict__ clk,
-                                                        hssk_gen gen, long long jg0) {
-  const long long t0_ = clk ? hssk_clock() : 0, w0_ = clk ? hssk_wallclock() : 0;
+template <int MBLK, bool TRANSB, bool GEN>
+__device__ __forceinline__ void sketch_tile(double* lds, long long n, long long k, const double* __restrict__ A, long long lda,
+                                            const double* __restrict__ B, long long ldb, double* __restrict__ Pz, long long ldp,
+                                            long long kchunk, int z, int tile, int i0, const hssk_gen& gen, long long jg0) {
   constexpr int BM = 64 * MBLK, BN2 = 128;
   constexpr int WM = BM / 2, MT = WM / 16, NT = 2;
   constexpr int A_DBL = BM * BK, B_DBL = BN2 * BK, SLOT = A_DBL + B_DBL;
   constexpr int NCH = GEN ? MBLK : MBLK + 2;
   constexpr bool KJ_IMAGE = TRANSB && !GEN;
-  HSSK_DYN_SHARED(double, lds);
 
   const int tid = threadIdx.x, lane = tid & 63, wave = hssk_uniform(tid >> 6);
   const int l15 = lane & 15, l4 = lane >> 4;
-  int bx = blockIdx.x;
-  {
-    const int nx = gridDim.x, x = bx & 7, q = nx >> 3, r = nx & 7;
-    bx = x * q + (x < r ? x : r) + (bx >> 3);
-  }
-  const long long j0 = (long long)(bx + jtile0) * BN2;
-  const int i0 = blockIdx.y * BM;
-  const long long kbeg = (long long)blockIdx.z * kchunk;
+  const long long j0 = (long long)tile * BN2;
+  const long long kbeg = (long long)z * kchunk;
   const long long kend = kbeg + kchunk < k ? kbeg + kchunk : k;
   const int nst = (int)((kend - kbeg) / BK);
   const int wm = (wave & 1) * WM, wn = (wave >> 1) * 32;
@@ -377,7 +367,6 @@
     if (st + 1 < nst) stage(st + 1, std::integral_constant<int, 1>());
     hssk_wait_glds<0>();
   }
-  double* Pz = P + (long long)blockIdx.z * pstride;
 #pragma unroll
   for (int a = 0; a < MT; a++)
 #pragma unroll
@@ -388,6 +377,24 @@
         const long long gj = j0 + wn + b * 16 + l4 + 4 * r;
         Pz[gi + gj * ldp] = acc[a][b][r];
       }
+}
+
+__device__ __forceinline__ int xcd_tile(int id, int nx) {
+  const int x = id & 7, q = nx >> 3, r = nx & 7;
+  return x * q + (x < r ? x : r) + (id >> 3);
+}
+
+template <int MBLK, bool TRANSB, int TAG = 0, bool GEN = false>
+__global__ __launch_bounds__(512, 2) void sketch_kernel(long long n, long long k, const double* __restrict__ A, long long lda,
+                                                        const double* __restrict__ B, long long ldb,
+                                                        double* __restrict__ P, long long ldp, long long pstride,
+                                                        long long kchunk, int jtile0, long long* __restrict__ clk,
+                                                        hssk_gen gen, long long jg0) {
+  const long long t0_ = clk ? hssk_clock() : 0, w0_ = clk ? hssk_wallclock() : 0;
+  HSSK_DYN_SHARED(double, lds);
+  const int bx = xcd_tile(blockIdx.x, gridDim.x);
+  sketch_tile<MBLK, TRANSB, GEN>(lds, n, k, A, lda, B, ldb, P + (long long)blockIdx.z * pstride, ldp, kchunk, blockIdx.z, bx + jtile0,
+                                 blockIdx.y * (64 * MBLK), gen, jg0);
   if (clk && threadIdx.x == 0) {
     const long long w1 = hssk_wallclock();
     if (blockIdx.x == 0 && blockIdx.y == 0 && blockIdx.z == 0) {
@@ -400,12 +407,61 @@
   }
 }
 
-__global__ void dgemm_reduce_kernel(int m, long long n, const double* __restrict__ P, long long ldp,
-                                    long long pstride, int nz, double alpha, double beta,
-                                    double* __restrict__ C, long long ldc) {
+struct SketchGroup {
+  const double* B;
+  double* P;
+  long long ldb, n, k, pstride, kchunk, jg0;
+  int ntiles, nz, jtile0, transB;
+  int first;
+  int tag;
+};
+struct SketchWork {
+  SketchGroup g[4];
+  int ngroups, nitems;
+};
+
+namespace ticket {
+template <int MBLK, bool TRANSB, int TAG, bool GEN>
+__global__ __launch_bounds__(512, 2) void sketch_kernel(SketchWork w, const double* __restrict__ A, long long lda, long long ldp,
+                                                        int* __restrict__ ticket, long long* __restrict__ clk, hssk_gen gen) {
+  HSSK_DYN_SHARED(double, lds);
+  HSSK_SHARED int s_item[4];
+  for (;;) {
+    const long long t0_ = hssk_clock();
+    __syncthreads();
+    if (threadIdx.x == 0) s_item[0] = hssk_gadd_i(ticket, 1);
+    __syncthreads();
+    const int item = hssk_uniform(s_item[0]);
+    if (item >= w.nitems) break;
+    const long long w0_ = hssk_wallclock();
+    int gi = 0;
+#pragma unroll
+    for (int q = 1; q < 4; q++)
+      if (q < w.ngroups && item >= w.g[q].first) gi = q;
+    const SketchGroup& g = w.g[gi];
+    const int l = item - g.first, z = l / g.ntiles;
+    const int bx = xcd_tile(l - z * g.ntiles, g.ntiles);
+    if (TRANSB && g.transB)
+      sketch_tile<MBLK, true, GEN>(lds, g.n, g.k, A, lda, g.B, g.ldb, g.P + (long long)z * g.pstride, ldp, g.kchunk, z, bx + g.jtile0, 0, gen, g.jg0);
+    else
+      sketch_tile<MBLK, false, GEN>(lds, g.n, g.k, A, lda, g.B, g.ldb, g.P + (long long)z * g.pstride, ldp, g.kchunk, z, bx + g.jtile0, 0, gen, g.jg0);
+    if (threadIdx.x == 0) {
+      const long long w1 = hssk_wallclock();
+      if (item == 0) {
+        clk[0] = hssk_clock() - t0_;
+        clk[1] = w1 - w0_;
+      }
+      long long* rec = clk + 4 + 4 * (long long)item;
+      rec[0] = w0_; rec[1] = w1; rec[2] = hssk_hwid(); rec[3] = (long long)bx | ((long long)g.tag << 32);
+    }
+  }
+}
+}
+
+__device__ __forceinline__ void reduce_body(int m, long long n, const double* __restrict__ P, long long ldp, long long pstride, int nz,
+                                            double alpha, double beta, double* __restrict__ C, long long ldc, long long bid, long long nb) {
   long long total = (long long)m * n;
-  for (long long e = (long long)blockIdx.x * blockDim.x + threadIdx.x; e < total;
-       e += (long long)gridDim.x * blockDim.x) {
+  for (long long e = bid * blockDim.x + threadIdx.x; e < total; e += nb * blockDim.x) {
     int i = (int)(e % m);
     long long j = e / m;
     double s = 0.;
@@ -416,14 +472,18 @@
     *c = v;
   }
 }
-
-__global__ void dgemm_reduce_wide_kernel(int m, long long n, const double* __restrict__ P, long long ldp,
-                                         long long pstride, int nz, double alpha, double beta,
-                                         double* __restrict__ C, long long ldc) {
-  HSSK_SHARED double s_part[256];
+__global__ void dgemm_reduce_kernel(int m, long long n, const double* __restrict__ P, long long ldp,
+                                    long long pstride, int nz, double alpha, double beta,
+                                    double* __restrict__ C, long long ldc) {
+  reduce_body(m, n, P, ldp, pstride, nz, alpha, beta, C, ldc, blockIdx.x, gridDim.x);
+}
+
+__device__ __forceinline__ void reduce_wide_body(double* s_part, int m, long long n, const double* __restrict__ P, long long ldp,
+                                                 long long pstride, int nz, double alpha, double beta, double* __restrict__ C,
+                                                 long long ldc, long long bid, long long nb) {
   const int el = threadIdx.x & 15, zl = threadIdx.x >> 4;
   const long long total = (long long)m * n;
-  for (long long e0 = (long long)blockIdx.x * 16; e0 < total; e0 += (long long)gridDim.x * 16) {
+  for (long long e0 = bid * 16; e0 < total; e0 += nb * 16) {
     const long long e = e0 + el;
     const int i = (int)(e % m);
     const long long j = e / m;
@@ -444,6 +504,33 @@
     }
     __syncthreads();
   }
+}
+__global__ void dgemm_reduce_wide_kernel(int m, long long n, const double* __restrict__ P, long long ldp,
+                                         long long pstride, int nz, double alpha, double beta,
+                                         double* __restrict__ C, long long ldc) {
+  HSSK_SHARED double s_part[256];
+  reduce_wide_body(s_part, m, n, P, ldp, pstride, nz, alpha, beta, C, ldc, blockIdx.x, gridDim.x);
+}
+
+struct FoldGroup {
+  const double* P;
+  double* C;
+  long long vcols, pstride, ldc;
+  int nz, wide;
+  unsigned block0, nblocks;
+};
+struct FoldWork {
+  FoldGroup g[6];
+  int ngroups;
+};
+__global__ void dgemm_fold_kernel(FoldWork w, int m, long long ldp, double alpha, double beta) {
+  HSSK_SHARED double s_part[256];
+  FoldGroup g = w.g[0];
+#pragma unroll
+  for (int q = 1; q < 6; q++)
+    if (q < w.ngroups && blockIdx.x >= w.g[q].block0) g = w.g[q];
+  if (g.wide) reduce_wide_body(s_part, m, g.vcols, g.P, ldp, g.pstride, g.nz, alpha, beta, g.C, g.ldc, blockIdx.x - g.block0, g.nblocks);
+  else reduce_body(m, g.vcols, g.P, ldp, g.pstride, g.nz, alpha, beta, g.C, g.ldc, blockIdx.x - g.block0, g.nblocks);
 }
 
 template <int BM, bool FULL, int TAG>
@@ -499,6 +586,10 @@
       hssk_rt::allow_dynamic_lds(sketch_kernel<MBLK, false, 0, true>, b);
       hssk_rt::allow_dynamic_lds(sketch_kernel<MBLK, true, 1, true>, b);
       hssk_rt::allow_dynamic_lds(sketch_kernel<MBLK, false, 1, true>, b);
+      hssk_rt::allow_dynamic_lds(ticket::sketch_kernel<MBLK, true, 0, false>, b);
+      hssk_rt::allow_dynamic_lds(ticket::sketch_kernel<MBLK, false, 0, false>, b);
+      hssk_rt::allow_dynamic_lds(ticket::sketch_kernel<MBLK, true, 0, true>, b);
+      hssk_rt::allow_dynamic_lds(ticket::sketch_kernel<MBLK, false, 0, true>, b);
       return true;
     } catch (const std::exception&) {
       return false;
@@ -518,30 +609,60 @@
   else if (BM == 128) launch_sketch_m<2, TAG>(ctx, transB, grid, n, k, A, lda, B, ldb, P, ldp, pstride, kchunk, jtile0, clk, gen, jg0);
   else launch_sketch_m<1, TAG>(ctx, transB, grid, n, k, A, lda, B, ldb, P, ldp, pstride, kchunk, jtile0, clk, gen, jg0);
 }
-}
-
-static void dgemm_impl(hssk_ctx* ctx, int transB, int m, long long n, long long k, double alpha, const double* A, long long lda,
-                       const double* B, long long ldb, const hssk_gen* gen, long long jg0, double beta, double* C, long long ldc) {
-  if (m <= 0 || n <= 0) return;
-  const int BM = m > 128 ? 192 : (m > 64 ? 128 : 64);
-  const unsigned gm = (unsigned)((m + BM - 1) / BM);
+template <int MBLK>
+void launch_ticket_m(hssk_ctx* ctx, bool both, unsigned wgs, const SketchWork& w, const double* A, long long lda, long long ldp,
+                     int* ticket, long long* clk, const hssk_gen* gen) {
+  const size_t shm = sketch_lds_bytes(MBLK);
+  const hssk_gen g0{0, 0, {0., 0., 0., 0.}};
+  if (gen) {
+    if (both) HSSK_LAUNCH((ticket::sketch_kernel<MBLK, true, 0, true>), dim3(wgs), dim3(512), shm, ctx->stream, w, A, lda, ldp, ticket, clk, *gen);
+    else HSSK_LAUNCH((ticket::sketch_kernel<MBLK, false, 0, true>), dim3(wgs), dim3(512), shm, ctx->stream, w, A, lda, ldp, ticket, clk, *gen);
+  } else {
+    if (both) HSSK_LAUNCH((ticket::sketch_kernel<MBLK, true, 0, false>), dim3(wgs), dim3(512), shm, ctx->stream, w, A, lda, ldp, ticket, clk, g0);
+    else HSSK_LAUNCH((ticket::sketch_kernel<MBLK, false, 0, false>), dim3(wgs), dim3(512), shm, ctx->stream, w, A, lda, ldp, ticket, clk, g0);
+  }
+}
+inline void launch_ticket(int BM, hssk_ctx* ctx, bool both, unsigned wgs, const SketchWork& w, const double* A, long long lda,
+                          long long ldp, int* ticket, long long* clk, const hssk_gen* gen) {
+  if (BM == 192) launch_ticket_m<3>(ctx, both, wgs, w, A, lda, ldp, ticket, clk, gen);
+  else if (BM == 128) launch_ticket_m<2>(ctx, both, wgs, w, A, lda, ldp, ticket, clk, gen);
+  else launch_ticket_m<1>(ctx, both, wgs, w, A, lda, ldp, ticket, clk, gen);
+}
+}
+
+namespace {
+struct Group { long long col0 = 0, ntiles = 0; int split = 1; long long kchunk = BK; int nz = 0; double* P = nullptr; long long cols = 0, vcols = 0; };
+struct Decomp {
+  int BM = 64;
+  unsigned gm = 1;
+  bool v2 = false;
+  Group gmain, gtail, gedge;
+  long long ldp = 0;
+  size_t ptot = 0;
+  Group* groups(int i) { return i == 0 ? &gmain : (i == 1 ? &gtail : &gedge); }
+  double* place(double* P) {
+    for (int i = 0; i < 3; i++) {
+      Group* g = groups(i);
+      if (!g->ntiles) continue;
+      g->P = P;
+      P += (size_t)ldp * g->cols * g->nz;
+    }
+    return P;
+  }
+};
+inline double* shifted(const Group& g, long long ldp) { return g.P - g.col0 * ldp; }
+
+Decomp decompose(int m, long long n, long long k, const double* A, long long lda, const double* B, long long ldb, bool gen) {
+  Decomp d;
+  const int BM = d.BM = m > 128 ? 192 : (m > 64 ? 128 : 64);
+  const unsigned gm = d.gm = (unsigned)((m + BM - 1) / BM);
   const long long ksteps = (k + BK - 1) / BK;
   const bool aligned = (m % BM == 0) && (k % BK == 0) && (lda % 2 == 0) && (gen || ldb % 2 == 0) &&
                        (((size_t)A | (gen ? (size_t)0 : (size_t)B)) % 16 == 0);
   static const int cus = hssk_rt::cu_count();
   const bool force_v1 = [] { const char* e = std::getenv("HSSK_DGEMM_V1"); return e && std::atoi(e) != 0; }();
-  const bool v2 = aligned && (gen || !force_v1) && k > 0 && n >= BN2 && sketch_prepare(BM);
-  if (gen && !v2) {
-    const long long nb_max = std::max<long long>(64, std::min<long long>(1024, (long long)(size_t(1) << 28) / std::max<long long>(k, 1)));
-    const long long ldg = k + (k & 1);
-    for (long long c0 = 0; c0 < n; c0 += nb_max) {
-      const long long nb = std::min(nb_max, n - c0);
-      double* G = ctx->gen_block(sizeof(double) * (size_t)ldg * nb);
-      if (hssk_gen_fill(ctx, gen, G, k, nb, ldg, 0, jg0 + c0, transB)) throw std::runtime_error(hssk_last_error());
-      dgemm_impl(ctx, 0, m, nb, k, alpha, A, lda, G, ldg, nullptr, 0, beta, C + c0 * ldc, ldc);
-    }
-    return;
-  }
+  const bool v2 = d.v2 = aligned && (gen || !force_v1) && k > 0 && n >= BN2 && sketch_prepare(BM);
+  if (gen && !v2) return d;
   const int BNt = v2 ? BN2 : BN;
   static const bool no_fold = [] { const char* e = std::getenv("HSSK_DGEMM_NO_FOLD"); return e && std::atoi(e) != 0; }();
   const bool fold_edge = v2 && !no_fold && n % BNt != 0 && n % 2 == 0;
@@ -549,7 +670,6 @@
   const long long edge_col0 = std::min<long long>(n, (long long)gn_full * BNt);
   const unsigned gn_edge = (unsigned)((n - edge_col0 + BN - 1) / BN);
   const long long slots = v2 ? cus : 2LL * cus;
-  struct Group { long long col0 = 0, ntiles = 0; int split = 1; long long kchunk = BK; int nz = 0; double* P = nullptr; long long cols = 0, vcols = 0; };
   auto chunk_of = [&](int split) {
     long long c = ((ksteps + split - 1) / split) * BK;
     return c > 0 ? c : (long long)BK;
@@ -559,7 +679,7 @@
     if (tiles <= 0 || k <= 0) return 1;
     return (int)std::max<long long>(1, std::min<long long>(max_split(), slots / tiles));
   };
-  Group gmain, gtail, gedge;
+  Group &gmain = d.gmain, &gtail = d.gtail, &gedge = d.gedge;
   if (gn_full) {
     const long long T = (long long)gm * gn_full;
     const double epi = 3.0, red = 0.0067 * (BNt / BN);
@@ -591,7 +711,8 @@
     gtail.col0 = gmain.cols; gtail.ntiles = gn_full - gmain.ntiles; gtail.split = one_round_split(gtail.ntiles); gtail.cols = gtail.ntiles * BNt;
   }
   gedge.col0 = edge_col0; gedge.ntiles = gn_edge; gedge.split = one_round_split((long long)gm * gn_edge); gedge.cols = n - edge_col0;
-  const long long ldp = m;
+  d.ldp = m;
+  const long long ldp = d.ldp;
   size_t ptot = 0;
   for (Group* g : {&gmain, &gtail, &gedge}) {
     if (!g->ntiles) continue;
@@ -600,18 +721,54 @@
     g->nz = (int)std::max<long long>(1, (k + g->kchunk - 1) / g->kchunk);
     ptot += (size_t)ldp * g->cols * g->nz;
   }
+  d.ptot = ptot;
+  return d;
+}
+
+void launch_edge(hssk_ctx* ctx, const Decomp& d, int transB, int m, long long n, long long k, const double* A, long long lda,
+                 const double* B, long long ldb, const hssk_gen* gen, long long jg0) {
+  const Group& gedge = d.gedge;
+  if (!gedge.ntiles) return;
+  const dim3 grid((unsigned)gedge.ntiles, d.gm, (unsigned)gedge.nz);
+  if (gen) {
+    const long long ldg = k + (k & 1);
+    double* G = ctx->gen_block(sizeof(double) * (size_t)ldg * gedge.cols);
+    if (hssk_gen_fill(ctx, gen, G, k, gedge.cols, ldg, 0, jg0 + gedge.col0, transB)) throw std::runtime_error(hssk_last_error());
+    const double* Gs = G - gedge.col0 * ldg;
+    launch_bm<false, 0>(d.BM, ctx, 0, grid, m, n, k, A, lda, Gs, ldg, shifted(gedge, d.ldp), d.ldp, d.ldp * gedge.cols, gedge.kchunk, (int)(gedge.col0 / BN), nullptr);
+  } else
+    launch_bm<false, 0>(d.BM, ctx, transB, grid, m, n, k, A, lda, B, ldb, shifted(gedge, d.ldp), d.ldp, d.ldp * gedge.cols, gedge.kchunk, (int)(gedge.col0 / BN), nullptr);
+}
+}
+
+static void fold_shape(int m, const Group& g, bool* wide, unsigned* blocks) {
+  const long long total = (long long)m * g.vcols;
+  *wide = g.nz >= 32 && total <= 65536;
+  *blocks = *wide ? (unsigned)((total + 15) / 16) : (unsigned)std::min<long long>((total + 255) / 256, 4096);
+}
+
+static void dgemm_impl(hssk_ctx* ctx, int transB, int m, long long n, long long k, double alpha, const double* A, long long lda,
+                       const double* B, long long ldb, const hssk_gen* gen, long long jg0, double beta, double* C, long long ldc) {
+  if (m <= 0 || n <= 0) return;
+  Decomp d = decompose(m, n, k, A, lda, B, ldb, gen != nullptr);
+  const int BM = d.BM;
+  const unsigned gm = d.gm;
+  if (gen && !d.v2) {
+    const long long nb_max = std::max<long long>(64, std::min<long long>(1024, (long long)(size_t(1) << 28) / std::max<long long>(k, 1)));
+    const long long ldg = k + (k & 1);
+    for (long long c0 = 0; c0 < n; c0 += nb_max) {
+      const long long nb = std::min(nb_max, n - c0);
+      double* G = ctx->gen_block(sizeof(double) * (size_t)ldg * nb);
+      if (hssk_gen_fill(ctx, gen, G, k, nb, ldg, 0, jg0 + c0, transB)) throw std::runtime_error(hssk_last_error());
+      dgemm_impl(ctx, 0, m, nb, k, alpha, A, lda, G, ldg, nullptr, 0, beta, C + c0 * ldc, ldc);
+    }
+    return;
+  }
+  Group &gmain = d.gmain, &gtail = d.gtail, &gedge = d.gedge;
+  const long long ldp = d.ldp;
   const size_t ntrace = gmain.ntiles ? (size_t)gmain.ntiles * gm * gmain.nz : 0;
-  double* P = ctx->scratch(sizeof(double) * (ptot + 4 + 4 * ntrace));
-  long long* clk = (long long*)(P + ptot);
-  {
-    double* q = P;
-    for (Group* g : {&gmain, &gtail, &gedge}) {
-      if (!g->ntiles) continue;
-      g->P = q;
-      q += (size_t)ldp * g->cols * g->nz;
-    }
-  }
-  auto shifted = [&](const Group& g) { return g.P - g.col0 * ldp; };
+  double* P = ctx->scratch(sizeof(double) * (d.ptot + 4 + 4 * ntrace));
+  long long* clk = (long long*)d.place(P);
   const Group* timed = gmain.ntiles ? &gmain : (gtail.ntiles ? &gtail : &gedge);
   auto bracket = [&](const Group* g, auto&& launch) {
     if (!g->ntiles) return;
@@ -620,20 +777,13 @@
     if (g == timed) hssk_rt::event_record(ctx->ev1, ctx->stream);
   };
   auto grid_of = [&](const Group& g) { return dim3((unsigned)g.ntiles, gm, (unsigned)g.nz); };
-  if (gen && gedge.ntiles) {
-    const long long ldg = k + (k & 1);
-    double* G = ctx->gen_block(sizeof(double) * (size_t)ldg * gedge.cols);
-    if (hssk_gen_fill(ctx, gen, G, k, gedge.cols, ldg, 0, jg0 + gedge.col0, transB)) throw std::runtime_error(hssk_last_error());
-    const double* Gs = G - gedge.col0 * ldg;
-    bracket(&gedge, [&] { launch_bm<false, 0>(BM, ctx, 0, grid_of(gedge), m, n, k, A, lda, Gs, ldg, shifted(gedge), ldp, ldp * gedge.cols, gedge.kchunk, (int)(gedge.col0 / BN), nullptr); });
-  } else
-  bracket(&gedge, [&] { launch_bm<false, 0>(BM, ctx, transB, grid_of(gedge), m, n, k, A, lda, B, ldb, shifted(gedge), ldp, ldp * gedge.cols, gedge.kchunk, (int)(gedge.col0 / BN), nullptr); });
-  if (v2) {
-    bracket(&gtail, [&] { launch_sketch<1>(BM, ctx, transB, grid_of(gtail), n, k, A, lda, B, ldb, shifted(gtail), ldp, ldp * gtail.cols, gtail.kchunk, (int)(gtail.col0 / BN2), nullptr, gen, jg0); });
-    bracket(&gmain, [&] { launch_sketch<0>(BM, ctx, transB, grid_of(gmain), n, k, A, lda, B, ldb, shifted(gmain), ldp, ldp * gmain.cols, gmain.kchunk, (int)(gmain.col0 / BN2), clk, gen, jg0); });
+  bracket(&gedge, [&] { launch_edge(ctx, d, transB, m, n, k, A, lda, B, ldb, gen, jg0); });
+  if (d.v2) {
+    bracket(&gtail, [&] { launch_sketch<1>(BM, ctx, transB, grid_of(gtail), n, k, A, lda, B, ldb, shifted(gtail, ldp), ldp, ldp * gtail.cols, gtail.kchunk, (int)(gtail.col0 / BN2), nullptr, gen, jg0); });
+    bracket(&gmain, [&] { launch_sketch<0>(BM, ctx, transB, grid_of(gmain), n, k, A, lda, B, ldb, shifted(gmain, ldp), ldp, ldp * gmain.cols, gmain.kchunk, (int)(gmain.col0 / BN2), clk, gen, jg0); });
   } else {
-    bracket(&gtail, [&] { launch_bm<true, 1>(BM, ctx, transB, grid_of(gtail), m, n, k, A, lda, B, ldb, shifted(gtail), ldp, ldp * gtail.cols, gtail.kchunk, (int)(gtail.col0 / BN), nullptr); });
-    bracket(&gmain, [&] { launch_bm<true, 0>(BM, ctx, transB, grid_of(gmain), m, n, k, A, lda, B, ldb, shifted(gmain), ldp, ldp * gmain.cols, gmain.kchunk, (int)(gmain.col0 / BN), clk); });
+    bracket(&gtail, [&] { launch_bm<true, 1>(BM, ctx, transB, grid_of(gtail), m, n, k, A, lda, B, ldb, shifted(gtail, ldp), ldp, ldp * gtail.cols, gtail.kchunk, (int)(gtail.col0 / BN), nullptr); });
+    bracket(&gmain, [&] { launch_bm<true, 0>(BM, ctx, transB, grid_of(gmain), m, n, k, A, lda, B, ldb, shifted(gmain, ldp), ldp, ldp * gmain.cols, gmain.kchunk, (int)(gmain.col0 / BN), clk); });
   }
   ctx->d_clk = gmain.ntiles ? clk : nullptr;
   ctx->dgemm_trace_wgs = (long long)ntrace;
@@ -641,14 +791,111 @@
   ctx->dgemm_timed_flops = 2.0 * (double)m * (double)timed->vcols * (double)k;
   for (const Group* g : {&gmain, &gtail, &gedge}) {
     if (!g->ntiles) continue;
-    long long total = (long long)m * g->vcols;
-    unsigned rb = (unsigned)std::min<long long>((total + 255) / 256, 4096);
-    if (g->nz >= 32 && total <= 65536)
-      HSSK_LAUNCH(dgemm_reduce_wide_kernel, dim3((unsigned)((total + 15) / 16)), dim3(256), 0, ctx->stream, m, g->vcols, (const double*)g->P, ldp, ldp * g->cols, g->nz, alpha, beta, C + g->col0 * ldc, ldc);
+    bool wide;
+    unsigned blocks;
+    fold_shape(m, *g, &wide, &blocks);
+    if (wide)
+      HSSK_LAUNCH(dgemm_reduce_wide_kernel, dim3(blocks), dim3(256), 0, ctx->stream, m, g->vcols, (const double*)g->P, ldp, ldp * g->cols, g->nz, alpha, beta, C + g->col0 * ldc, ldc);
     else
-      HSSK_LAUNCH(dgemm_reduce_kernel, dim3(rb), dim3(256), 0, ctx->stream, m, g->vcols, (const double*)g->P, ldp, ldp * g->cols, g->nz, alpha, beta, C + g->col0 * ldc, ldc);
+      HSSK_LAUNCH(dgemm_reduce_kernel, dim3(blocks), dim3(256), 0, ctx->stream, m, g->vcols, (const double*)g->P, ldp, ldp * g->cols, g->nz, alpha, beta, C + g->col0 * ldc, ldc);
   }
   hssk_rt::check_launch();
+}
+
+static void dgemm_pair_impl(hssk_ctx* ctx, int m, double alpha, const double* A, long long lda, double beta,
+                            const hssk_dgemm_job* jobs, int count) {
+  if (count < 0 || count > 2) throw std::invalid_argument("hssk_dgemm_pair: one or two jobs");
+  Decomp d[2];
+  bool take[2] = {false, false};
+  int ntake = 0, first = -1;
+  const hssk_gen* gen = nullptr;
+  for (int j = 0; j < count; j++) {
+    const hssk_dgemm_job& J = jobs[j];
+    if (J.gen) {
+      if (J.gen->kind != HSSK_GEN_TOEPLITZ && J.gen->kind != HSSK_GEN_TOEPLITZ_UPPER) throw std::invalid_argument("hssk_dgemm_pair: unknown generator kind");
+      if (J.k > 0x7fffffffLL || J.j0 + J.n > 0x7fffffffLL) throw std::invalid_argument("hssk_dgemm_pair: indices beyond 2^31");
+    }
+    if (m <= 0 || J.n <= 0) continue;
+    d[j] = decompose(m, J.n, J.k, A, lda, J.B, J.ldb, J.gen != nullptr);
+    take[j] = d[j].v2 && d[j].gm == 1 && (d[j].gmain.ntiles || d[j].gtail.ntiles);
+    if (take[j] && ntake) {
+      const hssk_dgemm_job& J0 = jobs[first];
+      const bool same = (J.gen != nullptr) == (J0.gen != nullptr) && (!J.gen || std::memcmp(J.gen, J0.gen, sizeof(hssk_gen)) == 0);
+      if (!same) take[j] = false;
+    }
+    if (take[j]) { if (!ntake++) first = j; gen = J.gen; }
+    else {
+      dgemm_impl(ctx, J.transB, m, J.n, J.k, alpha, A, lda, J.B, J.ldb, J.gen, J.j0, beta, J.C, J.ldc);
+      bool more = ntake > 0;
+      for (int q = j + 1; q < count; q++) more = more || jobs[q].n > 0;
+      if (more && hssk_dgemm_timing_defer(ctx)) throw std::runtime_error(hssk_last_error());
+    }
+  }
+  if (!ntake) return;
+  const long long ldp = m;
+  size_t ptot = 0, nitems = 0;
+  for (int j = 0; j < count; j++)
+    if (take[j]) {
+      ptot += d[j].ptot;
+      nitems += (size_t)(d[j].gmain.ntiles * d[j].gmain.nz + d[j].gtail.ntiles * d[j].gtail.nz);
+    }
+  if (nitems > 0x7fffffffull) throw std::invalid_argument("hssk_dgemm_pair: too many items");
+  double* P = ctx->scratch(sizeof(double) * (ptot + 4 + 4 * nitems));
+  {
+    double* q = P;
+    for (int j = 0; j < count; j++)
+      if (take[j]) q = d[j].place(q);
+  }
+  long long* clk = (long long*)(P + ptot);
+  int* ticket = (int*)(clk + 2);
+  for (int j = 0; j < count; j++)
+    if (take[j]) launch_edge(ctx, d[j], jobs[j].transB, m, jobs[j].n, jobs[j].k, A, lda, jobs[j].B, jobs[j].ldb, jobs[j].gen, jobs[j].j0);
+  SketchWork w{};
+  FoldWork f{};
+  bool both = false;
+  double flops = 0.;
+  unsigned fblocks = 0;
+  for (int kind = 0; kind < 3; kind++)
+    for (int j = 0; j < count; j++) {
+      if (!take[j]) continue;
+      const Group& g = *d[j].groups(kind);
+      if (!g.ntiles) continue;
+      const hssk_dgemm_job& J = jobs[j];
+      if (kind < 2) {
+        SketchGroup& s = w.g[w.ngroups++];
+        s.B = J.B; s.P = shifted(g, ldp);
+        s.ldb = J.ldb; s.n = J.n; s.k = J.k; s.pstride = ldp * g.cols; s.kchunk = g.kchunk; s.jg0 = J.j0;
+        s.ntiles = (int)g.ntiles; s.nz = g.nz; s.jtile0 = (int)(g.col0 / BN2); s.transB = J.transB ? 1 : 0;
+        s.first = w.nitems; s.tag = kind | (j << 8);
+        w.nitems += (int)(g.ntiles * g.nz);
+        both = both || J.transB;
+        flops += 2.0 * (double)m * (double)g.vcols * (double)J.k;
+      }
+      FoldGroup& r = f.g[f.ngroups++];
+      bool wide;
+      fold_shape(m, g, &wide, &r.nblocks);
+      r.P = g.P; r.C = J.C + g.col0 * J.ldc; r.vcols = g.vcols; r.pstride = ldp * g.cols; r.ldc = J.ldc; r.nz = g.nz; r.wide = wide ? 1 : 0;
+      r.block0 = fblocks;
+      fblocks += r.nblocks;
+    }
+  static const int cus = hssk_rt::cu_count();
+  hssk_rt::memset_async(ticket, 0, sizeof(long long), ctx->stream);
+  hssk_rt::event_record(ctx->ev0, ctx->stream);
+  launch_ticket(d[first].BM, ctx, both, (unsigned)std::min<long long>(cus, w.nitems), w, A, lda, ldp, ticket, clk, gen);
+  hssk_rt::event_record(ctx->ev1, ctx->stream);
+  ctx->d_clk = clk;
+  ctx->dgemm_trace_wgs = w.nitems;
+  ctx->dgemm_timed = true;
+  ctx->dgemm_timed_flops = flops;
+  HSSK_LAUNCH(dgemm_fold_kernel, dim3(fblocks), dim3(256), 0, ctx->stream, f, m, ldp, alpha, beta);
+  hssk_rt::check_launch();
+}
+
+extern "C" int hssk_dgemm_pair(hssk_ctx* ctx, int m, double alpha, const double* A, long long lda, double beta,
+                               const hssk_dgemm_job* jobs, int count) {
+  HSSK_API_BEGIN
+  dgemm_pair_impl(ctx, m, alpha, A, lda, beta, jobs, count);
+  HSSK_API_END
 }
 
 extern "C" int hssk_dgemm(hssk_ctx* ctx, int transB, int m, long long n, long long k, double alpha,
diff --git a/strumpack_amd/hssk.py b/strumpack_amd/hssk.py
--- a/strumpack_amd/hssk.py
+++ b/strumpack_amd/hssk.py
@@ -142,6 +142,12 @@
 
 class Gen(C.Structure):
     _fields_ = [("kind", C.c_int), ("reserved", C.c_int), ("p", C.c_double * 4)]
+
+
+class DgemmJob(C.Structure):
+    _fields_ = [("transB", C.c_int), ("reserved", C.c_int), ("n", C.c_longlong), ("k", C.c_longlong),
+                ("B", C.c_void_p), ("ldb", C.c_longlong), ("gen", C.c_void_p), ("j0", C.c_longlong),
+                ("C", C.c_void_p), ("ldc", C.c_longlong)]
 
 
 HSSK_SYMBOLS = [
@@ -158,7 +164,7 @@
     "hssk_plan_begin", "hssk_plan_end", "hssk_plan_replay", "hssk_plan_destroy", "hssk_plan_size",
     "hssk_sketch_gen", "hssk_gen_elems", "hssk_gen_fill", "hssk_colsets", "hssk_colsets_max_universe",
     "hssk_cluster_median", "hssk_pchol_id_vbatched", "hssk_pchol_id_max_m", "hssk_pchol_id_rank_cap", "hssk_sum_partials", "hssk_gram_vbatched", "hssk_gram_gen_vbatched", "hssk_gram_gen_supported",
-    "hssk_sgemm_sketch", "hssk_narrow_f32", "hssk_gather_elems_f32",
+    "hssk_sgemm_sketch", "hssk_narrow_f32", "hssk_gather_elems_f32", "hssk_dgemm_pair",
 ]
 
 
@@ -248,6 +254,7 @@
         L.hssk_dgemm.argtypes = [C.c_void_p, C.c_int, C.c_int, C.c_longlong, C.c_longlong,
                                  C.c_double, C.c_void_p, C.c_longlong, C.c_void_p, C.c_longlong,
                                  C.c_double, C.c_void_p, C.c_longlong]
+        L.hssk_dgemm_pair.argtypes = [C.c_void_p, C.c_int, C.c_double, C.c_void_p, C.c_longlong, C.c_double, C.c_void_p, C.c_int]
         L.hssk_sgemm_sketch.argtypes = [C.c_void_p, C.c_int, C.c_int, C.c_longlong, C.c_longlong,
                                         C.c_double, C.c_void_p, C.c_longlong, C.c_void_p, C.c_longlong,
                                         C.c_double, C.c_void_p, C.c_longlong]
```

Measured after the change: 69840. No clear change (-0.1%).
